# MadNLP/MadNLP.jl

Hardware: AMD Instinct MI355X
Metric: IP iterations/sec + ms per factorize!/solve!, condensed KKT n≈1e4 (higher is better)
Workload: dtype f64; 1 GPU; BASELINE config C3: case1354pegase-shaped sparse-condensed KKT, one instance; N=11192, m=16646, nnz(K)=68688; step = compress_J+compress_H+build_kkt+factorize (n_f=1) + inertia fetch + 2 solve_linear_system per instance; algorithm=BUNCHKAUFMAN (device: static-pivot LDL^T), outer_block=0, batch_per_gpu=1, batch_api=n/a (one instance), parallelism=1 GPU(s) x 1 independent instance(s)

## Files before the change

include/madnlp_hip.h:

```cpp
#ifndef MADNLP_HIP_H
#define MADNLP_HIP_H

#include <stdint.h>

#ifdef __cplusplus
extern "C" {
#endif

#define MNK_VERSION 100

enum { MNK_HOST = 0, MNK_DEVICE = 1 };

enum { MNK_BUNCHKAUFMAN = 1, MNK_LU = 2, MNK_QR = 3, MNK_CHOLESKY = 4, MNK_LDL = 5, MNK_EVD = 6 };

typedef struct mnk_ctx mnk_ctx;
typedef struct mnk_sc mnk_sc;
typedef struct mnk_dc mnk_dc;
typedef struct mnk_ls mnk_ls;

int mnk_version(void);
const char* mnk_last_error_string(void);
int mnk_ctx_create(int device, void* stream, mnk_ctx** out);
int mnk_ctx_destroy(mnk_ctx* ctx);
int mnk_ctx_synchronize(mnk_ctx* ctx);
// ... 196 lines not shown
int mnk_ipm_vec_scatter_axpy(mnk_ipm* ipm, double* y, const int64_t* idx, double a, const double* x, int64_t n);
int mnk_ipm_vec_gather(mnk_ipm* ipm, double* out, double a, const double* x, const int64_t* idx, int64_t n);
int mnk_ipm_bound_dual_axpy(mnk_ipm* ipm, double* zl, double* zu, double a, const double* dzl, const double* dzu);
int mnk_ipm_bound_dual_fill(mnk_ipm* ipm, double* zl, double* zu, double v);
int mnk_ipm_gemv(mnk_ipm* ipm, int trans, int64_t m, int64_t n, double alpha, const double* A, int64_t lda, const double* x,
                 double beta, double* y);

int mnk_ipm_vec_mul(mnk_ipm* ipm, double* out, const double* a, const double* b, int64_t n);
int mnk_ipm_scale_cons(mnk_ipm* ipm, double* c, const double* con_scale, const double* slack, const int64_t* slack_pos,
                       int64_t ns, const double* rhs, int64_t m);
int mnk_ipm_scale_grad(mnk_ipm* ipm, double* f, int64_t n, int64_t ntot, double factor);

typedef struct mnk_opf mnk_opf;
int mnk_opf_create(mnk_ctx* ctx, int64_t nbus, int64_t ngen, int64_t nbranch, const int32_t* fr, const int32_t* to,
                   const int32_t* gen_bus, const double* arc_coef, const double* bus_data, const double* gen_cost,
                   mnk_opf** out);
int mnk_opf_destroy(mnk_opf* opf);
int mnk_opf_sizes(mnk_opf* opf, int64_t* n, int64_t* m, int64_t* nnzj, int64_t* nnzh);
int mnk_opf_obj_terms(mnk_opf* opf, const double* x, double* terms );
int mnk_opf_grad(mnk_opf* opf, const double* x, double* g);
int mnk_opf_cons(mnk_opf* opf, const double* x, double* c);
int mnk_opf_jac_coord(mnk_opf* opf, const double* x, double* jac);
int mnk_opf_hess_coord(mnk_opf* opf, const double* x, const double* y, double obj_weight, double* hess);

typedef struct mnk_tape mnk_tape;
int mnk_tape_create(mnk_ctx* ctx, int64_t n, int64_t m, void* out);
int mnk_tape_destroy(void* tape);
int mnk_tape_add_pattern(void* tape, int kind , int64_t R, int k, int q,
                         const int32_t* var_index, const double* params, const int32_t* rows,
                         int64_t ninstr0, const int32_t* code0, int64_t nconst0, const double* consts0, int64_t nout0,
                         const int32_t* out_operand0, const int32_t* out_j0, const int32_t* out_l0, int nslot0,
                         int64_t ninstr1, const int32_t* code1, int64_t nconst1, const double* consts1, int64_t nout1,
                         const int32_t* out_operand1, const int32_t* out_j1, const int32_t* out_l1, int nslot1,
                         int64_t ninstr2, const int32_t* code2, int64_t nconst2, const double* consts2, int64_t nout2,
                         const int32_t* out_operand2, const int32_t* out_j2, const int32_t* out_l2, int nslot2);
int mnk_tape_finalize(void* tape);
int mnk_tape_sizes(void* tape, int64_t* n, int64_t* m, int64_t* nterms, int64_t* nnzj, int64_t* nnzh);
int mnk_tape_extended(void* tape, int* mask);
int mnk_tape_get_structure(void* tape, int32_t* jac_I, int32_t* jac_J, int32_t* hess_I, int32_t* hess_J);
int mnk_tape_obj_terms(void* tape, const double* x, double* terms );
int mnk_tape_grad(void* tape, const double* x, double* g);
int mnk_tape_cons(void* tape, const double* x, double* c);
int mnk_tape_jac_coord(void* tape, const double* x, double* jac);
int mnk_tape_hess_coord(void* tape, const double* x, const double* y, double obj_weight, double* hess);

typedef struct mnk_schur mnk_schur;
int mnk_schur_create(mnk_ctx* ctx, int64_t ns_local, int64_t blk, int64_t nd, int algo, mnk_schur** out);
int mnk_schur_destroy(mnk_schur* h);
int mnk_schur_set_block(mnk_schur* h, int64_t k, const double* A_kk, int64_t lda, const double* C_dk, int64_t ldc,
                        int loc);
int mnk_schur_build_local(mnk_schur* h, const double* S0, int64_t lds0, int loc_s0, double* S_out, int64_t lds_out);
int mnk_schur_factorize_s(mnk_schur* h, const double* S, int64_t lds, int loc, int* info);
int mnk_schur_inertia_s(mnk_schur* h, int64_t* num_pos, int64_t* num_zero, int64_t* num_neg);
int mnk_schur_scenario_inertia(mnk_schur* h, int64_t k, int64_t* num_pos, int64_t* num_zero, int64_t* num_neg);
int mnk_schur_scenario_bk_info(mnk_schur* h, int64_t k, int* active, int* count);
int mnk_schur_forward(mnk_schur* h, double* rhs_k, double* contrib_d);
int mnk_schur_solve_s(mnk_schur* h, double* rhs_d);
int mnk_schur_backward(mnk_schur* h, double* rhs_k, const double* x_d);
void* mnk_schur_s_buffer(mnk_schur* h);
int mnk_schur_set_structure(mnk_schur* h, int64_t n, int64_t m, int64_t nv, int64_t nc, int64_t nnzh, const int32_t* hess_I,
                            const int32_t* hess_J, int64_t nnzj, const int32_t* jac_I, const int32_t* jac_J, int64_t n_ineq,
                            const int64_t* ind_ineq, int64_t n_eq, const int64_t* ind_eq, int index_base, int64_t ns_global,
                            const int64_t* local_scen, int own_design);
int mnk_schur_assemble(mnk_schur* h, const double* hess, const double* jac, const double* pr_diag, const double* du_diag, int loc);
void* mnk_schur_s0_buffer(mnk_schur* h);
int mnk_schur_get_block(mnk_schur* h, int64_t k, double* A_kk, double* C_dk, double* S0);
int mnk_schur_solve(mnk_schur* h, double* rhs_k, double* rhs_d, int loc);

int mnk_ls_debug_solve_trace(mnk_ls* ls, unsigned long long* out, int64_t n);

int mnk_ls_debug_dag_state(mnk_ls* ls, int* flags, int64_t nflags, int* chain, int64_t nchain, int* have);

int mnk_debug_grid_at_launch(int cu_first, int num_cu, int first, int per_cu);
int mnk_debug_shader_clock(mnk_ctx* ctx, double* mhz);

int mnk_debug_dag_tasks(int ntile, int chunk, int band_tiles, int js2, int taper0, int* out, int cap, int* first_phase);
int mnk_debug_dag_merged_tasks(int ntile, int chunk, int band_tiles, int js2, int taper0, int fill, int ninst, int period,
                               int* out, int cap);
int mnk_debug_dag_deal(int ntile, int chunk, int band_tiles, int js2, int taper0, int fill, int ninst, int period, int nq, int gang,
                       int* tasks_out, int* order, int cap, int* off, int* first_phase);

int mnk_sc_debug_tile_env(mnk_sc* sc, int64_t order, int32_t* out, int cap);
int mnk_debug_tile_env_csc(int64_t n, const int32_t* colptr, const int32_t* rowval, int index_base, int32_t* out, int cap);

int mnk_debug_update(mnk_ctx* ctx, int variant, int64_t M, int64_t K, const double* A, int64_t lda,
                     double* C, double* C2, int64_t ldc, int reps, double* ms);

#ifdef __cplusplus
}
#endif
#endif
```

madnlp.jl_amd/_lib.py:

```python
from __future__ import annotations

import ctypes as C
import os
import subprocess

_HERE = os.path.dirname(os.path.abspath(__file__))
CSRC = os.path.join(_HERE, "csrc")
LIBDIR = os.path.join(_HERE, "lib")
LIBPATH = os.path.join(LIBDIR, "libmadnlp_hip.so")
_LIB_OVERRIDE = os.environ.get("MNK_LIBPATH")
SOURCES = ["gemm_f64.hip", "dag.hip", "factor.hip", "solve.hip", "ls.hip", "sparse_kkt.hip", "dense_kkt.hip", "bk.hip", "schur.hip", "ipm_vec.hip", "opf_eval.hip", "qr.hip", "lu.hip", "evd.hip", "qn.hip", "tape_eval.hip", "nlp_scale.hip"]
HEADERS = ["common.h", "ls.h", "kkt_vec.h", "gemm_tile.h", "leaf64.h", "ipm_handle.h", os.path.join("..", "..", "include", "madnlp_hip.h")]

MNK_HOST, MNK_DEVICE = 0, 1
MNK_BUNCHKAUFMAN, MNK_LU, MNK_QR, MNK_CHOLESKY, MNK_LDL, MNK_EVD = 1, 2, 3, 4, 5, 6
MNK_SC_JT, MNK_SC_HESS, MNK_SC_AUG, MNK_SC_DIAGBUF = 0, 1, 2, 3
MNK_QN_BFGS, MNK_QN_DAMPED_BFGS = 1, 2


def _stale() -> bool:
    if not os.path.exists(LIBPATH):
        return True
    t = os.path.getmtime(LIBPATH)
    deps = [os.path.join(CSRC, s) for s in SOURCES + HEADERS]
# ... 130 lines not shown
    "mnk_ipm_set_f_RR": (C.c_int, [_vp, _vp, _vp, _vp, _vp, C.c_double]),
    "mnk_ipm_set_aug_rhs_RR": (C.c_int, [_vp, _vp, _vp, _vp, _vp, _vp, _vp, _vp, _vp, _vp, _vp, C.c_int64, _vp, _vp, _vp, C.c_double, C.c_double, _vp, _vp, _vp, _vp]),
    "mnk_ipm_finish_aug_solve_RR": (C.c_int, [_vp, _vp, _vp, _vp, _vp, _vp, _vp, _vp, _vp, _vp, _vp, C.c_int64, C.c_double, C.c_double]),
    "mnk_ipm_reset_bound_dual_1": (C.c_int, [_vp, _vp, _vp, C.c_int64, C.c_double, C.c_double]),
    "mnk_ipm_set_initial_bounds": (C.c_int, [_vp, _vp, _vp, C.c_int64, C.c_double]),
    "mnk_ipm_set_initial_rhs": (C.c_int, [_vp, _vp, _vp, _vp, _vp, _vp, C.c_int64, _vp, _vp]),
    "mnk_ipm_set_aug_rhs_ifr": (C.c_int, [_vp, _vp, C.c_int64, _vp, _vp, _vp, _vp]),
    "mnk_ipm_set_g_ifr": (C.c_int, [_vp, _vp, _vp, _vp, _vp, _vp, _vp, C.c_double]),
    "mnk_ipm_initialize_variables": (C.c_int, [_vp, _vp, _vp, _vp, C.c_int64, C.c_double, C.c_double]),
    "mnk_ipm_get_dot": (C.c_int, [_vp, _vp, _vp, C.c_int64, C.POINTER(C.c_double)]),
    "mnk_ipm_get_sum": (C.c_int, [_vp, _vp, C.c_int64, C.POINTER(C.c_double)]),
    "mnk_ipm_get_norm2": (C.c_int, [_vp, _vp, C.c_int64, C.POINTER(C.c_double)]),
    "mnk_ipm_vec_copy": (C.c_int, [_vp, _vp, _vp, C.c_int64]),
    "mnk_ipm_vec_fill": (C.c_int, [_vp, _vp, C.c_int64, C.c_double]),
    "mnk_ipm_vec_axpby": (C.c_int, [_vp, _vp, C.c_double, _vp, C.c_double, _vp, C.c_int64]),
    "mnk_ipm_vec_scatter_axpy": (C.c_int, [_vp, _vp, _vp, C.c_double, _vp, C.c_int64]),
    "mnk_ipm_vec_gather": (C.c_int, [_vp, _vp, C.c_double, _vp, _vp, C.c_int64]),
    "mnk_ipm_bound_dual_axpy": (C.c_int, [_vp, _vp, _vp, C.c_double, _vp, _vp]),
    "mnk_ipm_bound_dual_fill": (C.c_int, [_vp, _vp, _vp, C.c_double]),
    "mnk_ipm_gemv": (C.c_int, [_vp, C.c_int, C.c_int64, C.c_int64, C.c_double, _vp, C.c_int64, _vp, C.c_double, _vp]),
    "mnk_ipm_vec_mul": (C.c_int, [_vp, _vp, _vp, _vp, C.c_int64]),
    "mnk_ipm_scale_cons": (C.c_int, [_vp, _vp, _vp, _vp, _vp, C.c_int64, _vp, C.c_int64]),
    "mnk_ipm_scale_grad": (C.c_int, [_vp, _vp, C.c_int64, C.c_int64, C.c_double]),
    "mnk_opf_create": (C.c_int, [_vp, C.c_int64, C.c_int64, C.c_int64, _vp, _vp, _vp, _vp, _vp, _vp, C.POINTER(_vp)]),
    "mnk_opf_destroy": (C.c_int, [_vp]),
    "mnk_opf_sizes": (C.c_int, [_vp, _i64p, _i64p, _i64p, _i64p]),
    "mnk_opf_obj_terms": (C.c_int, [_vp, _vp, _vp]),
    "mnk_opf_grad": (C.c_int, [_vp, _vp, _vp]),
    "mnk_opf_cons": (C.c_int, [_vp, _vp, _vp]),
    "mnk_opf_jac_coord": (C.c_int, [_vp, _vp, _vp]),
    "mnk_opf_hess_coord": (C.c_int, [_vp, _vp, _vp, C.c_double, _vp]),
    "mnk_tape_create": (C.c_int, [_vp, C.c_int64, C.c_int64, _vp]),
    "mnk_tape_destroy": (C.c_int, [_vp]),
    "mnk_tape_add_pattern": (C.c_int, [_vp, C.c_int, C.c_int64, C.c_int, C.c_int, _vp, _vp, _vp]
                             + [C.c_int64, _vp, C.c_int64, _vp, C.c_int64, _vp, _vp, _vp, C.c_int] * 3),
    "mnk_tape_finalize": (C.c_int, [_vp]),
    "mnk_tape_sizes": (C.c_int, [_vp, _i64p, _i64p, _i64p, _i64p, _i64p]),
    "mnk_tape_extended": (C.c_int, [_vp, _vp]),
    "mnk_tape_get_structure": (C.c_int, [_vp, _vp, _vp, _vp, _vp]),
    "mnk_tape_obj_terms": (C.c_int, [_vp, _vp, _vp]),
    "mnk_tape_grad": (C.c_int, [_vp, _vp, _vp]),
    "mnk_tape_cons": (C.c_int, [_vp, _vp, _vp]),
    "mnk_tape_jac_coord": (C.c_int, [_vp, _vp, _vp]),
    "mnk_tape_hess_coord": (C.c_int, [_vp, _vp, _vp, C.c_double, _vp]),
    "mnk_sc_set_aug_RR": (C.c_int, [_vp, _vp, _vp, _vp, _vp, _vp, _vp, _vp, _vp, _vp, _vp, C.c_double, C.c_double, C.c_double]),
    "mnk_dc_set_aug_RR": (C.c_int, [_vp, _vp, _vp, _vp, _vp, _vp, _vp, _vp, _vp, _vp, _vp, C.c_double, C.c_double, C.c_double]),
    "mnk_ls_bk_info": (C.c_int, [_vp, C.POINTER(C.c_int), C.POINTER(C.c_int), _vp, _vp]),
    "mnk_ls_get_stat": (C.c_int, [_vp, C.c_char_p, C.POINTER(C.c_double)]),
    "mnk_sc_set_bounds": (C.c_int, [_vp, C.c_int64, _vp, C.c_int64, _vp, C.c_int]),
    "mnk_sc_set_barrier_terms": (C.c_int, [_vp, _vp, _vp, _vp, _vp, _vp, C.c_int]),
    "mnk_sc_solve_kkt": (C.c_int, [_vp, _vp, _vp, C.c_int]),
    "mnk_sc_mul": (C.c_int, [_vp, _vp, _vp, C.c_double, C.c_double, C.c_int]),
    "mnk_dc_set_bounds": (C.c_int, [_vp, C.c_int64, _vp, C.c_int64, _vp, C.c_int]),
    "mnk_dc_set_barrier_terms": (C.c_int, [_vp, _vp, _vp, _vp, _vp, _vp, C.c_int]),
    "mnk_dc_solve_kkt": (C.c_int, [_vp, _vp, _vp, C.c_int]),
    "mnk_dc_mul": (C.c_int, [_vp, _vp, _vp, C.c_double, C.c_double, C.c_int]),
    "mnk_schur_create": (C.c_int, [_vp, C.c_int64, C.c_int64, C.c_int64, C.c_int, C.POINTER(_vp)]),
    "mnk_schur_destroy": (C.c_int, [_vp]),
    "mnk_schur_set_block": (C.c_int, [_vp, C.c_int64, _vp, C.c_int64, _vp, C.c_int64, C.c_int]),
    "mnk_schur_build_local": (C.c_int, [_vp, _vp, C.c_int64, C.c_int, _vp, C.c_int64]),
    "mnk_schur_factorize_s": (C.c_int, [_vp, _vp, C.c_int64, C.c_int, C.POINTER(C.c_int)]),
    "mnk_schur_inertia_s": (C.c_int, [_vp, _i64p, _i64p, _i64p]),
    "mnk_schur_scenario_inertia": (C.c_int, [_vp, C.c_int64, _i64p, _i64p, _i64p]),
    "mnk_schur_scenario_bk_info": (C.c_int, [_vp, C.c_int64, C.POINTER(C.c_int), C.POINTER(C.c_int)]),
    "mnk_schur_forward": (C.c_int, [_vp, _vp, _vp]),
    "mnk_schur_solve_s": (C.c_int, [_vp, _vp]),
    "mnk_schur_backward": (C.c_int, [_vp, _vp, _vp]),
    "mnk_schur_s_buffer": (C.c_void_p, [_vp]),
    "mnk_schur_set_structure": (C.c_int, [_vp, C.c_int64, C.c_int64, C.c_int64, C.c_int64, C.c_int64, _vp, _vp, C.c_int64, _vp, _vp,
                                          C.c_int64, _vp, C.c_int64, _vp, C.c_int, C.c_int64, _vp, C.c_int]),
    "mnk_schur_assemble": (C.c_int, [_vp, _vp, _vp, _vp, _vp, C.c_int]),
    "mnk_schur_s0_buffer": (_vp, [_vp]),
    "mnk_schur_get_block": (C.c_int, [_vp, C.c_int64, _vp, _vp, _vp]),
    "mnk_schur_solve": (C.c_int, [_vp, _vp, _vp, C.c_int]),
    "mnk_ls_debug_solve_trace": (C.c_int, [_vp, _vp, C.c_int64]),
    "mnk_ls_debug_dag_state": (C.c_int, [_vp, _vp, C.c_int64, _vp, C.c_int64, _vp]),
    "mnk_debug_grid_at_launch": (C.c_int, [C.c_int, C.c_int, C.c_int, C.c_int]),
    "mnk_debug_shader_clock": (C.c_int, [_vp, _vp]),
    "mnk_debug_dag_tasks": (C.c_int, [C.c_int, C.c_int, C.c_int, C.c_int, C.c_int, _vp, C.c_int, _vp]),
    "mnk_debug_dag_merged_tasks": (C.c_int, [C.c_int] * 8 + [_vp, C.c_int]),
    "mnk_debug_dag_deal": (C.c_int, [C.c_int] * 10 + [_vp, _vp, C.c_int, _vp, _vp]),
    "mnk_sc_debug_tile_env": (C.c_int, [_vp, C.c_int64, _vp, C.c_int]),
    "mnk_debug_tile_env_csc": (C.c_int, [C.c_int64, _vp, _vp, C.c_int, _vp, C.c_int]),
    "mnk_factorize_batch_begin": (C.c_int, []),
    "mnk_factorize_batch_end": (C.c_int, []),
    "mnk_solve_batch_begin": (C.c_int, []),
    "mnk_solve_batch_end": (C.c_int, []),
    "mnk_release_idle_streams": (C.c_int, [C.c_int]),
    "mnk_sc_step_batch": (C.c_int, [C.c_int, _vp, _vp, _vp, _vp, _vp, _vp, C.c_int]),
    "mnk_ls_inertia_batch": (C.c_int, [C.c_int, _vp, _i64p, _i64p, _i64p]),
    "mnk_ls_solve_batch": (C.c_int, [C.c_int, _vp, _vp, C.c_int]),
    "mnk_debug_update": (C.c_int, [_vp, C.c_int, C.c_int64, C.c_int64, _vp, C.c_int64, _vp, _vp, C.c_int64, C.c_int,
                                   C.POINTER(C.c_double)]),
    "mnk_gemm_nt": (C.c_int, [_vp, C.c_int, C.c_int64, C.c_int64, C.c_int64, _vp, C.c_int64, _vp,
                              C.c_int64, _vp, C.c_int64]),
}


def lib():
    global _lib
    if _lib is not None:
        return _lib
    if not os.path.exists(LIBPATH):
        raise ImportError(
            f"{LIBPATH} is missing: run `python -c 'import __graft_entry__ as g; g.build()'` "
            "(hipcc --offload-arch=gfx950).  There is no CPU fallback for the KKT hot path.")
    try:
        import torch
    except Exception:
        pass
    l = C.CDLL(_LIB_OVERRIDE if _LIB_OVERRIDE and os.path.exists(_LIB_OVERRIDE) else LIBPATH)
    for name, (res, args) in SIGNATURES.items():
        f = getattr(l, name)
        f.restype = res
        f.argtypes = args
    _lib = l
    return l


class HipError(RuntimeError):
    pass


def check(rc: int, what: str = ""):
    if rc != 0:
        msg = lib().mnk_last_error_string()
        raise HipError(f"{what} failed (rc={rc}): {msg.decode() if msg else ''}")
```

madnlp.jl_amd/csrc/common.h:

```cpp
#pragma once
#include <hip/hip_runtime.h>
#include <cstdint>
#include <cstdlib>
#include <cstdio>
#include <cstring>
#include <mutex>
#include <string>
#include <vector>

#include "../../include/madnlp_hip.h"

namespace mnk {

void set_error(const char* fmt, ...);

#define MNK_HIP(call)                                                                   \
    do {                                                                                \
        hipError_t e_ = (call);                                                         \
        if (e_ != hipSuccess) {                                                         \
            mnk::set_error("%s:%d: %s -> %s", __FILE__, __LINE__, #call, hipGetErrorString(e_)); \
            return -2;                                                                  \
        }                                                                               \
    } while (0)

// ... 115 lines not shown

struct mnk_ctx {
    int device = 0;
    hipStream_t stream = nullptr;
    bool own_stream = false;
    hipStream_t sp = nullptr, su = nullptr;
    int panel_cus = 0;
    hipStream_t sp_dag = nullptr, su_dag = nullptr;
    hipStream_t sp_dagB = nullptr, su_dagB = nullptr;
    bool shared_dag_streams = false;
    int dag_cus = 0;
    hipStream_t sp_dag2 = nullptr, su_dag2 = nullptr;
    int dag_cus2 = 0;
    hipEvent_t ev_a = nullptr, ev_b = nullptr;
    hipStream_t s_fill = nullptr;
    std::vector<hipEvent_t> ev_panel, ev_next, ev_next2, ev_bdone;
    int num_cu = 256;
    int cu_first = 0;
    int total_cu = 256;
    bool partitioned = false;
    void* persist_slot = nullptr;
    int children = 0;
    bool released = false;
};
int mnk_masked_stream_pair(mnk_ctx* ctx, int chain_cus, hipStream_t* sp, hipStream_t* su);
int mnk_ctx_ensure_panel_streams(mnk_ctx* ctx);
int mnk_ctx_ensure_dag(mnk_ctx* ctx);
int mnk_ctx_ensure_dag2(mnk_ctx* ctx);
int mnk_ctx_ensure_batch_streams(mnk_ctx* ctx);
int mnk_solve_warmup(hipStream_t s);
int mnk_ctx_bulk_wgs(const mnk_ctx* ctx, int first, int per_cu);
int mnk_dag_warmup(hipStream_t* streams, int n, int nwg);
int mnk_live_contexts(int device);
int mnk_persist_begin(mnk_ctx* ctx, hipStream_t s);
int mnk_persist_end(mnk_ctx* ctx, hipStream_t s, int rc);
void mnk_ctx_child_added(mnk_ctx* ctx);
void mnk_ctx_child_gone(mnk_ctx* ctx);

namespace mnk {
struct PpDag {
    int* front;
    const int* af;
    int ntile;
    int need_front;
    int front_from;
    int af_tilecol;
    long spin_limit;
    unsigned long long* trace;
    unsigned long long* vmax;
    int* dbg;
};
}

namespace mnk {

int launch_gemm_nt(hipStream_t s, int mode, int64_t M, int64_t N, int64_t K,
                   const double* A, int64_t lda, const double* B, int64_t ldb,
                   double* C, int64_t ldc, const double* colscale, double* C2, int64_t ldc2,
                   const int* info_flag);
struct TrsmBatchRec { double* X; double* V; const double* dblk; const double* inv16; const double* dinv; const int* info; };
struct GemmBatchRec { const double* A; const double* B; double* C; const int* info; };
int launch_gemm_nt_batch(hipStream_t s, int64_t M, int64_t N, int64_t K, const GemmBatchRec* recs_dev, int nbatch, int64_t lda,
                         int64_t ldb, int64_t ldc);
int launch_gemm_nt_lower_small(hipStream_t s, int64_t M, int64_t N, int64_t K, const double* A, int64_t lda,
                               const double* B, int64_t ldb, double* C, int64_t ldc, const int* info_flag);
int gemm_nt_lower_tiles(int64_t M, int64_t N);
int launch_gemm_nt_dbg(hipStream_t s, int shared_ab, int64_t M, int64_t N, int64_t K, const double* A, int64_t lda,
                       const double* B, int64_t ldb, double* C, int64_t ldc);
int launch_gemm_nt_lower_range(hipStream_t s, int64_t M, int64_t N, int64_t K, const double* A, int64_t lda,
                               const double* B, int64_t ldb, double* C, int64_t ldc, const int* info_flag,
                               int tile_begin, int tile_count);
int launch_gemm_nt_queue(hipStream_t s, int64_t M, int64_t N, int64_t K, const double* A, int64_t lda,
                         const double* B, int64_t ldb, double* C, int64_t ldc, int* counter, int cus,
                         const int* info_flag);

int dag_build_tasks(int ntile, int chunk, int band_tiles, int js2, std::vector<int>& out, int taper0, std::vector<int>* ready);
int dag_add_fill_tasks(int ntile, std::vector<int>& tasks, std::vector<int>& ready, int n1);
void dag_merge_tasks(const std::vector<int>& tasks, const std::vector<int>& ready, int ninst, int period, std::vector<int>& out);
constexpr int DAG_NQ = 8;
constexpr int DAG_QHEAD_STRIDE = 32;
constexpr int DAG_QHEAD_WORDS = (DAG_NQ + 1) * DAG_QHEAD_STRIDE;
void dag_deal_tasks(const std::vector<int>& tasks, const std::vector<int>& ready, int t0, int t1, int nq, int gang, std::vector<int>& order,
                    std::vector<int>& off);

}
```

madnlp.jl_amd/csrc/dag.hip:

```cpp
#include <algorithm>
#include <atomic>
#include <cfloat>
#include <climits>
#include <vector>

#include "gemm_tile.h"
#include "ls.h"

namespace mnk {


struct DagInst {
    double* F;
    int64_t ld;
    double* V;
    const double* dinv;
    const double* dblk;
    const double* inv16;
    int* front;
    int* af;
    int* tprog;
    int* info;
    unsigned long long* vmax;
    double* zfill;
    int64_t N;
    const int* env;
    const int* envgate;
};

typedef const DagInst __attribute__((address_space(4))) * DagInstP;

struct DagArgs {
    const DagInst* insts;
    const int4* tasks;
    int ntasks;
    int ntile;
    int* qctr;
    long spin_limit;
    unsigned long long* trace;
    unsigned long long* wgstat;
    int fake_share;
};

constexpr int DAG_BANDACC = 1, DAG_FINAL = 2, DAG_FIRST = 4, DAG_FILL = 8;

template <class IP>
__device__ __forceinline__ int dag_wait_front(IP a, long spin_limit, int s0, int s1, int s2, int s3, int c, int kend, int* s_val) {
    if (threadIdx.x < 64) {
        const int lane = threadIdx.x;
        const int idx = lane == 0 ? s0 : (lane == 1 ? s1 : (lane == 2 ? s2 : s3));
        long spins = 0;
        int r;
        for (;;) {
            int f = lane < 4 ? __hip_atomic_load(a->front + idx, __ATOMIC_RELAXED, __HIP_MEMORY_SCOPE_AGENT) : INT_MAX;
            f = min(f, __shfl_xor(f, 1));
            f = min(f, __shfl_xor(f, 2));
            r = __builtin_amdgcn_readfirstlane(f);
            if (r > c) break;
            __builtin_amdgcn_s_sleep(4);
            if ((++spins & 255) == 0) {
                if (__hip_atomic_load(a->info, __ATOMIC_RELAXED, __HIP_MEMORY_SCOPE_AGENT) != 0) {
                    r = -1;
                    break;
                }
                if (spins > spin_limit) {
                    if (lane == 0 && atomicCAS(a->info, 0, -7) == 0) a->info[1] = 1;
                    r = -1;
                    break;
                }
            }
        }
        if (r > kend) r = kend;
        __builtin_amdgcn_fence(__ATOMIC_ACQUIRE, "agent");
        if (lane == 0) *s_val = r;
    }
    __syncthreads();
    const int r = *s_val;
    __syncthreads();
    return r;
}

template <class IP>
__device__ __forceinline__ bool dag_wait_words(IP a, long spin_limit, const int* w0, int t0, const int* w1, int t1, int* s_val) {
    if (threadIdx.x < 64) {
        const int lane = threadIdx.x;
        long spins = 0;
        int ok = 1;
        for (;;) {
            const int v = lane < 2 ? __hip_atomic_load(lane == 0 ? w0 : w1, __ATOMIC_RELAXED, __HIP_MEMORY_SCOPE_AGENT) : INT_MAX;
            if (__all(v >= (lane == 0 ? t0 : (lane == 1 ? t1 : INT_MIN)))) break;
            __builtin_amdgcn_s_sleep(2);
            if ((++spins & 255) == 0) {
                if (__hip_atomic_load(a->info, __ATOMIC_RELAXED, __HIP_MEMORY_SCOPE_AGENT) != 0) {
                    ok = 0;
                    break;
                }
                if (spins > spin_limit) {
                    if (lane == 0 && atomicCAS(a->info, 0, -7) == 0) a->info[1] = 2;
                    ok = 0;
                    break;
                }
            }
        }
        __builtin_amdgcn_fence(__ATOMIC_ACQUIRE, "agent");
        if (lane == 0) *s_val = ok;
    }
    __syncthreads();
    const int ok = *s_val;
    __syncthreads();
    return ok != 0;
// ... 279 lines not shown
#pragma unroll
            for (int i = 0; i < 8; ++i) { asm volatile("" : "+v"(X[i][0])); asm volatile("" : "+v"(X[i][1])); }
            if (tr) tr[1] = tr[3] = wall_clock64();
            if (dag_wait_front(in, a.spin_limit, 2 * J, 2 * J + 1, 2 * J, 2 * J + 1, J, J + 1, &s_val) < 0) return false;
            if (tr) { tr[4] = wall_clock64(); s_stat[1] += tr[4] - tr[3]; }
            dag_finalize_tile<LDL>(in, row0, col0, 2 * J, smem_raw, tid, X, tr);
            if (tr) s_stat[3] += wall_clock64() - tr[4];
        } else if (!(I == J && kend > k0)) {
            v4f64 acc[4][4];
#pragma unroll
            for (int i = 0; i < 4; ++i)
#pragma unroll
                for (int j = 0; j < 4; ++j) acc[i][j] = v4f64{0.0, 0.0, 0.0, 0.0};
            if (flags & DAG_FINAL) __builtin_amdgcn_s_setprio(3);
            if (!gemm_nt_mainloop<2, 2, 4, 0, 8>(acc, Ak, in->ld, Bk, in->ld, (kend - k0) * 16, smem_raw, tid, gate)) return false;
            if (tr) tr[1] = wall_clock64();
            if (!wait_chunk_order()) return false;
            if (kend > k0)
                gemm_nt_epilogue<2, 2, 4, 2, false, true>(acc, row0, col0, (int64_t)1 << 40, (int64_t)1 << 40, in->F, in->ld, nullptr, nullptr, 0, tid);
            if (tr) tr[3] = wall_clock64();
        } else {
            v4f64 acc[4][4];
#pragma unroll
            for (int i = 0; i < 4; ++i)
#pragma unroll
                for (int j = 0; j < 4; ++j) acc[i][j] = v4f64{0.0, 0.0, 0.0, 0.0};
            __builtin_amdgcn_s_setprio(3);
            if (!wait_chunk_order()) return false;
            gemm_nt_load_neg_lower<2, 2, 4>(acc, row0, col0, in->F, in->ld, tid);
            if (!gemm_nt_mainloop<2, 2, 4, 0, 8>(acc, Ak, in->ld, Bk, in->ld, (kend - k0) * 16, smem_raw, tid, gate)) return false;
            if (tr) tr[1] = wall_clock64();
            gemm_nt_store_neg_lower<2, 2, 4>(acc, row0, col0, in->F, in->ld, tid);
            if (tr) tr[3] = wall_clock64();
        }
        return true;
        };
        const bool done = run_task();
        asm volatile("s_waitcnt vmcnt(0)" ::: "memory");
        __syncthreads();
        if (done && tid == 0) {
            __builtin_amdgcn_fence(__ATOMIC_RELEASE, "agent");
            asm volatile("s_waitcnt vmcnt(0)" ::: "memory");
            if (!(flags & DAG_FINAL)) {
                __hip_atomic_store(in->tprog + (int64_t)I * a.ntile + J, q + 1, __ATOMIC_RELAXED, __HIP_MEMORY_SCOPE_AGENT);
            } else if (!(flags & DAG_BANDACC)) {
                __hip_atomic_store(in->front + 2 * I, J + 1, __ATOMIC_RELAXED, __HIP_MEMORY_SCOPE_AGENT);
                __hip_atomic_store(in->front + 2 * I + 1, J + 1, __ATOMIC_RELAXED, __HIP_MEMORY_SCOPE_AGENT);
            } else {
                __hip_atomic_store(in->af + (int64_t)I * a.ntile + J, 1, __ATOMIC_RELAXED, __HIP_MEMORY_SCOPE_AGENT);
            }
            if (tr) tr[5] = wall_clock64();
        }
        __builtin_amdgcn_s_setprio(0);
        __syncthreads();
        };
        do_task((DagInstP)(uintptr_t)(a.insts + inst));
    }
}

struct DagArgs1 {
    double* F;
    int64_t ld;
    double* V;
    const double* dinv;
    const double* dblk;
    const double* inv16;
    const int4* tasks;
    int ntasks;
    int* front;
    int* af;
    int* tprog;
    int ntile;
    int* qctr;
    int* info;
    long spin_limit;
    unsigned long long* trace;
    unsigned long long* wgstat;
    unsigned long long* vmax;
    int fake_share;
    double* zfill;
    int64_t N;
    const int* env;
    const int* envgate;
    const int* qoff;
    int* qheads;
    int nq;
};

__device__ __forceinline__ int dag_pop(const int* __restrict__ qoff, int* __restrict__ qheads, int nq, int* sq) {
    const int h = sq[0];
    if (h >= 0) {
        const int beg = qoff[h], n = qoff[h + 1] - beg;
        const int i = atomicAdd(qheads + h * DAG_QHEAD_STRIDE, 1);
        if (i < n) return beg + i;
        sq[0] = -1 - h;
    }
    for (;;) {
        int best = -1, most = 0;
        for (int x = 0; x < nq; ++x) {
            const int left = qoff[x + 1] - qoff[x] - __hip_atomic_load(qheads + x * DAG_QHEAD_STRIDE, __ATOMIC_RELAXED, __HIP_MEMORY_SCOPE_AGENT);
            if (left > most) { most = left; best = x; }
        }
        if (best < 0) return INT_MAX;
        const int i = atomicAdd(qheads + best * DAG_QHEAD_STRIDE, 1);
        if (i < qoff[best + 1] - qoff[best]) {
            sq[1] += 1;
            atomicAdd(qheads + nq * DAG_QHEAD_STRIDE, 1);
            return qoff[best] + i;
        }
    }
}

template <bool LDL>
__global__ __launch_bounds__(256, 3) void dag_bulk_kernel1(DagArgs1 a) {
    extern __shared__ __attribute__((aligned(16))) char smem_raw[];
    __shared__ int s_val;
    __shared__ int s_q[2];
    if (threadIdx.x == 0) {
        unsigned xcc;
        asm volatile("s_getreg_b32 %0, hwreg(HW_REG_XCC_ID)" : "=s"(xcc));
        s_q[0] = a.nq > 0 ? (int)(xcc & 15u) % a.nq : 0;
        s_q[1] = 0;
    }
    __shared__ unsigned long long s_stat[4];
    if (threadIdx.x < 4) s_stat[threadIdx.x] = 0;
    const int* __restrict__ env = a.env != nullptr && __builtin_amdgcn_readfirstlane(*a.envgate) == 0 ? a.env : nullptr;
    __syncthreads();
    for (;;) {
        int tid = threadIdx.x;
        asm volatile("" : "+v"(tid));
        if (tid == 0)
            s_val = __hip_atomic_load(a.info, __ATOMIC_RELAXED, __HIP_MEMORY_SCOPE_AGENT) != 0
                        ? INT_MAX
                        : (a.nq > 0 ? dag_pop(a.qoff, a.qheads, a.nq, s_q) : atomicAdd(a.qctr, 1));
        __syncthreads();
        const int t = s_val;
        __syncthreads();
        if (t >= a.ntasks) {
            if (a.wgstat != nullptr && tid == 0) {
                unsigned long long* w = a.wgstat + (int64_t)blockIdx.x * 8;
                w[0] = s_stat[0]; w[1] = wall_clock64(); w[2] = s_stat[1]; w[3] = s_stat[2]; w[4] = s_stat[3];
                w[5] = a.nq > 0 ? (unsigned long long)(1 + (s_q[0] >= 0 ? s_q[0] : -1 - s_q[0])) : 0; w[6] = (unsigned long long)s_q[1];
            }
            return;
        }
        if (a.wgstat != nullptr && tid == 0) { if (s_stat[0] == 0) s_stat[0] = wall_clock64(); ++s_stat[2]; }
        const int4 tk = a.tasks[t];
        const int flags = __builtin_amdgcn_readfirstlane(tk.x) & 255, q = __builtin_amdgcn_readfirstlane(tk.x) >> 8;
        const int I = __builtin_amdgcn_readfirstlane(tk.y), J = __builtin_amdgcn_readfirstlane(tk.z) & 0xfff;
        const int kbeg = __builtin_amdgcn_readfirstlane(tk.w) & 0xffff, kend = __builtin_amdgcn_readfirstlane(tk.w) >> 16;
        const int64_t row0 = (int64_t)128 * I, col0 = (int64_t)128 * J;
        unsigned long long* tr = a.trace != nullptr && tid == 0
                                     ? a.trace + (int64_t)(a.nq > 0 ? (int)((unsigned)__builtin_amdgcn_readfirstlane(tk.z) >> 12) : t) * 8
                                     : nullptr;
        if (tr) { tr[0] = wall_clock64(); tr[6] = 0; tr[7] = 0; }
        if (flags & DAG_FILL) {
            if (a.zfill != nullptr) dag_fill_tile(&a, I, J, tid);
            continue;
        }

        int eI = 0, k0 = kbeg;
        if (env != nullptr) {
            eI = __builtin_amdgcn_readfirstlane(env[I]);
            k0 = min(kend, max(kbeg, max(eI, __builtin_amdgcn_readfirstlane(env[J]))));
        }
        int limit = 0;
        auto gate_at = [&](int kc) -> int {
            const unsigned long long w0 = tr ? wall_clock64() : 0;
            const int r = dag_wait_front(&a, a.spin_limit, 2 * I, 2 * I + 1, 2 * J, 2 * J + 1, kc, kend, &s_val);
            if (tr) { const unsigned long long w1 = wall_clock64(); tr[2] = w1; tr[6] += 1; tr[7] += w1 - w0; s_stat[1] += w1 - w0; }
            return r;
        };
        auto gate = [&](int kt) -> bool {
            if (kt < limit) return true;
            const int r = gate_at(k0 + (kt >> 4));
            if (r < 0) return false;
            limit = (__builtin_amdgcn_readfirstlane(r) - k0) * 16;
            return true;
        };
        const double* Ak = a.F + (a.fake_share > 0 ? (int64_t)128 * (kend + I % a.fake_share) : row0) + (int64_t)128 * k0 * a.ld;
        const double* Bk = (LDL ? a.V : a.F) + (a.fake_share > 0 ? (int64_t)128 * (kend + J % a.fake_share) : col0) + (int64_t)128 * k0 * a.ld;
        auto wait_chunk_order = [&]() -> bool {
            if (flags & DAG_FIRST) return true;
            const int* word = a.tprog + (int64_t)I * a.ntile + J;
            const unsigned long long w0 = tr ? wall_clock64() : 0;
            if (!dag_wait_words(&a, a.spin_limit, word, q, word, q, &s_val)) return false;
            if (tr) s_stat[1] += wall_clock64() - w0;
            return true;
        };
        if ((flags & DAG_FINAL) && !(flags & DAG_BANDACC)) {
            __builtin_amdgcn_s_setprio(3);
            if (!wait_chunk_order()) return;
            if (J < eI) {
                if (kend > kbeg && gate_at(kbeg) < 0) return;
                if (LDL) dag_zero_tile(a.V, a.ld, row0, col0, tid);
                goto publish;
            }
            v4f64 X[8][2];
            {
                const int lane = tid & 63, w = tid >> 6;
                const double* Cs = a.F + (row0 + 32 * w + (lane & 15)) + (col0 + (lane >> 4)) * a.ld;
#pragma unroll
                for (int cb = 0; cb < 8; ++cb)
#pragma unroll
                    for (int r = 0; r < 4; ++r) {
                        const double* cp = Cs + (int64_t)(16 * cb + 4 * r) * a.ld;
                        X[cb][0][r] = cp[0];
                        X[cb][1][r] = cp[16];
                    }
            }
            if (kend > kbeg && gate_at(kbeg) < 0) return;
            if (kend > k0) (void)gemm_nt_mainloop3<2, 8, true>(X, Ak, a.ld, Bk, a.ld, (kend - k0) * 16, smem_raw, tid);
#pragma unroll
            for (int i = 0; i < 8; ++i) { asm volatile("" : "+v"(X[i][0])); asm volatile("" : "+v"(X[i][1])); }
            if (tr) tr[1] = tr[3] = wall_clock64();
            if (dag_wait_front(&a, a.spin_limit, 2 * J, 2 * J + 1, 2 * J, 2 * J + 1, J, J + 1, &s_val) < 0) return;
            if (tr) { tr[4] = wall_clock64(); s_stat[1] += tr[4] - tr[3]; }
            dag_finalize_tile<LDL>(&a, row0, col0, 2 * J, smem_raw, tid, X, tr);
            if (tr) s_stat[3] += wall_clock64() - tr[4];
        } else if (!(I == J && kend > k0)) {
            v4f64 acc[4][4];
#pragma unroll
            for (int i = 0; i < 4; ++i)
#pragma unroll
                for (int j = 0; j < 4; ++j) acc[i][j] = v4f64{0.0, 0.0, 0.0, 0.0};
            if (flags & DAG_FINAL) __builtin_amdgcn_s_setprio(3);
            if (!gemm_nt_mainloop<2, 2, 4, 0, 8>(acc, Ak, a.ld, Bk, a.ld, (kend - k0) * 16, smem_raw, tid, gate)) return;
            if (tr) tr[1] = wall_clock64();
            if (!wait_chunk_order()) return;
            if (kend > k0)
                gemm_nt_epilogue<2, 2, 4, 2, false, true>(acc, row0, col0, (int64_t)1 << 40, (int64_t)1 << 40, a.F, a.ld, nullptr, nullptr, 0, tid);
            if (tr) tr[3] = wall_clock64();
        } else {
            v4f64 acc[4][4];
#pragma unroll
            for (int i = 0; i < 4; ++i)
#pragma unroll
                for (int j = 0; j < 4; ++j) acc[i][j] = v4f64{0.0, 0.0, 0.0, 0.0};
            __builtin_amdgcn_s_setprio(3);
            if (!wait_chunk_order()) return;
            gemm_nt_load_neg_lower<2, 2, 4>(acc, row0, col0, a.F, a.ld, tid);
            if (!gemm_nt_mainloop<2, 2, 4, 0, 8>(acc, Ak, a.ld, Bk, a.ld, (kend - k0) * 16, smem_raw, tid, gate)) return;
            if (tr) tr[1] = wall_clock64();
            gemm_nt_store_neg_lower<2, 2, 4>(acc, row0, col0, a.F, a.ld, tid);
            if (tr) tr[3] = wall_clock64();
        }
    publish:
        asm volatile("s_waitcnt vmcnt(0)" ::: "memory");
        __syncthreads();
        if (tid == 0) {
            __builtin_amdgcn_fence(__ATOMIC_RELEASE, "agent");
            asm volatile("s_waitcnt vmcnt(0)" ::: "memory");
            if (!(flags & DAG_FINAL)) {
                __hip_atomic_store(a.tprog + (int64_t)I * a.ntile + J, q + 1, __ATOMIC_RELAXED, __HIP_MEMORY_SCOPE_AGENT);
            } else if (!(flags & DAG_BANDACC)) {
                __hip_atomic_store(a.front + 2 * I, J + 1, __ATOMIC_RELAXED, __HIP_MEMORY_SCOPE_AGENT);
                __hip_atomic_store(a.front + 2 * I + 1, J + 1, __ATOMIC_RELAXED, __HIP_MEMORY_SCOPE_AGENT);
            } else {
                __hip_atomic_store(a.af + (int64_t)I * a.ntile + J, 1, __ATOMIC_RELAXED, __HIP_MEMORY_SCOPE_AGENT);
            }
            if (tr) tr[5] = wall_clock64();
        }
        __builtin_amdgcn_s_setprio(0);
        __syncthreads();
    }
}

int dag_build_tasks(int ntile, int chunk, int band_tiles, int js2, std::vector<int>& out, int taper0, std::vector<int>* ready) {
    struct T { int ready, cls, J, I, flags, q, kbeg, kend; };
    std::vector<T> ts;
    auto add_tile = [&](int I, int J, int K, bool band) {
        const int body = band ? K : std::max(0, K - 1);
        std::vector<int> cuts{body};
        int e = body;
        for (int len = taper0; len < chunk && e > 0; len *= 2) { e = std::max(0, e - len); cuts.push_back(e); }
        const int first = 1 + (I * 5 + J * 3) % chunk;
        while (e > first) { e = std::max(first, e - chunk); cuts.push_back(e); }
        if (e > 0) cuts.push_back(0);
        int q = 0;
        for (int c = (int)cuts.size() - 1; c > 0; --c, ++q) {
            const int kb = cuts[c], ke = cuts[c - 1];
            const bool last = band && ke == K;
            ts.push_back({ke, band ? 0 : 2, J, I, (band ? DAG_BANDACC : 0) | (last ? DAG_FINAL : 0) | (q == 0 ? DAG_FIRST : 0), q, kb, ke});
        }
        if (!band) ts.push_back({K, 1, J, I, DAG_FINAL | (q == 0 ? DAG_FIRST : 0), q, body, K});
    };
    for (int Jt = 0; Jt < ntile; ++Jt) {
        const int Js = Jt / 2;
        const int bt = Js >= js2 ? ntile : band_tiles;
        for (int I = 2 * Js + bt; I < ntile; ++I) add_tile(I, Jt, Jt, false);
        if (2 * Js - 2 > 0)
            for (int I = std::max(2 * Js, Jt); I < 2 * Js + bt && I < ntile; ++I) add_tile(I, Jt, 2 * Js - 2, true);
    }
    std::stable_sort(ts.begin(), ts.end(), [](const T& x, const T& y) {
        if (x.ready != y.ready) return x.ready < y.ready;
        if (x.cls != y.cls) return x.cls < y.cls;
        if (x.J != y.J) return x.J < y.J;
        return x.I < y.I;
    });
    out.clear();
    out.reserve(ts.size() * 4);
    if (ready != nullptr) { ready->clear(); ready->reserve(ts.size()); }
    int n1 = 0;
    for (const T& t : ts) {
        if (t.ready <= 2 * js2) ++n1;
        if (ready != nullptr) ready->push_back(t.ready);
        out.push_back(t.flags | (t.q << 8));
        out.push_back(t.I);
        out.push_back(t.J);
        out.push_back(t.kbeg | (t.kend << 16));
    }
    return n1;
}

int dag_add_fill_tasks(int ntile, std::vector<int>& tasks, std::vector<int>& ready, int n1) {
    const int nt = (int)(tasks.size() / 4), nfill = ntile * (ntile + 1) / 2;
    const int span = n1 > 0 ? n1 : nt;
    if (span <= 0) return n1;
    std::vector<int> out, rdy;
    out.reserve(tasks.size() + 4 * (size_t)nfill);
    rdy.reserve(ready.size() + nfill);
    int fi = 0, fj = 0, done = 0;
    auto emit_fill = [&](int r) {
        out.push_back(DAG_FILL); out.push_back(fi); out.push_back(fj); out.push_back(0);
        rdy.push_back(r);
        if (++fi >= ntile) { ++fj; fi = fj; }
        ++done;
    };
    for (int t = 0; t < nt; ++t) {
        for (int k = 0; k < 4; ++k) out.push_back(tasks[4 * t + k]);
        rdy.push_back(ready[t]);
        if (t < span)
            while (done < (int)((int64_t)(t + 1) * nfill / span)) emit_fill(ready[t]);
    }
    tasks.swap(out);
    ready.swap(rdy);
    return n1 > 0 ? n1 + nfill : 0;
}

void dag_merge_tasks(const std::vector<int>& tasks, const std::vector<int>& ready, int ninst, int period, std::vector<int>& out) {
    const int nt = (int)ready.size();
    out.clear();
    out.reserve((size_t)ninst * nt * 4);
    std::vector<int> pos(ninst, 0);
    for (;;) {
        int best = -1;
        long bkey = 0;
        for (int i = 0; i < ninst; ++i) {
            if (pos[i] >= nt) continue;
            const long key = (long)i * period + ready[pos[i]];
            if (best < 0 || key < bkey) { best = i; bkey = key; }
        }
        if (best < 0) break;
        const int t = pos[best]++;
        out.push_back(tasks[4 * t]);
        out.push_back(tasks[4 * t + 1] | (best << 16));
        out.push_back(tasks[4 * t + 2]);
        out.push_back(tasks[4 * t + 3]);
    }
}

void dag_deal_tasks(const std::vector<int>& tasks, const std::vector<int>& ready, int t0, int t1, int nq, int gang, std::vector<int>& order,
                    std::vector<int>& off) {
    nq = std::max(nq, 1);
    std::vector<std::vector<int>> qs(nq);
    std::vector<int64_t> load(nq, 0);
    int rr = 0;
    auto cls = [&](int t) { const int f = tasks[4 * (size_t)t] & 255; return (f & DAG_FILL) ? 3 : ((f & DAG_BANDACC) ? 0 : ((f & DAG_FINAL) ? 1 : 2)); };
    auto ksteps = [&](int t) { return (tasks[4 * (size_t)t] & DAG_FILL) ? 0 : (tasks[4 * (size_t)t + 3] >> 16) - (tasks[4 * (size_t)t + 3] & 0xffff); };
    auto same = [&](int x, int y) {
        return ready[x] == ready[y] && cls(x) == cls(y) && tasks[4 * (size_t)x + 2] == tasks[4 * (size_t)y + 2] &&
               tasks[4 * (size_t)x + 3] == tasks[4 * (size_t)y + 3] && (tasks[4 * (size_t)x + 1] >> 16) == (tasks[4 * (size_t)y + 1] >> 16);
    };
    auto deal = [&](int b, int e) {
        int q = 0;
        if (gang >= 0) {
            q = rr % nq;
            for (int i = 1; i < nq; ++i)
                if (load[(rr + i) % nq] < load[q]) q = (rr + i) % nq;
            rr = q + 1;
        }
        for (int t = b; t < e; ++t) { qs[q].push_back(t); load[q] += ksteps(t); }
    };
    for (int i = t0; i < t1;) {
        int j = i + 1;
        const int c = cls(i);
        if (gang > 1 && (c == 0 || c == 2))
            while (j < t1 && same(i, j)) ++j;
        for (int b = i; b < j; b += std::max(gang, 1)) deal(b, std::min(j, b + std::max(gang, 1)));
        i = j;
    }
    order.clear();
    off.assign(1, 0);
    for (int q = 0; q < nq; ++q) {
        order.insert(order.end(), qs[q].begin(), qs[q].end());
        off.push_back((int)order.size());
    }
}

template <bool LDL>
static int launch_bulk_t(hipStream_t s, const DagArgs& a, int nwg) {
    const size_t smem = TILE3_LDS_BYTES;
    auto kern = dag_bulk_kernel<LDL>;
    static std::atomic<uint64_t> attr_devs{0};
    int dev = 0;
    MNK_HIP(hipGetDevice(&dev));
    if (!(attr_devs.load(std::memory_order_relaxed) >> (dev & 63) & 1)) {
        MNK_HIP(hipFuncSetAttribute((const void*)kern, hipFuncAttributeMaxDynamicSharedMemorySize, (int)smem));
        attr_devs.fetch_or(1ull << (dev & 63), std::memory_order_relaxed);
    }
    hipLaunchKernelGGL(kern, dim3(nwg), dim3(256), smem, s, a);
    MNK_HIP(hipGetLastError());
    return 0;
}

template <bool LDL>
static int launch_bulk1_t(hipStream_t s, const DagArgs1& a, int nwg) {
    const size_t smem = TILE3_LDS_BYTES;
    auto kern = dag_bulk_kernel1<LDL>;
    static std::atomic<uint64_t> attr_devs{0};
    int dev = 0;
    MNK_HIP(hipGetDevice(&dev));
    if (!(attr_devs.load(std::memory_order_relaxed) >> (dev & 63) & 1)) {
        MNK_HIP(hipFuncSetAttribute((const void*)kern, hipFuncAttributeMaxDynamicSharedMemorySize, (int)smem));
        attr_devs.fetch_or(1ull << (dev & 63), std::memory_order_relaxed);
    }
    hipLaunchKernelGGL(kern, dim3(nwg), dim3(256), smem, s, a);
    MNK_HIP(hipGetLastError());
    return 0;
}

static int launch_dag_bulk(hipStream_t s, bool ldl, const DagInst& one, const DagInst* insts, const int* tasks, int ntasks, int ntile,
                           int* qctr, long spin_limit, int nwg, unsigned long long* trace, unsigned long long* wgstat,
                           const int* qoff = nullptr, int* qheads = nullptr, int nq = 0) {
    if (ntasks <= 0) return 0;
    static const int fake = getenv("MNK_DAG_FAKE_SHARE") ? atoi(getenv("MNK_DAG_FAKE_SHARE")) : 0;
    if (insts == nullptr) {
        DagArgs1 a{one.F, one.ld, one.V, one.dinv, one.dblk, one.inv16, reinterpret_cast<const int4*>(tasks), ntasks, one.front, one.af,
                   one.tprog, ntile, qctr, one.info, spin_limit, trace, wgstat, one.vmax, fake, one.zfill, one.N, one.env, one.envgate,
                   qoff, qheads, nq};
        return ldl ? launch_bulk1_t<true>(s, a, nwg) : launch_bulk1_t<false>(s, a, nwg);
    }
    DagArgs a{insts, reinterpret_cast<const int4*>(tasks), ntasks, ntile, qctr, spin_limit, trace, wgstat, fake};
    return ldl ? launch_bulk_t<true>(s, a, nwg) : launch_bulk_t<false>(s, a, nwg);
}

}

using namespace mnk;

int mnk_dag_warmup(hipStream_t* streams, int n, int nwg) {
    static mnk::DevBuf<int> ctr;
    if (!ctr.p) {
        if (ctr.alloc(4)) return -2;
        MNK_HIP(hipMemset(ctr.p, 0, 4 * sizeof(int)));
    }
    for (int i = 0; i < n; ++i) {
        if (streams[i] == nullptr) continue;
        mnk::DagArgs1 a1{};
        a1.qctr = ctr.p;
        a1.info = ctr.p + 1;
        mnk::DagArgs a{};
        a.qctr = ctr.p;
        int rc = mnk::launch_bulk1_t<true>(streams[i], a1, nwg);
        if (!rc) rc = mnk::launch_bulk1_t<false>(streams[i], a1, nwg);
        if (!rc) rc = mnk::launch_bulk_t<true>(streams[i], a, nwg);
        if (!rc) rc = mnk::launch_bulk_t<false>(streams[i], a, nwg);
        if (rc) return rc;
    }
    for (int i = 0; i < n; ++i)
        if (streams[i] != nullptr) MNK_HIP(mnk::stream_wait(streams[i]));
    return 0;
}

long mnk_ls_dag_spin_limit(const mnk_ls* ls) {
    if (ls->dag_spin_limit > 0) return ls->dag_spin_limit;
    const double n = (double)ls->Np;
    const double t_est = n * n * n / 3.0 / 50e12;
    const double polls = 10.0 * t_est / 0.17e-6;
    const double floor_polls = mnk_live_contexts(ls->ctx->device) > 1 ? 5880000.0 : 588000.0;
    return (long)std::min(16777216.0, std::max(floor_polls, polls));
}

static int bulk_xcds(const mnk_ctx* c, int first) {
    bool has[8] = {false, false, false, false, false, false, false, false};
    for (int b = std::max(first, 0); b < c->num_cu; ++b) has[(c->cu_first + b) % 8] = true;
    int n = 0;
    for (bool x : has) n += x ? 1 : 0;
    return n;
}

static mnk::DagInst dag_instance(mnk_ls* ls) {
    const int ntile = (int)(ls->Np / 128), nblk = (int)(ls->Np / NBI);
    int* front = ls->dag_flags.p + 2;
    int* af = front + nblk;
    int* tprog = af + (size_t)ntile * ntile;
    double* zfill = (ls->dag_fill && ls->dag_has_fill && ls->spare_pending && ls->fact_spare.p && !ls->spare_zeroed) ? ls->fact_spare.p : nullptr;
    const bool env = ls->envelope && ls->env_dev != nullptr && ls->env_word.p != nullptr;
    return mnk::DagInst{ls->fact.p, ls->ld, ls->algo == MNK_LDL ? ls->vfull.p : nullptr, ls->dinv.p, ls->dblk.p, ls->inv16.p,
                        front, af, tprog, ls->info_dev.p, mnk_ls_growth_word(ls), zfill, ls->N, env ? ls->env_dev : nullptr,
                        env ? ls->env_word.p + 1 : nullptr};
}

int mnk_ls_dag_prepare(mnk_ls* ls) {
    mnk_ctx* ctx = ls->ctx;
    hipStream_t s = ctx->stream;
    const int64_t Np = ls->Np, ld = ls->ld;
    const bool ldl = ls->algo == MNK_LDL;
    const int ntile = (int)(Np / 128), nblk = (int)(Np / NBI), nsc = (int)((Np + 255) / 256);
    const size_t nflags = (size_t)2 + nblk + 2 * (size_t)ntile * ntile;
    auto give_up = [&]() {
        (void)hipGetLastError();
        ls->dag_tasks.release();
        ls->dag_flags.release();
        ls->dag_qoff.release();
        ls->dag_qheads.release();
        ls->vfull.release();
        return 1;
    };
    if (!ls->dag_tasks.p) {
        const int64_t deep_rows = std::min<int64_t>((int64_t)ctx->dag_cus2 * NBI, ls->dag_deep_rows);
        ls->dag_js2 = (ctx->dag_cus2 > 0 && Np <= deep_rows) ? 0 : nsc;
        if (ls->dag_js2_override >= 0) ls->dag_js2 = std::min(nsc, ls->dag_js2_override);
        std::vector<int>& h = ls->dag_host_tasks;
        ls->dag_ntasks1 = mnk::dag_build_tasks(ntile, ls->dag_chunk, ls->dag_band / 2, ls->dag_js2, h, ls->dag_taper0, &ls->dag_host_ready);
        ls->dag_has_fill = ls->dag_fill && ls->prefill && Np <= ls->prefill_max_rows;
        if (ls->dag_has_fill && h.empty()) ls->dag_has_fill = false;
        if (ls->dag_has_fill) ls->dag_ntasks1 = mnk::dag_add_fill_tasks(ntile, h, ls->dag_host_ready, ls->dag_ntasks1);
        ls->dag_ntasks = (int)(h.size() / 4);
        std::vector<int> dev_list = h, qoff(32, 0);
        ls->dag_nq[0] = ls->dag_nq[1] = 0;
        if (ls->dag_xcd_queues && ls->dag_ntasks < (1 << 20) && ntile < 4096) {
            const int part[3] = {0, ls->dag_ntasks1, ls->dag_ntasks};
            const int chain_cus[2] = {ctx->dag_cus, ctx->dag_cus2};
            for (int ph = 0; ph < 2; ++ph) {
                const int t0 = part[ph], t1 = part[ph + 1];
                if (t1 - t0 < mnk_ctx_bulk_wgs(ctx, chain_cus[ph], 3) || bulk_xcds(ctx, chain_cus[ph]) != mnk::DAG_NQ) continue;
                std::vector<int> order, off;
                mnk::dag_deal_tasks(h, ls->dag_host_ready, t0, t1, mnk::DAG_NQ, ls->dag_gang, order, off);
                for (int p = 0; p < t1 - t0; ++p) {
                    for (int k = 0; k < 4; ++k) dev_list[4 * (size_t)(t0 + p) + k] = h[4 * (size_t)order[p] + k];
                    dev_list[4 * (size_t)(t0 + p) + 2] |= (order[p] - t0) << 12;
                }
                for (int x = 0; x <= mnk::DAG_NQ; ++x) qoff[16 * ph + x] = off[x];
                ls->dag_nq[ph] = mnk::DAG_NQ;
            }
        }
        if (ls->dag_tasks.alloc(h.size() + 4)) return give_up();
        if (!ls->dag_qoff.p && ls->dag_qoff.alloc(qoff.size())) return give_up();
        if (!ls->dag_qheads.p && ls->dag_qheads.alloc(2 * (size_t)mnk::DAG_QHEAD_WORDS)) return give_up();
        {
            mnk::H2DGuard h2d;
            if (!h.empty() && hipMemcpyAsync(ls->dag_tasks.p, dev_list.data(), dev_list.size() * sizeof(int), hipMemcpyHostToDevice, s) != hipSuccess) return give_up();
            if (hipMemcpyAsync(ls->dag_qoff.p, qoff.data(), qoff.size() * sizeof(int), hipMemcpyHostToDevice, s) != hipSuccess) return give_up();
            if (mnk::stream_wait(s) != hipSuccess) return give_up();
        }
        if (ls->dag_flags.alloc(nflags)) return give_up();
    }
    if (ldl && !ls->vfull.p && ls->vfull.alloc((size_t)ld * Np + SLACK)) {
        (void)hipGetLastError();
        bool ok = false;
        if (ls->fact_spare.p && !ls->spare_zeroed) {
            ls->fact_spare.release();
            ls->prefill = 0;
            ls->spare_pending = false;
            ok = ls->vfull.alloc((size_t)ld * Np + SLACK) == 0;
        }
        if (!ok) return give_up();
    }
    if (ls->dag_trace_on) {
        const size_t ntr = (size_t)ls->dag_ntasks * 8 + 4096 * 8 + 1024 * 8;
        if (ls->dag_trace.n < ntr && ls->dag_trace.alloc(ntr)) return give_up();
    }
    return 0;
}

int mnk_ls_run_factorization_dag(mnk_ls* ls) {
    mnk_ctx* ctx = ls->ctx;
    hipStream_t s = ctx->stream;
    const int64_t Np = ls->Np;
    const bool ldl = ls->algo == MNK_LDL;
    const int ntile = (int)(Np / 128), nblk = (int)(Np / NBI), nsc = (int)((Np + 255) / 256);
    const size_t nflags = (size_t)2 + nblk + 2 * (size_t)ntile * ntile;
    MNK_REQUIRE(ls->dag_tasks.p && ls->dag_flags.p && (!ldl || ls->vfull.p), "task-DAG schedule: mnk_ls_dag_prepare was not called");
    const mnk::DagInst inst = dag_instance(ls);
    ls->dag_filled = inst.zfill != nullptr;
    ls->env_used = inst.env != nullptr;
    hipLaunchKernelGGL(mnk::dag_reset_kernel, dim3((unsigned)std::min<size_t>((nflags + 1023) / 1024, 64)), dim3(256), 0, s,
                       ls->dag_flags.p, (int64_t)nflags, ls->info_dev.p, inst, (mnk::DagInst*)nullptr, (const mnk::SmallSysRec*)nullptr,
                       ls->env_word.p, ls->dag_qheads.p, ls->dag_qheads.p ? 2 * mnk::DAG_QHEAD_WORDS : 0);
    ls->env_armed = false;
    int* qctr = ls->dag_flags.p;
    int* front = inst.front;
    const long spin_limit = mnk_ls_dag_spin_limit(ls);
    unsigned long long* trace = nullptr;
    if (ls->dag_trace_on && ls->dag_trace.p) {
        const size_t ntr = (size_t)ls->dag_ntasks * 8 + 4096 * 8 + 1024 * 8;
        MNK_HIP(hipMemsetAsync(ls->dag_trace.p, 0, ntr * sizeof(unsigned long long), s));
        trace = ls->dag_trace.p;
    }
    const int js2 = ls->dag_js2;
    auto phase = [&](hipStream_t sp, hipStream_t su, int chain_cus, int task0, int ntask, int* counter, int js_begin, int js_end,
                     unsigned strips) -> int {
        const bool small = js_begin == 0 && js_end == nsc && js2 == 0 && ls->dag_chain_inline;
        if (small) sp = s;
        MNK_HIP(hipEventRecord(ctx->ev_a, s));
        if (!small) MNK_HIP(hipStreamWaitEvent(sp, ctx->ev_a, 0));
        MNK_HIP(hipStreamWaitEvent(su, ctx->ev_a, 0));
        mnk::PpDag dag{front, inst.af, ntile, 0, 0, -1, spin_limit, trace ? trace + (size_t)ls->dag_ntasks * 8 + (size_t)js_begin * 8 * 16 : nullptr,
                  mnk_ls_growth_word(ls), ls->dag_debug ? ls->dag_dbg.p : nullptr};
        int rc = mnk_launch_pchain(ls, sp, dag, js_begin, js_end, strips);
        if (rc) return rc;
        const int ph = (int)(counter - qctr), nq = ls->dag_nq[ph];
        MNK_REQUIRE(nq == 0 || (ntask >= mnk_ctx_bulk_wgs(ctx, chain_cus, 3) && bulk_xcds(ctx, chain_cus) == nq),
                    "task-DAG schedule: the bulk grid does not cover the XCDs the task list was dealt for");
        rc = mnk::launch_dag_bulk(su, ldl, inst, nullptr, ls->dag_tasks.p + 4 * (size_t)task0, ntask, ntile, counter, spin_limit,
                                  std::min(ntask, mnk_ctx_bulk_wgs(ctx, chain_cus, 3)), trace ? trace + 8 * (size_t)task0 : nullptr,
                                  trace ? trace + (size_t)ls->dag_ntasks * 8 + 4096 * 8 + (task0 > 0 ? 512 * 8 : 0) : nullptr,
                                  ls->dag_qoff.p + 16 * ph, ls->dag_qheads.p + ph * mnk::DAG_QHEAD_WORDS, nq);
        if (rc) return rc;
        if (js_begin == 0 && js_end > 0) {
            const int64_t safe = std::min<int64_t>(js_end, std::max<int64_t>(0, (ntile - ls->dag_band / 2 - 1) / 2)) & ~(int64_t)1;
            if (strips == (unsigned)ls->dag_band && safe > 0) {
                rc = mnk_ls_invert_blocks(ls, su, 0, safe);
                if (rc) return rc;
                ls->inv_done = safe;
            }
        }
        if (small) {
            rc = mnk_ls_invert_blocks(ls, s, 0, nsc);
            if (rc) return rc;
            ls->inv_done = nsc;
        } else if (js_begin == 0 && js_end == nsc && js2 == 0) {
            hipLaunchKernelGGL(mnk::dag_gate_kernel, dim3(1), dim3(1), 0, su, front + (nblk - 1), ntile, ls->info_dev.p, spin_limit);
            rc = mnk_ls_invert_blocks(ls, su, 0, nsc);
            if (rc) return rc;
            ls->inv_done = nsc;
        }
        if (!small) MNK_HIP(hipEventRecord(ctx->ev_a, sp));
        MNK_HIP(hipEventRecord(ctx->ev_b, su));
        if (!small) MNK_HIP(hipStreamWaitEvent(s, ctx->ev_a, 0));
        MNK_HIP(hipStreamWaitEvent(s, ctx->ev_b, 0));
        return 0;
    };
    if (js2 > 0) {
        int rc = phase(ctx->sp_dag, ctx->su_dag, ctx->dag_cus, 0, ls->dag_ntasks1, qctr, 0, std::min(js2, nsc),
                       (unsigned)std::min<int64_t>(ls->dag_band, Np / NBI));
        if (rc) return rc;
    }
    if (js2 < nsc) {
        const int64_t rows2 = Np - 256 * (int64_t)js2;
        MNK_REQUIRE(ctx->sp_dag2 != nullptr, "task-DAG schedule: the deep-band streams are missing");
        int rc = phase(ctx->sp_dag2, ctx->su_dag2, ctx->dag_cus2, ls->dag_ntasks1, ls->dag_ntasks - ls->dag_ntasks1,
                       qctr + 1, js2, nsc, (unsigned)(rows2 / NBI));
        if (rc) return rc;
    }
    return 0;
}

namespace {
struct BatchState {
    int depth = 0;
    bool active = false;
    std::vector<mnk_ls*> pend;
};
thread_local BatchState t_batch;

struct BatchBuffers {
    mnk::DevBuf<int> tasks;
    mnk::DevBuf<int> qctr;
    mnk::DevBuf<char> insts, pcsys, aux;
    char* stage = nullptr;
    size_t stage_bytes = 0;
    hipEvent_t stage_ev = nullptr;
    int ntile = 0, ninst = 0, period = 0, chunk = 0, taper0 = 0, band = 0, ntasks = 0;
    bool fill = false;
    hipEvent_t ev[4] = {nullptr, nullptr, nullptr, nullptr};
};
BatchBuffers g_batch[64];
}

bool mnk_batch_active() { return t_batch.active; }

bool mnk_batch_defer(mnk_ls* ls) {
    if (!t_batch.active) return false;
    const int nsc = (int)((ls->Np + 255) / 256);
    if (ls->algo_now != 5 || (ls->dag_js2 != nsc && ls->dag_js2 != 0) || ls->dag_trace_on || ls->ctx->partitioned) return false;
    if (mnk_ctx_ensure_batch_streams(ls->ctx) != 0) (void)hipGetLastError();
    if (!ls->ctx->sp_dagB) return false;
    if (!ls->ev_defer && hipEventCreateWithFlags(&ls->ev_defer, hipEventDisableTiming) != hipSuccess) { (void)hipGetLastError(); return false; }
    if (hipEventRecord(ls->ev_defer, ls->ctx->stream) != hipSuccess) { (void)hipGetLastError(); return false; }
    ls->deferred = true;
    t_batch.pend.push_back(ls);
    return true;
}

static void batch_mark_done(mnk_ls* ls) {
    ls->factorized = true;
    ls->info_valid = false;
    ls->bk_active = false;
    ls->deferred = false;
}

static int batch_run_group(std::vector<mnk_ls*>& g) {
    mnk_ls* l0 = g[0];
    mnk_ctx* c0 = l0->ctx;
    hipStream_t h = c0->stream;
    MNK_HIP(hipSetDevice(c0->device));
    const int64_t Np = l0->Np;
    const bool ldl = l0->algo == MNK_LDL;
    const int ntile = (int)(Np / 128), nsc = (int)((Np + 255) / 256), ninst = (int)g.size();
    const size_t nflags = (size_t)2 + (size_t)(Np / NBI) + 2 * (size_t)ntile * ntile;
    for (mnk_ls* ls : g)
        if (ls->ctx->stream != h) MNK_HIP(hipStreamWaitEvent(h, ls->ev_defer, 0));
    int rc = mnk_persist_begin(c0, h);
    if (rc) return rc;
    auto body = [&]() -> int {
        BatchBuffers& B = g_batch[c0->device & 63];
        const int period = std::max((ntile + 1) / 2, l0->batch_period > 0 ? l0->batch_period : 0);
        if (B.ntile != ntile || B.ninst != ninst || B.period != period || B.chunk != l0->dag_chunk || B.taper0 != l0->dag_taper0 ||
            B.band != l0->dag_band || B.fill != l0->dag_has_fill || !B.tasks.p) {
            std::vector<int> merged;
            mnk::dag_merge_tasks(l0->dag_host_tasks, l0->dag_host_ready, ninst, period, merged);
            if (B.tasks.alloc(merged.size() + 4)) return -2;
            { mnk::H2DGuard h2d; MNK_HIP(hipMemcpy(B.tasks.p, merged.data(), merged.size() * sizeof(int), hipMemcpyHostToDevice)); }
            if (!B.qctr.p && B.qctr.alloc(4)) return -2;
            if (B.insts.alloc(sizeof(mnk::DagInst) * (size_t)ninst)) return -2;
            for (hipEvent_t& e : B.ev)
                if (!e) MNK_HIP(hipEventCreateWithFlags(&e, hipEventDisableTiming));
            B.ntile = ntile; B.ninst = ninst; B.period = period; B.chunk = l0->dag_chunk; B.taper0 = l0->dag_taper0;
            B.band = l0->dag_band; B.fill = l0->dag_has_fill; B.ntasks = (int)(merged.size() / 4);
        }
        std::vector<mnk::DagInst> hin;
        mnk::DagInst* insts_dev = reinterpret_cast<mnk::DagInst*>(B.insts.p);
        for (mnk_ls* ls : g) {
            hin.push_back(dag_instance(ls));
            ls->dag_filled = hin.back().zfill != nullptr;
            ls->env_used = hin.back().env != nullptr;
            hipLaunchKernelGGL(mnk::dag_reset_kernel, dim3((unsigned)std::min<size_t>((nflags + 1023) / 1024, 64)), dim3(256), 0, h,
                               ls->dag_flags.p, (int64_t)nflags, ls->info_dev.p, hin.back(), insts_dev + (hin.size() - 1),
                               (const mnk::SmallSysRec*)nullptr, ls->env_word.p);
            ls->env_armed = false;
        }
        MNK_HIP(hipMemsetAsync(B.qctr.p, 0, 4 * sizeof(int), h));
        hipStream_t sp[2] = {c0->sp_dag, c0->sp_dagB}, su = c0->su_dagB;
        MNK_HIP(hipEventRecord(B.ev[0], h));
        MNK_HIP(hipStreamWaitEvent(sp[0], B.ev[0], 0));
        MNK_HIP(hipStreamWaitEvent(sp[1], B.ev[0], 0));
        MNK_HIP(hipStreamWaitEvent(su, B.ev[0], 0));
        const unsigned strips = (unsigned)std::min<int64_t>(l0->dag_band, Np / NBI);
        const int bulk_wgs = mnk_ctx_bulk_wgs(c0, 2 * c0->dag_cus, 3);
        auto launch_chain = [&](int i) -> int {
            mnk_ls* ls = g[i];
            mnk::PpDag dag{hin[i].front, hin[i].af, ntile, 0, 0, -1, mnk_ls_dag_spin_limit(ls), nullptr, mnk_ls_growth_word(ls)};
            return mnk_launch_pchain(ls, sp[i & 1], dag, 0, nsc, strips);
        };
        auto launch_tail = [&](int i) -> int {
            mnk_ls* ls = g[i];
            int r = mnk_ls_invert_blocks(ls, sp[i & 1], 0, nsc);
            if (r) return r;
            ls->inv_done = nsc;
            return mnk_ls_launch_finish_info(ls, sp[i & 1]);
        };
        for (int i = 0; i < std::min(2, ninst); ++i) {
            int r = launch_chain(i);
            if (r) return r;
        }
        int r = mnk::launch_dag_bulk(su, ldl, hin[0], insts_dev, B.tasks.p, B.ntasks, ntile, B.qctr.p,
                                     mnk_ls_dag_spin_limit(l0), std::min(B.ntasks, bulk_wgs), nullptr, nullptr);
        if (r) return r;
        for (int i = 0; i < ninst; ++i) {
            r = launch_tail(i);
            if (r) return r;
            if (i + 2 < ninst) {
                r = launch_chain(i + 2);
                if (r) return r;
            }
        }
        MNK_HIP(hipEventRecord(B.ev[1], sp[0]));
        MNK_HIP(hipEventRecord(B.ev[2], sp[1]));
        MNK_HIP(hipEventRecord(B.ev[3], su));
        for (int e = 1; e < 4; ++e) MNK_HIP(hipStreamWaitEvent(h, B.ev[e], 0));
        return 0;
    };
    rc = body();
    rc = mnk_persist_end(c0, h, rc);
    if (rc) return rc;
    MNK_HIP(hipEventRecord(l0->ev_defer, h));
    for (mnk_ls* ls : g) {
        if (ls->ctx->stream != h) MNK_HIP(hipStreamWaitEvent(ls->ctx->stream, l0->ev_defer, 0));
        batch_mark_done(ls);
        int r = mnk_ls_prefill_spare(ls);
        if (r) return r;
    }
    return 0;
}

static int batch_run_group_small(std::vector<mnk_ls*>& g) {
    mnk_ls* l0 = g[0];
    mnk_ctx* c0 = l0->ctx;
    hipStream_t h = c0->stream;
    MNK_HIP(hipSetDevice(c0->device));
    const int64_t Np = l0->Np;
    const bool ldl = l0->algo == MNK_LDL;
    const int ntile = (int)(Np / 128), nsc = (int)((Np + 255) / 256), strips = (int)(Np / NBI);
    const size_t nflags = (size_t)2 + (size_t)(Np / NBI) + 2 * (size_t)ntile * ntile;
    const int ntasks1 = l0->dag_ntasks;
    const int bulk_min = ntasks1 > 0 ? std::max(32, c0->num_cu / 4) : 0;
    auto chain_cus_for = [&](int k) { return std::min(c0->num_cu, (k * strips + 63) / 64 * 64); };
    int kmax = std::min(32, (c0->num_cu - bulk_min) / strips);
    while (kmax > 1 && chain_cus_for(kmax) > c0->num_cu - bulk_min) --kmax;
    if (kmax < 2) {
        for (mnk_ls* ls : g) {
            ls->deferred = false;
            int rc = mnk_ls_run_factorization_now(ls);
            if (rc) return rc;
        }
        return 0;
    }
    for (mnk_ls* ls : g)
        if (ls->ctx->stream != h) MNK_HIP(hipStreamWaitEvent(h, ls->ev_defer, 0));
    BatchBuffers& B = g_batch[c0->device & 63];
    for (size_t r0 = 0; r0 < g.size(); r0 += (size_t)kmax) {
        const int k = (int)std::min<size_t>(kmax, g.size() - r0);
        hipStream_t sp = nullptr, su = nullptr;
        int rc = mnk_masked_stream_pair(c0, chain_cus_for(k), &sp, &su);
        if (rc) return rc;
        if (ntasks1 > 0 && su == nullptr) { set_error("factorize batch: no CUs left for the bulk kernel"); return -1; }
        rc = mnk_persist_begin(c0, h);
        if (rc) return rc;
        auto body = [&]() -> int {
            if (ntasks1 > 0 && (B.ntile != ntile || B.ninst != k || B.period != 0 || B.chunk != l0->dag_chunk || B.taper0 != l0->dag_taper0 ||
                                B.band != l0->dag_band || B.fill != l0->dag_has_fill || !B.tasks.p)) {
                std::vector<int> merged;
                mnk::dag_merge_tasks(l0->dag_host_tasks, l0->dag_host_ready, k, 0, merged);
                if (B.tasks.alloc(merged.size() + 4)) return -2;
                { mnk::H2DGuard h2d; MNK_HIP(hipMemcpy(B.tasks.p, merged.data(), merged.size() * sizeof(int), hipMemcpyHostToDevice)); }
                B.ntile = ntile; B.ninst = k; B.period = 0; B.chunk = l0->dag_chunk; B.taper0 = l0->dag_taper0;
                B.band = l0->dag_band; B.fill = l0->dag_has_fill; B.ntasks = (int)(merged.size() / 4);
            }
            if (!B.qctr.p && B.qctr.alloc(4)) return -2;
            if (B.insts.n < sizeof(mnk::DagInst) * (size_t)k && B.insts.alloc(sizeof(mnk::DagInst) * (size_t)std::max(k, 32))) return -2;
            if (B.pcsys.n < mnk_pchain_sys_bytes() * (size_t)k && B.pcsys.alloc(mnk_pchain_sys_bytes() * (size_t)std::max(k, 32))) return -2;
            for (hipEvent_t& e : B.ev)
                if (!e) MNK_HIP(hipEventCreateWithFlags(&e, hipEventDisableTiming));
            std::vector<mnk::DagInst> hin;
            std::vector<int*> fronts;
            std::vector<const int*> afs;
            mnk::DagInst* insts_dev = reinterpret_cast<mnk::DagInst*>(B.insts.p);
            const size_t pc_bytes = mnk_pchain_sys_bytes();
            const size_t need = (size_t)k * (sizeof(mnk::DagInst) + pc_bytes + sizeof(mnk::SmallSysRec));
            if (B.aux.n < sizeof(mnk::SmallSysRec) * (size_t)k && B.aux.alloc(sizeof(mnk::SmallSysRec) * (size_t)std::max(k, 32))) return -2;
            if (B.stage_ev == nullptr) MNK_HIP(hipEventCreateWithFlags(&B.stage_ev, hipEventDisableTiming));
            else MNK_HIP(hipEventSynchronize(B.stage_ev));
            if (B.stage_bytes < need) {
                mnk::LaunchLock lock;
                if (B.stage) { mnk::quiesce_persistent(); (void)hipHostFree(B.stage); B.stage = nullptr; }
                const size_t cap = (size_t)std::max(k, 32) * (sizeof(mnk::DagInst) + pc_bytes + sizeof(mnk::SmallSysRec));
                MNK_HIP(hipHostMalloc((void**)&B.stage, cap, hipHostMallocDefault));
                B.stage_bytes = cap;
            }
            mnk::DagInst* st_inst = reinterpret_cast<mnk::DagInst*>(B.stage);
            char* st_pc = B.stage + (size_t)k * sizeof(mnk::DagInst);
            mnk::SmallSysRec* st_aux = reinterpret_cast<mnk::SmallSysRec*>(st_pc + (size_t)k * pc_bytes);
            const bool batch_aux = l0->linv_mfma && !l0->solve512;
            for (int i = 0; i < k; ++i) {
                mnk_ls* ls = g[r0 + i];
                hin.push_back(dag_instance(ls));
                ls->dag_filled = hin.back().zfill != nullptr;
                hin.back().env = nullptr;
                hin.back().envgate = nullptr;
                ls->env_used = false;
                fronts.push_back(hin.back().front);
                afs.push_back(hin.back().af);
                st_inst[i] = hin.back();
                mnk_pchain_fill_sys(ls, st_pc + (size_t)i * pc_bytes, hin.back().front, hin.back().af);
                mnk_ls_fill_small_rec(ls, st_aux + i);
            }
            MNK_HIP(hipMemcpyAsync(B.insts.p, st_inst, (size_t)k * sizeof(mnk::DagInst), hipMemcpyHostToDevice, h));
            MNK_HIP(hipMemcpyAsync(B.pcsys.p, st_pc, (size_t)k * pc_bytes, hipMemcpyHostToDevice, h));
            MNK_HIP(hipMemcpyAsync(B.aux.p, st_aux, (size_t)k * sizeof(mnk::SmallSysRec), hipMemcpyHostToDevice, h));
            MNK_HIP(hipEventRecord(B.stage_ev, h));
            const mnk::SmallSysRec* aux_dev = reinterpret_cast<const mnk::SmallSysRec*>(B.aux.p);
            hipLaunchKernelGGL(mnk::dag_reset_kernel, dim3((unsigned)std::min<size_t>((nflags + 1023) / 1024, 64), (unsigned)k), dim3(256), 0, h,
                               (int*)nullptr, (int64_t)0, (int*)nullptr, hin[0], (mnk::DagInst*)nullptr, aux_dev);
            MNK_HIP(hipMemsetAsync(B.qctr.p, 0, 4 * sizeof(int), h));
            MNK_HIP(hipEventRecord(B.ev[0], h));
            MNK_HIP(hipStreamWaitEvent(sp, B.ev[0], 0));
            if (su != nullptr) MNK_HIP(hipStreamWaitEvent(su, B.ev[0], 0));
            int r = mnk_launch_pchain_multi(g.data() + r0, k, sp, nullptr, B.pcsys.p, fronts.data(), afs.data());
            if (r) return r;
            if (ntasks1 > 0) {
                const int bulk_wgs = mnk_ctx_bulk_wgs(c0, chain_cus_for(k), 3);
                r = mnk::launch_dag_bulk(su, ldl, hin[0], insts_dev, B.tasks.p, B.ntasks, ntile, B.qctr.p, mnk_ls_dag_spin_limit(l0),
                                         std::min(B.ntasks, bulk_wgs), nullptr, nullptr);
                if (r) return r;
                MNK_HIP(hipEventRecord(B.ev[2], su));
                MNK_HIP(hipStreamWaitEvent(h, B.ev[2], 0));
            }
            MNK_HIP(hipEventRecord(B.ev[1], sp));
            MNK_HIP(hipStreamWaitEvent(h, B.ev[1], 0));
            if (su != nullptr) MNK_HIP(hipStreamWaitEvent(su, B.ev[1], 0));
            if (su != nullptr) MNK_HIP(hipStreamWaitEvent(sp, B.ev[2], 0));
            if (batch_aux) {
                r = mnk_ls_invert_blocks_batch(h, ldl, aux_dev, k, Np);
                if (r) return r;
                r = mnk_ls_finish_info_batch(h, aux_dev, k, ldl ? (l0->N >= 4096 ? 1024 : 256) : 64);
                if (r) return r;
                for (int i = 0; i < k; ++i) {
                    mnk_ls* ls = g[r0 + i];
                    ls->inv_done = nsc;
                    if (!ls->ev_info) MNK_HIP(hipEventCreateWithFlags(&ls->ev_info, hipEventDisableTiming));
                    MNK_HIP(hipEventRecord(ls->ev_info, h));
                    ls->ev_info_recorded = true;
                }
                return 0;
            }
            hipStream_t inv_s[3] = {h, sp, su != nullptr ? su : sp};
            for (int i = 0; i < k; ++i) {
                mnk_ls* ls = g[r0 + i];
                hipStream_t si = inv_s[i % 3];
                r = mnk_ls_invert_blocks(ls, si, 0, nsc);
                if (r) return r;
                ls->inv_done = nsc;
                r = mnk_ls_launch_finish_info(ls, si);
                if (r) return r;
            }
            MNK_HIP(hipEventRecord(B.ev[1], sp));
            MNK_HIP(hipStreamWaitEvent(h, B.ev[1], 0));
            if (su != nullptr) {
                MNK_HIP(hipEventRecord(B.ev[2], su));
                MNK_HIP(hipStreamWaitEvent(h, B.ev[2], 0));
            }
            return 0;
        };
        rc = body();
        rc = mnk_persist_end(c0, h, rc);
        if (rc) return rc;
    }
    MNK_HIP(hipEventRecord(l0->ev_defer, h));
    for (mnk_ls* ls : g) {
        if (ls->ctx->stream != h) MNK_HIP(hipStreamWaitEvent(ls->ctx->stream, l0->ev_defer, 0));
        batch_mark_done(ls);
        int r = mnk_ls_prefill_spare(ls);
        if (r) return r;
    }
    return 0;
}

static int batch_flush() {
    std::vector<mnk_ls*> pend;
    pend.swap(t_batch.pend);
    int rc_all = 0;
    while (!pend.empty()) {
        mnk_ls* l0 = pend.front();
// ... 30 lines not shown

bool mnk_ls_pending_elsewhere(const mnk_ls* ls) {
    return ls->deferred && std::find(t_batch.pend.begin(), t_batch.pend.end(), ls) == t_batch.pend.end();
}

int mnk_ls_sync_deferred_fact(mnk_ls* ls) {
    if (!ls->deferred) return 0;
    if (std::find(t_batch.pend.begin(), t_batch.pend.end(), ls) == t_batch.pend.end()) {
        set_error("a factorize! call of this solver is pending in a batch that another thread opened (mnk_factorize_batch_end must come first)");
        return -1;
    }
    return batch_flush();
}

extern "C" int mnk_factorize_batch_begin(void) {
    ++t_batch.depth;
    t_batch.active = true;
    return 0;
}

extern "C" int mnk_factorize_batch_end(void) {
    if (t_batch.depth <= 0) { set_error("mnk_factorize_batch_end: no batch is open on this thread"); return -1; }
    if (--t_batch.depth > 0) return 0;
    t_batch.active = false;
    return batch_flush();
}

extern "C" int mnk_debug_dag_tasks(int ntile, int chunk, int band_tiles, int js2, int taper0, int* out, int cap, int* first_phase) {
    if (ntile <= 0 || chunk <= 0 || band_tiles <= 0 || taper0 <= 0) return -1;
    std::vector<int> h;
    const int n1 = mnk::dag_build_tasks(ntile, chunk, band_tiles, js2, h, taper0, nullptr);
    const int n = (int)(h.size() / 4);
    if (first_phase != nullptr) *first_phase = n1;
    if (out != nullptr)
        for (int i = 0; i < std::min(n, cap) * 4; ++i) out[i] = h[i];
    return n;
}

extern "C" int mnk_debug_dag_merged_tasks(int ntile, int chunk, int band_tiles, int js2, int taper0, int fill, int ninst, int period,
                                          int* out, int cap) {
    if (ntile <= 0 || chunk <= 0 || band_tiles <= 0 || taper0 <= 0 || ninst <= 0 || period < 0) return -1;
    std::vector<int> h, ready, merged;
    int n1 = mnk::dag_build_tasks(ntile, chunk, band_tiles, js2, h, taper0, &ready);
    if (fill) n1 = mnk::dag_add_fill_tasks(ntile, h, ready, n1);
    mnk::dag_merge_tasks(h, ready, ninst, period, merged);
    const int n = (int)(merged.size() / 4);
    if (out != nullptr)
        for (int i = 0; i < std::min(n, cap) * 4; ++i) out[i] = merged[i];
    return n;
}

extern "C" int mnk_debug_dag_deal(int ntile, int chunk, int band_tiles, int js2, int taper0, int fill, int ninst, int period, int nq,
                                  int gang, int* tasks_out, int* order, int cap, int* off, int* first_phase) {
    if (ntile <= 0 || chunk <= 0 || band_tiles <= 0 || taper0 <= 0 || ninst <= 0 || period < 0 || nq <= 0 || nq > 64 || gang == 0) return -1;
    std::vector<int> h, ready;
    int n1 = mnk::dag_build_tasks(ntile, chunk, band_tiles, js2, h, taper0, &ready);
    if (fill) n1 = mnk::dag_add_fill_tasks(ntile, h, ready, n1);
    if (ninst > 1) {
        std::vector<int> merged, mready, pos(ninst, 0);
        mnk::dag_merge_tasks(h, ready, ninst, period, merged);
        for (size_t t = 0; t < merged.size() / 4; ++t) { const int i = merged[4 * t + 1] >> 16; mready.push_back(i * period + ready[pos[i]++]); }
        h.swap(merged);
        ready.swap(mready);
        n1 = (int)ready.size();
    }
    const int n = (int)ready.size();
    if (first_phase != nullptr) *first_phase = n1;
    const int part[3] = {0, n1, n};
    int written = 0;
    for (int ph = 0; ph < 2; ++ph) {
        std::vector<int> ord, o;
        mnk::dag_deal_tasks(h, ready, part[ph], part[ph + 1], nq, gang, ord, o);
        for (int x = 0; x <= nq; ++x)
            if (off != nullptr) off[ph * (nq + 1) + x] = part[ph] + o[x];
        for (int v : ord) {
            if (order != nullptr && written < cap) order[written] = v;
            ++written;
        }
    }
    if (tasks_out != nullptr)
        for (int i = 0; i < std::min(n, cap) * 4; ++i) tasks_out[i] = h[i];
    return n;
}
```

madnlp.jl_amd/csrc/factor.hip:

```cpp
#include <atomic>
#include <type_traits>
#include <atomic>
#include <cfloat>
#include <chrono>
#include <cmath>
#include <cstdlib>

#include "ls.h"
#include "leaf64.h"

namespace mnk {

template <bool LDL, int NS>
__device__ __forceinline__ void trsm64_mfma_body(double* __restrict__ F, int64_t ld, int64_t j0, int64_t Np,
                                                 const double* __restrict__ Dblk, const double* __restrict__ inv16,
                                                 const double* __restrict__ dinv, double* __restrict__ W, int64_t ldw,
                                                 int64_t wcol, const int* __restrict__ info,
                                                 unsigned long long* __restrict__ vmax) {
    if (*info != 0) return;
    const int lane = threadIdx.x & 63, wave = threadIdx.x >> 6;
    const int l15 = lane & 15, l4 = lane >> 4;
    const int64_t r0 = j0 + 64 + ((int64_t)blockIdx.x * 4 + wave) * (16 * NS);
    if (r0 >= Np) return;
    double Ln[6][4];
// ... 912 lines not shown
        }
    }
    const bool ldl = ls->algo == MNK_LDL;
    const int epoch16 = ls->epoch * 16;
    double* V = ldl ? ls->vfull.p : nullptr;
    if (ldl)
        hipLaunchKernelGGL(pchain_kernel<true>, dim3(strips), dim3(256), PC_LDS_BYTES, sp, ls->fact.p, ls->ld, ls->Np, ls->dblk.p,
                           ls->inv16.p, ls->dvec.p, ls->dinv.p, V, ls->info_dev.p, ls->pivot_tol, ls->flag_p.p, epoch16,
                           ls->debug_pp_missing, dag, js_begin, js_end);
    else
        hipLaunchKernelGGL(pchain_kernel<false>, dim3(strips), dim3(256), PC_LDS_BYTES, sp, ls->fact.p, ls->ld, ls->Np, ls->dblk.p,
                           ls->inv16.p, ls->dvec.p, ls->dinv.p, V, ls->info_dev.p, ls->pivot_tol, ls->flag_p.p, epoch16,
                           ls->debug_pp_missing, dag, js_begin, js_end);
    MNK_HIP(hipGetLastError());
    return 0;
}

static int run_factorization_body(mnk_ls* ls);

size_t mnk_pchain_sys_bytes() { return sizeof(mnk::PcSys); }
void mnk_pchain_fill_sys(mnk_ls* ls, void* rec_host, int* front, const int* af) {
    const bool ldl = ls->algo == MNK_LDL;
    *static_cast<mnk::PcSys*>(rec_host) = mnk::PcSys{ls->fact.p, ls->ld, ls->Np, ls->dblk.p, ls->inv16.p, ls->dvec.p, ls->dinv.p,
                                                       ldl ? ls->vfull.p : nullptr, ls->info_dev.p, ls->pivot_tol, ls->flag_p.p,
                                                       ls->epoch * 16, front, af, (int)(ls->Np / 128), mnk_ls_dag_spin_limit(ls),
                                                       mnk_ls_growth_word(ls)};
}

int mnk_launch_pchain_multi(mnk_ls* const* v, int n, hipStream_t sp, hipStream_t fill_stream, void* table, int* const* front,
                            const int* const* af) {
    {
        static std::atomic<uint64_t> attr_devs{0};
        int dev = 0;
        MNK_HIP(hipGetDevice(&dev));
        if (!(attr_devs.load(std::memory_order_relaxed) >> (dev & 63) & 1)) {
            MNK_HIP(hipFuncSetAttribute((const void*)pchain_multi_kernel<true>, hipFuncAttributeMaxDynamicSharedMemorySize, PC_LDS_BYTES));
            MNK_HIP(hipFuncSetAttribute((const void*)pchain_multi_kernel<false>, hipFuncAttributeMaxDynamicSharedMemorySize, PC_LDS_BYTES));
            attr_devs.fetch_or(1ull << (dev & 63), std::memory_order_relaxed);
        }
    }
    mnk::PcSys* dst = static_cast<mnk::PcSys*>(table);
    const bool ldl = v[0]->algo == MNK_LDL;
    const int strips = (int)(v[0]->Np / NBI);
    for (int i = 0; i < n && fill_stream != nullptr; ++i) {
        mnk_ls* ls = v[i];
        mnk::PcSys rec{ls->fact.p, ls->ld, ls->Np, ls->dblk.p, ls->inv16.p, ls->dvec.p, ls->dinv.p, ldl ? ls->vfull.p : nullptr,
                       ls->info_dev.p, ls->pivot_tol, ls->flag_p.p, ls->epoch * 16, front[i], af[i], (int)(ls->Np / 128),
                       mnk_ls_dag_spin_limit(ls), mnk_ls_growth_word(ls)};
        hipLaunchKernelGGL(pc_set_sys_kernel, dim3(1), dim3(1), 0, fill_stream, rec, dst + i);
    }
    MNK_HIP(hipGetLastError());
    if (ldl)
        hipLaunchKernelGGL(pchain_multi_kernel<true>, dim3((unsigned)(n * strips)), dim3(256), PC_LDS_BYTES, sp, dst, strips);
    else
        hipLaunchKernelGGL(pchain_multi_kernel<false>, dim3((unsigned)(n * strips)), dim3(256), PC_LDS_BYTES, sp, dst, strips);
    MNK_HIP(hipGetLastError());
    return 0;
}

int mnk_ls_run_factorization(mnk_ls* ls) {
    if (ls->algo == MNK_QR) return mnk_qr_factor(ls);
    if (ls->algo == MNK_LU) return mnk_lu_factor(ls);
    if (ls->algo == MNK_EVD) return mnk_evd_factor(ls);
    mnk_ctx* ctx = ls->ctx;
    hipStream_t s = ctx->stream;
    const int64_t Np = ls->Np;
    if (ls->panel_algo >= 4 && !ls->flag_p.p) {
        if (ls->flag_p.alloc(Np / NBI + 1)) return -2;
        MNK_HIP(hipMemsetAsync(ls->flag_p.p, 0, (Np / NBI + 1) * sizeof(int), s));
    }
    ++ls->epoch;
    ls->inv_done = 0;
    ls->factor_invalid = false;
    ls->t_fact_launch_ms = mnk_host_ms();
    {
        const int want = (ls->early_reject && ls->accept_only_pd && ls->algo == MNK_LDL && ls->src_persistent) ? 1 : 0;
        if (want != ls->reject_on_device) {
            MNK_HIP(hipMemsetAsync(ls->info_dev.p + 2, want, sizeof(int), s));
            ls->reject_on_device = want;
        }
    }
    ls->algo_now = ls->panel_algo;
    ls->env_used = false;
    const int64_t min_rows = mnk_batch_active() ? std::min<int64_t>(ls->dag_min_rows, 256) : ls->dag_min_rows;
    if (ls->algo_now == 5 && (ctx->dag_cus < ls->dag_band || !ls->lookahead || Np < min_rows || Np > ls->dag_max_rows)) ls->algo_now = 4;
    if (ls->algo_now == 5 && ctx->sp_dag == nullptr && mnk_ctx_ensure_dag(ctx) != 0) { (void)hipGetLastError(); ls->algo_now = 4; }
    if (ls->algo_now == 5 && ctx->sp_dag == nullptr) ls->algo_now = 4;
    ++ls->fact_count;
    if (ls->pp_blocked && ls->fact_count >= ls->pp_retry_at) ls->pp_blocked = false;
    if (ls->algo_now >= 4 && ls->pp_blocked) ls->algo_now = 1;
    if (ls->algo_now == 5 && mnk_ls_dag_prepare(ls) != 0) ls->algo_now = 4;
    if (ls->algo_now == 5 && ls->dag_js2 < (Np + 255) / 256) {
        if (mnk_ctx_ensure_dag2(ctx) != 0) (void)hipGetLastError();
        if (ctx->sp_dag2 == nullptr) ls->algo_now = 4;
    }
    if (ls->algo_now == 5 && mnk_batch_defer(ls)) return 0;
    return mnk_ls_run_factorization_now(ls);
}

int mnk_ls_run_factorization_now(mnk_ls* ls) {
    mnk_ctx* ctx = ls->ctx;
    hipStream_t s = ctx->stream;
    const bool persistent = ls->algo_now >= 4;
    if (persistent) {
        int rc0 = mnk_persist_begin(ctx, s);
        if (rc0) return rc0;
    }
    const int rc_run = run_factorization_body(ls);
    return persistent ? mnk_persist_end(ctx, s, rc_run) : rc_run;
}

static int run_factorization_body(mnk_ls* ls) {
    mnk_ctx* ctx = ls->ctx;
    hipStream_t s = ctx->stream;
    const int64_t Np = ls->Np, ld = ls->ld;
    const bool ldl = ls->algo == MNK_LDL;
    double* F = ls->fact.p;
    const int64_t NBO = mnk_ls_effective_nbo(ls);
    if (ls->algo_now != 5) MNK_HIP(hipMemsetAsync(ls->info_dev.p, 0, 2 * sizeof(int), s));
    std::vector<int64_t> bnd{0};
    for (int64_t pos = 0; pos < Np;) {
        const bool tail = ls->lookahead && NBO < Np && ls->tail_rows > 0 && Np - pos <= ls->tail_rows && ls->tail_nbo < NBO;
        pos = std::min<int64_t>(pos + (tail ? ls->tail_nbo : NBO), Np);
        bnd.push_back(pos);
    }
    const int64_t npanel = (int64_t)bnd.size() - 1;
    const bool la = ls->lookahead && npanel > 1;

    if (ls->algo_now == 5) {
        int rc = mnk_ls_run_factorization_dag(ls);
        if (rc) return rc;
    } else if (!la) {
        for (int64_t ko = 0; ko < Np; ko += NBO) {
            const int64_t kend = std::min<int64_t>(ko + NBO, Np);
            int rc = factor_outer_panel(ls, s, ko, kend, ls->wbuf[0].p);
            if (rc) return rc;
            const int64_t Mt = Np - kend;
            if (Mt > 0) {
                const double* Wsrc = ldl ? ls->wbuf[0].p + kend : F + kend + ko * ld;
                rc = launch_gemm_nt(s, 2, Mt, Mt, kend - ko, Wsrc, ldl ? ls->ldw : ld, F + kend + ko * ld, ld,
                                    F + kend + kend * ld, ld, nullptr, nullptr, 0, ls->info_dev.p);
                if (rc) return rc;
            }
        }
    } else {
        { int rc_s = mnk_ctx_ensure_panel_streams(ctx); if (rc_s) return rc_s; }
        hipStream_t sp = ctx->sp, su = ctx->su;
        if ((int64_t)ctx->ev_panel.size() < npanel + 1) {
            const size_t old = ctx->ev_panel.size();
            ctx->ev_panel.resize(npanel + 1);
            ctx->ev_next.resize(npanel + 1);
            ctx->ev_next2.resize(npanel + 1);
            ctx->ev_bdone.resize(npanel + 1);
            for (size_t e = old; e < ctx->ev_panel.size(); ++e) {
                MNK_HIP(hipEventCreateWithFlags(&ctx->ev_panel[e], hipEventDisableTiming));
                MNK_HIP(hipEventCreateWithFlags(&ctx->ev_next[e], hipEventDisableTiming));
                MNK_HIP(hipEventCreateWithFlags(&ctx->ev_next2[e], hipEventDisableTiming));
                MNK_HIP(hipEventCreateWithFlags(&ctx->ev_bdone[e], hipEventDisableTiming));
            }
        }
        const int pcus = ctx->panel_cus;
        const int ucus = pcus > 0 ? ctx->num_cu - pcus : ctx->num_cu;
        const bool share = ls->share != 0;
        if (share) {
            if (ls->tile_ctr.n < 8 * ((size_t)npanel + 1)) {
                int rc0 = ls->tile_ctr.alloc(8 * ((size_t)npanel + 1));
// ... 309 lines not shown
```

madnlp.jl_amd/csrc/gemm_tile.h:

```cpp
#pragma once
#include "common.h"

namespace mnk {

typedef double v4f64 __attribute__((ext_vector_type(4)));
typedef double v2f64 __attribute__((ext_vector_type(2)));

constexpr int BK = 16;
constexpr bool tile_big(int wm, int wn, int wt) { return wm == 2 && wn == 2 && wt == 4; }
constexpr int tile_bk(int wm, int wn, int wt) { return tile_big(wm, wn, wt) ? 8 : BK; }
constexpr int tile_occ(int wm, int wn, int wt) { return tile_big(wm, wn, wt) ? 3 : 2; }

template <int MODE>
__device__ __forceinline__ void decode_tile(int logical, int ntm, int nc, int sw, int& tm, int& tn) {
    if (MODE == 2 || MODE == 4) {
        const double bq = 2.0 * ntm + 1.0;
        int c = (int)((bq - sqrt(bq * bq - 8.0 * (double)logical)) * 0.5);
        if (c < 0) c = 0;
        while (c > 0 && c * ntm - c * (c - 1) / 2 > logical) --c;
        while ((c + 1) * ntm - (c + 1) * c / 2 <= logical) ++c;
        if (sw <= 1) {
            tn = c;
            tm = tn + (logical - (c * ntm - c * (c - 1) / 2));
            return;
        }
        const int r0 = (c / sw) * sw;
        const int W = nc - r0 < sw ? nc - r0 : sw;
        int rem = logical - (r0 * ntm - r0 * (r0 - 1) / 2);
        const int tri = W * (W + 1) / 2;
        if (rem < tri) {
            int i = (int)((sqrt(8.0 * (double)rem + 1.0) - 1.0) * 0.5);
            while (i > 0 && i * (i + 1) / 2 > rem) --i;
            while ((i + 1) * (i + 2) / 2 <= rem) ++i;
            tm = r0 + i;
            tn = r0 + (rem - i * (i + 1) / 2);
        } else {
            rem -= tri;
            tm = r0 + W + rem / W;
            tn = r0 + rem % W;
        }
    } else {
        tm = logical % ntm;
        tn = logical / ntm;
    }
}

struct GemmNoGate {
    __device__ __forceinline__ bool operator()(int) const { return true; }
};
template <int WM, int WN, int WT, int DBG, int BKT, class GATE = GemmNoGate>
__device__ __forceinline__ bool gemm_nt_mainloop(v4f64 (&acc)[WT][WT], const double* __restrict__ Ag, int64_t lda,
                                                 const double* __restrict__ Bg, int64_t ldb, int nk, char* smem_raw,
                                                 int tid, GATE gate = GATE()) {
    constexpr int NT = 64 * WM * WN;
    constexpr int WS = 16 * WT;
    constexpr int BM = WS * WM, BN = WS * WN;
    constexpr int LDA_S = BM + 16, LDB_S = BN + 16;
    constexpr int APIECES = (BM / 2) * BKT / NT;
    constexpr int BPIECES = (BN / 2) * BKT / NT;
    static_assert(APIECES >= 1 && BPIECES >= 1, "tile too small for the thread count");

    double* As = reinterpret_cast<double*>(smem_raw);
    double* Bs = As + 2 * BKT * LDA_S;

    const int lane = tid & 63;
    const int wave = tid >> 6;
    const int wm = wave % WM, wn = wave / WM;
    const int l15 = lane & 15, l4 = lane >> 4;

    v2f64 ra[APIECES], rb[BPIECES];

    auto gload = [&](int kt) {
        const int64_t k0 = (int64_t)kt * BKT;
#pragma unroll
        for (int q = 0; q < APIECES; ++q) {
            int p = tid + NT * q;
            int k = p / (BM / 2), r = (p % (BM / 2)) * 2;
            ra[q] = *reinterpret_cast<const v2f64*>(Ag + r + (k0 + k) * lda);
        }
#pragma unroll
        for (int q = 0; q < BPIECES; ++q) {
            int p = tid + NT * q;
            int k = p / (BN / 2), r = (p % (BN / 2)) * 2;
            rb[q] = *reinterpret_cast<const v2f64*>(Bg + r + (k0 + k) * ldb);
        }
    };
    auto sstore = [&](int buf) {
        double* as = As + buf * BKT * LDA_S;
        double* bs = Bs + buf * BKT * LDB_S;
#pragma unroll
        for (int q = 0; q < APIECES; ++q) {
            int p = tid + NT * q;
            int k = p / (BM / 2), r = (p % (BM / 2)) * 2;
            *reinterpret_cast<v2f64*>(as + k * LDA_S + r) = ra[q];
        }
#pragma unroll
        for (int q = 0; q < BPIECES; ++q) {
            int p = tid + NT * q;
            int k = p / (BN / 2), r = (p % (BN / 2)) * 2;
            *reinterpret_cast<v2f64*>(bs + k * LDB_S + r) = rb[q];
        }
    };

    constexpr bool DMA = BM == 128 && BN == 128 && (DBG == 0 || DBG == 1 || DBG == 4);
    constexpr int NW = NT / 64;
    auto gl_lds = [&](int kt, int buf) {
        const int64_t k0 = (int64_t)kt * BKT;
        double* as = As + buf * BKT * LDA_S;
        double* bs = Bs + buf * BKT * LDB_S;
#pragma unroll
        for (int i = 0; i < BKT / NW; ++i) {
            const int k = wave * (BKT / NW) + i;
            __builtin_amdgcn_global_load_lds((const __attribute__((address_space(1))) void*)(Ag + (k0 + k) * lda + lane * 2),
                                             (__attribute__((address_space(3))) void*)(as + k * LDA_S), 16, 0, 0);
            __builtin_amdgcn_global_load_lds((const __attribute__((address_space(1))) void*)(Bg + (k0 + k) * ldb + lane * 2),
                                             (__attribute__((address_space(3))) void*)(bs + k * LDB_S), 16, 0, 0);
        }
    };
    if (nk <= 0) return true;
    if (!gate(0)) return false;
    if (DMA) {
        gl_lds(0, 0);
        asm volatile("s_waitcnt vmcnt(0)" ::: "memory");
    } else {
        gload(0);
        sstore(0);
    }
    __syncthreads();

    for (int kt = 0; kt < nk; ++kt) {
        const int cur = kt & 1;
        if (kt + 1 < nk && !gate(kt + 1)) return false;
        if (DMA) {
            if (kt + 1 < nk) gl_lds(kt + 1, cur ^ 1);
        } else if (DBG != 3 && kt + 1 < nk) {
            gload(kt + 1);
        }
        const double* as = As + cur * BKT * LDA_S + wm * WS + l15;
        const double* bs = Bs + cur * BKT * LDB_S + wn * WS + l15;
#pragma unroll
        for (int kk = 0; kk < BKT / 4; ++kk) {
            double af[WT], bf[WT];
#pragma unroll
            for (int i = 0; i < WT; ++i) {
                af[i] = as[(kk * 4 + l4) * LDA_S + i * 16];
                bf[i] = bs[(kk * 4 + l4) * LDB_S + i * 16];
            }
#pragma unroll
            for (int ni = 0; ni < WT; ++ni)
#pragma unroll
                for (int mi = 0; mi < WT; ++mi)
                    acc[ni][mi] = __builtin_amdgcn_mfma_f64_16x16x4f64(bf[ni], af[mi], acc[ni][mi], 0, 0, 0);
        }
        if (DMA) {
            asm volatile("s_waitcnt vmcnt(0)" ::: "memory");
            __syncthreads();
        } else {
            if (DBG != 3 && kt + 1 < nk) sstore(cur ^ 1);
            if (DBG != 2 && DBG != 3) __syncthreads();
        }
    }
    return true;
}

constexpr int TILE3_ROWS = 8 * 128 + 16 * 4;
constexpr int TILE3_LDS_BYTES = 3 * 2 * TILE3_ROWS * 8;
__device__ __forceinline__ constexpr int tile3_row(int k) { return k * 128 + 16 * ((k + 1) >> 1); }
template <int MI = 4, int NI = 4, bool NEG = false, class GATE = GemmNoGate>
__device__ __forceinline__ bool gemm_nt_mainloop3(v4f64 (&acc)[NI][MI], const double* __restrict__ Ag, int64_t lda,
                                                  const double* __restrict__ Bg, int64_t ldb, int nk, char* smem_raw, int tid,
                                                  GATE gate = GATE()) {
    static_assert(MI * NI == 16 && 128 % (16 * MI) == 0, "four waves cover the 128x128 tile");
    constexpr int BKT = 8, WSM = 16 * MI, WSN = 16 * NI, WAVES_M = 128 / WSM;
    double* Ls = reinterpret_cast<double*>(smem_raw);
    const int lane = tid & 63;
    const int wave = tid >> 6;
    const int wm = wave % WAVES_M, wn = wave / WAVES_M;
    const int l15 = lane & 15, l4 = lane >> 4;
    auto gl_lds = [&](int kt, int buf) {
        const int64_t k0 = (int64_t)kt * BKT;
        double* as = Ls + buf * 2 * TILE3_ROWS;
        double* bs = as + TILE3_ROWS;
#pragma unroll
        for (int i = 0; i < 2; ++i) {
            const int k = wave * 2 + i;
            const int off = tile3_row(k);
            __builtin_amdgcn_global_load_lds((const __attribute__((address_space(1))) void*)(Ag + (k0 + k) * lda + lane * 2),
                                             (__attribute__((address_space(3))) void*)(as + off), 16, 0, 0);
            __builtin_amdgcn_global_load_lds((const __attribute__((address_space(1))) void*)(Bg + (k0 + k) * ldb + lane * 2),
                                             (__attribute__((address_space(3))) void*)(bs + off), 16, 0, 0);
        }
    };
    if (nk <= 0) return true;
    if (!gate(0)) return false;
    gl_lds(0, 0);
    if (nk > 1) {
        if (!gate(1)) return false;
        gl_lds(1, 1);
        asm volatile("s_waitcnt vmcnt(4)\n\ts_barrier" ::: "memory");
    } else {
        asm volatile("s_waitcnt vmcnt(0)\n\ts_barrier" ::: "memory");
    }
    int cur = 0;
    for (int kt = 0; kt < nk; ++kt) {
        const int nxt2 = cur == 0 ? 2 : cur - 1;
        const bool more = kt + 2 < nk;
        if (more) {
            if (!gate(kt + 2)) return false;
            gl_lds(kt + 2, nxt2);
        }
        const double* as = Ls + cur * 2 * TILE3_ROWS + wm * WSM + l15 + tile3_row(l4);
        const double* bs = Ls + cur * 2 * TILE3_ROWS + TILE3_ROWS + wn * WSN + l15 + tile3_row(l4);
#pragma unroll
        for (int kk = 0; kk < BKT / 4; ++kk) {
            double af[MI];
#pragma unroll
            for (int i = 0; i < MI; ++i) {
                af[i] = as[kk * (4 * 128 + 32) + i * 16];
                if (NEG) af[i] = -af[i];
            }
#pragma unroll
            for (int n0 = 0; n0 < NI; n0 += 4) {
                double bf[4];
#pragma unroll
                for (int i = 0; i < 4; ++i) bf[i] = bs[kk * (4 * 128 + 32) + (n0 + i) * 16];
#pragma unroll
                for (int ni = 0; ni < 4; ++ni)
#pragma unroll
                    for (int mi = 0; mi < MI; ++mi)
                        acc[n0 + ni][mi] = __builtin_amdgcn_mfma_f64_16x16x4f64(bf[ni], af[mi], acc[n0 + ni][mi], 0, 0, 0);
                if (NI > 4) __builtin_amdgcn_sched_barrier(0);
            }
        }
        if (more)
            asm volatile("s_waitcnt vmcnt(4)\n\ts_barrier" ::: "memory");
// ... 128 lines not shown
```

madnlp.jl_amd/csrc/ls.h:

```cpp
#pragma once
#include <algorithm>
#include <functional>
#include <memory>
#include <string>
#include <vector>

#include "common.h"

struct mnk_sc {
    mnk_ctx* ctx = nullptr;
    int64_t n = 0, m = 0, nnzj = 0, nnzh = 0;
    int64_t nnz_jt = 0, nnz_hess = 0, nnz_aug = 0, len_jptr = 0;
    std::vector<int32_t> jt_colptr, jt_rowval, h_colptr, h_rowval, aug_colptr, aug_rowval;
    std::vector<int32_t> tile_env;
    mnk::DevBuf<int32_t> d_tile_env;
    std::vector<int64_t> jt_map, h_map;
    std::vector<int32_t> d_dst, d_src, hp_dst, hp_src, j_dst, j_c, j_k, j_l;
    mnk::DevBuf<int32_t> jt_seg_ptr, jt_seg_src, h_seg_ptr, h_seg_src;
    mnk::DevBuf<int32_t> aug_hptr, aug_hsrc;
    mnk::DevBuf<int32_t> aug_dsrc;
    mnk::DevBuf<int32_t> aug_jptr, aug_jc, aug_jk, aug_jl;
    mnk::DevBuf<int32_t> aug_row, aug_col;
    mnk::DevBuf<int32_t> d_jt_colptr, d_jt_rowval, d_jt_colidx, d_h_colptr, d_h_rowval, d_h_colidx;
    mnk::DevBuf<double> jac_coo, hess_coo, jt_nz, h_nz, aug_nz, diag_buffer, pr_diag, du_diag;
    void* extra = nullptr;
    std::shared_ptr<int> alive = std::make_shared<int>(0);
};

inline std::vector<int32_t> mnk_tile_envelope(int64_t n, const int32_t* row, const int32_t* col, int64_t nnz) {
    std::vector<int32_t> fnz(n);
    for (int64_t i = 0; i < n; ++i) fnz[i] = (int32_t)i;
    for (int64_t k = 0; k < nnz; ++k)
        if (row[k] >= 0 && row[k] < n && col[k] < fnz[row[k]]) fnz[row[k]] = col[k];
    const int64_t ntile = (n + 127) / 128;
    std::vector<int32_t> env(ntile);
    for (int64_t I = 0; I < ntile; ++I) {
        int32_t f = (int32_t)(128 * I);
        for (int64_t i = 128 * I; i < std::min<int64_t>(n, 128 * I + 128); ++i) f = std::min(f, fnz[i]);
        env[I] = f / 128;
    }
    return env;
}

struct mnk_dc {
    mnk_ctx* ctx = nullptr;
    int condensed = 1;
    bool mirror_pending = false;
    int64_t n = 0, m = 0, ns = 0, n_eq = 0, order = 0;
    std::vector<int64_t> ind_ineq, ind_eq;
    mnk::DevBuf<int64_t> d_ind_ineq, d_ind_eq;
    mnk::DevBuf<double> hess, jac, aug, pr_diag, du_diag, diag_buffer;
    mnk::DevBuf<double> jis;
    int64_t ld_jis = 0, kpad = 0, npad = 0;
    void* extra = nullptr;
    void* qn = nullptr;
    std::shared_ptr<int> alive = std::make_shared<int>(0);
};
void mnk_dc_qn_release(mnk_dc* dc);

constexpr int EVD_BLOCK = 32;

struct mnk_ls {
    mnk_ctx* ctx = nullptr;
    int64_t N = 0, Np = 0, ld = 0, ldw = 0, nbo = 512;
    bool nbo_auto = true;
    int algo = MNK_LDL;
    double pivot_tol = 0.0;
    int lookahead = 1;
    int share = 1;
    int small_tiles = 400;
    int split_a = 2;
    int64_t single_rows = 2560;
    int64_t tail_rows = 4096;
    int64_t tail_nbo = 256;
    int small_tiles_mid = 1000;
    mnk::DevBuf<int> tile_ctr;
    mnk::DevBuf<double> fact, wbuf[2], linv, dblk, inv16, linv256, linv256t, dvec, dinv, xwork;
    mnk::DevBuf<double> fact_spare;
    hipEvent_t ev_spare = nullptr, ev_free = nullptr;
    bool spare_zeroed = false, spare_pending = false;
    int prefill = 1;
    int64_t prefill_max_rows = 24576;
    int epoch = 0;
    mnk::DevBuf<int> flag_p;
    int panel0_whole = 1;
    int algo_now = 1;
    bool pp_blocked = false;
    int64_t fact_count = 0, pp_retry_at = 0, pp_backoff = 16;
    int pp_fallbacks = 0;
    int last_timeout_site = 0;
    double stall_ms_total = 0.0;
    double t_fact_launch_ms = 0.0;
    int64_t pp_fuse_rows = 4096;
    int64_t own_cols = 128;
    mnk::DevBuf<int> dag_tasks;
    int dag_ntasks = 0, dag_ntasks1 = 0, dag_js2 = 0;
    std::vector<int> dag_host_tasks, dag_host_ready;
    int dag_fill = 1;
    bool dag_has_fill = false;
    bool dag_filled = false;
    int batch_period = 0;
    hipEvent_t ev_info = nullptr;
    bool ev_info_recorded = false;
    hipEvent_t ev_defer = nullptr;
    bool deferred = false;
    int dag_xcd_queues = 1;
    int dag_gang = 4;
    int dag_nq[2] = {0, 0};
    mnk::DevBuf<int> dag_qoff;
    mnk::DevBuf<int> dag_qheads;
    mnk::DevBuf<int> dag_flags;
    mnk::DevBuf<double> vfull;
    mnk::DevBuf<unsigned long long> dag_trace;
    bool dag_trace_on = false;
    int64_t inv_done = 0;
    int dag_band = 16;
    int dag_taper0 = 2;
    long dag_spin_limit = 0;
    int dag_chunk = 64;
    int64_t dag_min_rows = 1280;
    int64_t dag_deep_rows = 5376;
    int envelope = 1;
    const int32_t* env_dev = nullptr;
    std::vector<int32_t> env_host;
    mnk::DevBuf<int32_t> env_own;
    mnk::DevBuf<int> env_word;
    bool env_used = false;
    bool env_armed = false;
    int64_t dag_max_rows = 30720;
    int panel_algo = 5;
    int persistent_solve = 1;
    int solve512 = 0;
    int64_t solve512_min_rows = 4096;
    int dag_chain_inline = 1;
    std::vector<std::string> env_keys;
    int dag_js2_override = -1;
    int linv_mfma = 1;
    mnk::DevBuf<double> linv512, linv512t, linv512tmp;
    int pub_next = 0;
    bool pub_clean[2] = {false, false};
    int* solve_abort = nullptr;
    long ps_spin_limit = 6000000;
    int debug_pp_missing = -1;
    int debug_ps_missing = -1;
    mnk::DevBuf<unsigned long long> solve_trace;
    mnk::DevBuf<int> info_dev;
    mnk::DevBuf<unsigned long long> inertia_dev;
    unsigned long long* pin = nullptr;
    unsigned long long* pin_dev = nullptr;
    bool bk_requested = false;
    int bk_fallback = 1;
    int early_reject = 0;
    int reject_on_device = -1;
    bool src_persistent = false;
    bool factor_invalid = false;
    int64_t early_rejects = 0, early_reject_col = -1, early_reject_redone = 0;
    int probe = 1;
    mnk_ls* probe_ls = nullptr;
    int64_t probe_order = 0;
    int64_t probe_hint_col = -1;
    int probe_since_hint = 1 << 20;
    bool probe_last_rejected = false;
    int64_t probe_hits = 0, probe_misses = 0;
    int accept_only_pd = 0;
    double bk_growth_tol = 64.0, bk_growth_tol_qd = 1e8;
    double last_growth = 0.0;
    int64_t last_sign_changes = 0;
    mnk::DevBuf<unsigned long long> amax_dev;
    bool bk_active = false;
    int bk_count = 0;
    std::function<int()> retransfer;
    mnk::DevBuf<int> bk_perm, bk_ptype;
    mnk::DevBuf<double> bk_doff, bk_dcoup, bk_work;
    mnk::DevBuf<char> bk_state;
    mnk::DevBuf<double> bk_wv, bk_tmp;
    mnk::DevBuf<unsigned long long> bk_msg;
    mnk::DevBuf<int> bk_aux;
    int bk_panel_wgs = 0;
    int bk_max_wgs = 0;
    long bk_spin_limit = 1L << 21;
    int debug_bk_missing = -1;
    bool bk_multi_last = false, bk_mw_blocked = false;
    int bk_mw_fallbacks = 0;
    bool factorized = false, info_valid = false;
    int dag_debug = 0;
    mnk::DevBuf<int> dag_dbg;
    std::vector<int> dbg_flags, dbg_chain;
    bool spare_by_dag = false;
    int info = 0;
    int64_t npos = 0, nzero = 0, nneg = 0;
    mnk::DevBuf<double> qr_v, qr_t, qr_w, qr_p;
    mnk::DevBuf<double> lu_ut, lu_p;
    mnk::DevBuf<int> lu_cand, lu_ipiv, lu_perm, lu_info;
    mnk::DevBuf<double> evd_a, evd_v, evd_rt, evd_colsum, evd_lam, evd_part;
    mnk::DevBuf<int> evd_ident, evd_rank;
    int evd_sweep_cap = 60;
    int evd_sweeps = 0;
};

int64_t mnk_ls_effective_nbo(const mnk_ls* ls);
int mnk_qr_alloc(mnk_ls* ls);
int mnk_qr_factor(mnk_ls* ls);
int mnk_qr_solve(mnk_ls* ls, double* x, int64_t nrhs, int64_t ldx, int loc);
int mnk_launch_tril_to_full(hipStream_t s, double* F, int64_t ld, int64_t N, int64_t Np);
int mnk_launch_upper_bsolve(hipStream_t s, const double* F, int64_t ld, int64_t Np, double* y, double* x);
int mnk_lu_alloc(mnk_ls* ls);
int mnk_lu_factor(mnk_ls* ls);
int mnk_lu_fetch_info(mnk_ls* ls);
// ... 54 lines not shown
```

madnlp.jl_amd/csrc/ls.hip:

```cpp
#include <cstdarg>
#include <cstdlib>
#include <atomic>
#include <map>
#include <mutex>

#include <cfloat>
#include "ls.h"

namespace mnk {

static thread_local std::string g_err;
void set_error(const char* fmt, ...) {
    char buf[1024];
    va_list ap;
    va_start(ap, fmt);
    vsnprintf(buf, sizeof(buf), fmt, ap);
    va_end(ap);
    g_err = buf;
}

__global__ __launch_bounds__(256) void fill_lower_kernel(double* __restrict__ F, int64_t ld, int64_t N, int64_t Np) {
    const int64_t col = blockIdx.x;
    const int64_t first = (col / PAD) * PAD;
    const int64_t r = first + ((int64_t)blockIdx.y * 256 + threadIdx.x) * 2;
// ... 538 lines not shown
    rc |= ls->linv.alloc((size_t)(ls->Np / NBI) * NBI * NBI);
    rc |= ls->dblk.alloc((size_t)(ls->Np / NBI) * NBI * NBI);
    rc |= ls->inv16.alloc((size_t)(ls->Np / NBI) * 1024);
    rc |= ls->linv256.alloc((size_t)((ls->Np + 255) / 256) * 65536);
    rc |= ls->linv256t.alloc((size_t)((ls->Np + 255) / 256) * 65536);
    rc |= ls->dvec.alloc(ls->Np);
    rc |= ls->dinv.alloc(ls->Np);
    rc |= ls->xwork.alloc(10 * ls->Np);
    if (hipHostMalloc((void**)&ls->solve_abort, sizeof(int), hipHostMallocDefault) != hipSuccess) {
        (void)hipGetLastError();
        ls->solve_abort = nullptr;
        rc |= -2;
    } else {
        *ls->solve_abort = 0;
    }
    if (hipHostMalloc((void**)&ls->pin, 8 * sizeof(unsigned long long), hipHostMallocMapped) != hipSuccess ||
        hipHostGetDevicePointer((void**)&ls->pin_dev, ls->pin, 0) != hipSuccess) {
        (void)hipGetLastError();
        rc |= -2;
    }
    rc |= ls->info_dev.alloc(4);
    rc |= ls->inertia_dev.alloc(3);
    if (algo == MNK_QR) {
        rc |= mnk_qr_alloc(ls);
        ls->prefill = 0;
    }
    if (algo == MNK_LU) {
        rc |= mnk_lu_alloc(ls);
        ls->prefill = 0;
    }
    if (algo == MNK_EVD) {
        rc |= mnk_evd_alloc(ls);
        ls->prefill = 0;
    }
    if (rc) { delete ls; return -2; }
    MNK_HIP(hipMemsetAsync(ls->fact.p, 0, ((size_t)ls->ld * ls->Np + SLACK) * sizeof(double), ctx->stream));
    mnk_ctx_child_added(ctx);
    *out = ls;
    return 0;
}

int mnk_ls_destroy(mnk_ls* ls) {
    if (!ls) return 0;
    (void)hipSetDevice(ls->ctx->device);
    if (mnk_ls_pending_elsewhere(ls)) {
        set_error("mnk_ls_destroy: a factorize! call of this solver is pending in a batch that another thread opened "
                  "(that thread's mnk_factorize_batch_end must come first); the solver was NOT destroyed");
        return -1;
    }
    (void)mnk_ls_sync_deferred(ls);
    (void)mnk::stream_wait(ls->ctx->stream);
    if (ls->probe_ls) { (void)mnk_ls_destroy(ls->probe_ls); ls->probe_ls = nullptr; }
    mnk::LaunchLock lock;
    mnk::quiesce_persistent();
    if (ls->solve_abort) (void)hipHostFree(ls->solve_abort);
    if (ls->pin) (void)hipHostFree(ls->pin);
    if (ls->ctx->s_fill) (void)mnk::stream_wait(ls->ctx->s_fill);
    if (ls->ev_spare) (void)hipEventDestroy(ls->ev_spare);
    if (ls->ev_free) (void)hipEventDestroy(ls->ev_free);
    if (ls->ev_defer) (void)hipEventDestroy(ls->ev_defer);
    if (ls->ev_info) (void)hipEventDestroy(ls->ev_info);
    mnk_ctx* ctx = ls->ctx;
    delete ls;
    mnk_ctx_child_gone(ctx);
    return 0;
}

int mnk_ls_set_option(mnk_ls* ls, const char* key, double value) {
    MNK_REQUIRE(ls && key, "mnk_ls_set_option: NULL argument");
    { int rc_d = mnk_ls_sync_deferred(ls); if (rc_d) return rc_d; }
    for (const std::string& k : ls->env_keys)
        if (k == key) {
            static std::mutex warn_mutex;
            static std::vector<std::string> warned;
            std::lock_guard<std::mutex> lock(warn_mutex);
            if (std::find(warned.begin(), warned.end(), k) == warned.end()) {
                warned.push_back(k);
                fprintf(stderr, "madnlp_hip: set_option('%s', %g) ignored: the option is pinned by MNK_OPTIONS / MNK_PANEL_ALGO / "
                                "MNK_PERSISTENT_SOLVE for this process (query: get_stat(\"pinned:%s\"))\n", key, value, key);
            }
            return 0;
        }
    if (!strcmp(key, "pivot_tol")) { ls->pivot_tol = value; return 0; }
    if (!strcmp(key, "envelope")) { ls->envelope = value != 0.0; return 0; }
    if (!strcmp(key, "split_a")) { ls->split_a = (int)value; return 0; }
    if (!strcmp(key, "tail_rows")) { ls->tail_rows = (int64_t)value; return 0; }
    if (!strcmp(key, "tail_nbo")) { ls->tail_nbo = (int64_t)value; return 0; }
    if (!strcmp(key, "own_cols")) { ls->own_cols = std::max<long>(64, (long)value / 64 * 64); return 0; }
    if (!strcmp(key, "panel0_whole")) { ls->panel0_whole = (int)value; return 0; }
    if (!strcmp(key, "dag_js2")) { ls->dag_js2_override = (int)value; return 0; }
    if (!strcmp(key, "outer_block")) {
        int64_t v = (int64_t)value;
        MNK_REQUIRE(v == 0 || (v >= NBI && v % NBI == 0), "outer_block must be 0 (by size) or a positive multiple of 64");
        ls->nbo_auto = v == 0;
        if (v > 0) ls->nbo = v;
        ls->wbuf[0].release();
        ls->wbuf[1].release();
        return 0;
    }
    if (!strcmp(key, "solve512")) { ls->solve512 = value != 0; return 0; }
    if (!strcmp(key, "solve512_min_rows")) { ls->solve512_min_rows = (int64_t)value; return 0; }
    if (!strcmp(key, "linv_mfma")) { ls->linv_mfma = value != 0.0; return 0; }
    if (!strcmp(key, "dag_chain_inline")) { ls->dag_chain_inline = value != 0.0; return 0; }
    if (!strcmp(key, "prefill")) { ls->prefill = value != 0; return 0; }
    if (!strcmp(key, "prefill_max_rows")) { ls->prefill_max_rows = (int64_t)value; return 0; }
    if (!strcmp(key, "single_rows")) {
        ls->single_rows = (int64_t)value;
        ls->wbuf[0].release();
        ls->wbuf[1].release();
        return 0;
    }
    if (!strcmp(key, "lookahead")) { ls->lookahead = value != 0.0; return 0; }
    if (!strcmp(key, "share")) { ls->share = (int)value; return 0; }
    if (!strcmp(key, "small_tiles")) { ls->small_tiles = (int)value; return 0; }
    if (!strcmp(key, "small_tiles_mid")) { ls->small_tiles_mid = (int)value; return 0; }
    if (!strcmp(key, "panel_algo")) {
        MNK_REQUIRE((int)value == 1 || (int)value == 4 || (int)value == 5, "panel_algo must be 1, 4 or 5");
        ls->panel_algo = (int)value;
        return 0;
    }
    if (!strcmp(key, "pp_fuse_rows")) { ls->pp_fuse_rows = (int64_t)value; return 0; }
    if (!strcmp(key, "dag_min_rows")) { ls->dag_min_rows = (int64_t)value; return 0; }
    if (!strcmp(key, "dag_taper0")) {
        MNK_REQUIRE(value >= 1.0 && value <= 16.0, "dag_taper0 must be in 1..16");
        ls->dag_taper0 = (int)value;
        ls->dag_tasks.release();
        return 0;
    }
    if (!strcmp(key, "dag_chunk")) {
        MNK_REQUIRE(value >= 1.0 && value <= 64.0, "dag_chunk must be in 1..64");
        ls->dag_chunk = (int)value;
        ls->dag_tasks.release();
        return 0;
    }
    if (!strcmp(key, "dag_band")) {
        MNK_REQUIRE(value >= 8.0 && value <= 64.0 && (int)value % 4 == 0 && (double)(int)value == value, "dag_band must be a multiple of 4 in 8..64");
        ls->dag_band = (int)value;
        ls->dag_tasks.release();
        return 0;
    }
    if (!strcmp(key, "dag_spin_limit")) {
        MNK_REQUIRE(value >= 1024.0, "dag_spin_limit must be at least 1024");
        ls->dag_spin_limit = (long)value;
        return 0;
    }
    if (!strcmp(key, "dag_fill")) { ls->dag_fill = value != 0.0; ls->dag_tasks.release(); return 0; }
    if (!strcmp(key, "dag_xcd_queues")) { ls->dag_xcd_queues = value != 0.0; ls->dag_tasks.release(); return 0; }
    if (!strcmp(key, "dag_gang")) {
        MNK_REQUIRE(value <= 64.0 && value != 0.0 && (double)(int)value == value, "dag_gang must be an integer in 1..64 (or negative)");
        ls->dag_gang = (int)value;
        ls->dag_tasks.release();
        return 0;
    }
    if (!strcmp(key, "batch_period")) { ls->batch_period = (int)value; return 0; }
    if (!strcmp(key, "dag_trace")) { ls->dag_trace_on = value != 0.0; return 0; }
    if (!strcmp(key, "dag_max_rows")) { ls->dag_max_rows = (int64_t)value; return 0; }
    if (!strcmp(key, "dag_deep_rows")) { ls->dag_deep_rows = (int64_t)value; ls->dag_tasks.release(); return 0; }
    if (!strcmp(key, "bk_fallback")) { ls->bk_fallback = (int)value; return 0; }
    if (!strcmp(key, "bk_panel_wgs")) {
        MNK_REQUIRE(value == 0.0 || value == 1.0, "bk_panel_wgs must be 0 or 1");
        ls->bk_panel_wgs = (int)value;
        return 0;
    }
    if (!strcmp(key, "accept_only_pd")) { ls->accept_only_pd = value != 0; return 0; }
    if (!strcmp(key, "probe")) { ls->probe = value != 0; return 0; }
    if (!strcmp(key, "early_reject")) { ls->early_reject = value != 0; return 0; }
// ... 35 lines not shown
    if (!strcmp(key, "debug_pp_missing")) { ls->debug_pp_missing = (int)value; return 0; }
    if (!strcmp(key, "debug_ps_missing")) { ls->debug_ps_missing = (int)value; return 0; }
    if (!strcmp(key, "solve_trace")) {
        if (value != 0.0) {
            int rc = ls->solve_trace.alloc((size_t)(ls->Np / 64) * 8);
            if (rc) return rc;
            MNK_HIP(hipMemset(ls->solve_trace.p, 0, (size_t)(ls->Np / 64) * 8 * sizeof(unsigned long long)));
        } else {
            ls->solve_trace.release();
        }
        return 0;
    }
    set_error("mnk_ls_set_option: unknown option '%s'", key);
    return -1;
}

static int ensure_wbuf(mnk_ls* ls) {
    if (ls->algo != MNK_LDL || ls->wbuf[0].p) return 0;
    const size_t cnt = (size_t)ls->ldw * std::min<int64_t>(mnk_ls_effective_nbo(ls), ls->Np) + SLACK;
    int rc = ls->wbuf[0].alloc(cnt);
    if (!rc && mnk_ls_effective_nbo(ls) < ls->Np) rc = ls->wbuf[1].alloc(cnt);
    return rc;
}

static unsigned long long* amax_word(mnk_ls* ls) {
    if (!(ls->bk_requested && ls->bk_fallback && ls->algo == MNK_LDL)) return nullptr;
    if (!ls->amax_dev.p && ls->amax_dev.alloc(AMAX_WORDS)) return nullptr;
    (void)hipMemsetAsync(ls->amax_dev.p, 0, AMAX_WORDS * sizeof(unsigned long long), ls->ctx->stream);
    return ls->amax_dev.p;
}

static int prepare_fill(mnk_ls* ls) {
    mnk_ctx* ctx = ls->ctx;
    hipStream_t s = ctx->stream;
    dim3 grid((unsigned)ls->Np, (unsigned)((ls->Np / 2 + 255) / 256));
    bool pre = ls->prefill && ls->Np <= ls->prefill_max_rows;
    if (pre && !ls->fact_spare.p) {
        if (ls->fact_spare.alloc(ls->fact.n) != 0) { (void)hipGetLastError(); ls->prefill = 0; pre = false; }
        if (pre && !ctx->s_fill && hipStreamCreateWithFlags(&ctx->s_fill, hipStreamNonBlocking) != hipSuccess) { ls->prefill = 0; pre = false; }
        if (pre && (hipEventCreateWithFlags(&ls->ev_spare, hipEventDisableTiming) != hipSuccess ||
                    hipEventCreateWithFlags(&ls->ev_free, hipEventDisableTiming) != hipSuccess)) { ls->prefill = 0; pre = false; }
        if (pre) MNK_HIP(hipMemsetAsync(ls->fact_spare.p, 0, ls->fact_spare.n * sizeof(double), s));
    }
    if (pre && ls->spare_zeroed && ls->spare_by_dag && !ls->info_valid) {
        ls->spare_zeroed = false;
        ls->spare_by_dag = false;
    }
    if (pre && ls->spare_zeroed) {
        std::swap(ls->fact.p, ls->fact_spare.p);
        MNK_HIP(hipStreamWaitEvent(s, ls->ev_spare, 0));
        ls->spare_zeroed = false;
    } else {
        hipLaunchKernelGGL(fill_lower_kernel, grid, dim3(256), 0, s, ls->fact.p, ls->ld, ls->N, ls->Np);
    }
    ls->spare_pending = pre;
    MNK_HIP(hipGetLastError());
    return 0;
}

}
int mnk_ls_prefill_spare(mnk_ls* ls) {
    if (!ls->spare_pending) return 0;
    ls->spare_pending = false;
    if (ls->dag_filled) {
        ls->dag_filled = false;
        MNK_HIP(hipEventRecord(ls->ev_spare, ls->ctx->stream));
        ls->spare_zeroed = true;
        ls->spare_by_dag = true;
        return 0;
    }
    ls->spare_by_dag = false;
    mnk_ctx* ctx = ls->ctx;
    dim3 grid((unsigned)ls->Np, (unsigned)((ls->Np / 2 + 255) / 256));
    MNK_HIP(hipEventRecord(ls->ev_free, ctx->stream));
    MNK_HIP(hipStreamWaitEvent(ctx->s_fill, ls->ev_free, 0));
    hipLaunchKernelGGL(fill_lower_kernel, grid, dim3(256), 0, ctx->s_fill, ls->fact_spare.p, ls->ld, ls->N, ls->Np);
    MNK_HIP(hipGetLastError());
    MNK_HIP(hipEventRecord(ls->ev_spare, ctx->s_fill));
    ls->spare_zeroed = true;
    return 0;
}
extern "C" {

static int* set_envelope(mnk_ls* ls, const int32_t* env_dev, const std::vector<int32_t>& env_host) {
    ls->env_dev = nullptr;
    if (!ls->envelope || env_dev == nullptr || ls->algo == MNK_QR || ls->algo == MNK_LU || ls->algo == MNK_EVD) return nullptr;
    if (!ls->env_word.p) {
        if (ls->env_word.alloc(2) || hipMemsetAsync(ls->env_word.p, 0, 2 * sizeof(int), ls->ctx->stream) != hipSuccess) {
            (void)hipGetLastError();
            ls->env_word.release();
            return nullptr;
        }
    }
    if (ls->env_armed && hipMemsetAsync(ls->env_word.p, 0, sizeof(int), ls->ctx->stream) != hipSuccess) { (void)hipGetLastError(); return nullptr; }
    ls->env_armed = true;
    ls->env_dev = env_dev;
    ls->env_host.assign(env_host.begin(), env_host.begin() + std::min<size_t>(env_host.size(), (size_t)(ls->Np / 128)));
    return ls->env_word.p;
}

static int transfer_sc(mnk_ls* ls, mnk_sc* sc) {
    int rc = prepare_fill(ls);
    if (rc) return rc;
    const int64_t nnz = sc->nnz_aug;
    int* nonfinite = set_envelope(ls, sc->d_tile_env.p, sc->tile_env);
    hipLaunchKernelGGL(scatter_csc_kernel, dim3((unsigned)((nnz + 255) / 256)), dim3(256), 0, ls->ctx->stream,
                       ls->fact.p, ls->ld, sc->aug_row.p, sc->aug_col.p, sc->aug_nz.p, nnz, amax_word(ls),
                       ls->N < sc->n ? (int32_t)ls->N : INT32_MAX, nonfinite);
    MNK_HIP(hipGetLastError());
    return 0;
}

static int probe_leading_block(mnk_ls* ls, mnk_sc* sc, bool* rejected) {
    *rejected = false;
    if (!(ls->probe && ls->early_reject && ls->accept_only_pd && ls->algo == MNK_LDL && ls->N == sc->n && !mnk_batch_active())) return 0;
    if (ls->probe_last_rejected || ls->probe_hint_col < 0 || ls->probe_since_hint > 3) return 0;
    const int64_t m = (ls->probe_hint_col + 256) / 256 * 256;
    if (m < 512 || 2 * m > ls->N) return 0;
    if (ls->probe_ls == nullptr || ls->probe_order != m) {
        if (ls->probe_ls) { (void)mnk_ls_destroy(ls->probe_ls); ls->probe_ls = nullptr; }
        mnk_ls* child = nullptr;
        if (mnk_ls_create(ls->ctx, m, ls->algo, &child) != 0) { (void)hipGetLastError(); return 0; }
        child->probe = 0;
        child->accept_only_pd = 1;
        child->early_reject = 1;
        ls->probe_ls = child;
        ls->probe_order = m;
    }
    mnk_ls* c = ls->probe_ls;
    c->pivot_tol = ls->pivot_tol;
    c->envelope = ls->envelope;
    if (c->dag_xcd_queues != ls->dag_xcd_queues || c->dag_gang != ls->dag_gang) {
        c->dag_xcd_queues = ls->dag_xcd_queues;
        c->dag_gang = ls->dag_gang;
        c->dag_tasks.release();
    }
    int rc = mnk_ls_factorize_sc_async(c, sc);
    if (!rc) rc = mnk_ls_fetch_info(c);
    if (rc) return rc;
    if (c->npos == m && c->nzero == 0 && c->nneg == 0) { ++ls->probe_misses; return 0; }
    ++ls->probe_hits;
    ++ls->early_rejects;
    ls->early_reject_col = c->factor_invalid ? c->early_reject_col : m - 1;
    ls->info = 1;
    ls->npos = c->npos;
    ls->nzero = c->nzero;
    ls->nneg = ls->N - ls->npos - ls->nzero;
    ls->factor_invalid = true;
    ls->info_valid = true;
    ls->factorized = true;
    ls->bk_active = false;
    ls->probe_last_rejected = true;
    if (2 * ls->early_reject_col < ls->N) { ls->probe_hint_col = ls->early_reject_col; ls->probe_since_hint = 0; }
    *rejected = true;
    return 0;
}

int mnk_ls_factorize_sc_async(mnk_ls* ls, mnk_sc* sc) {
    MNK_REQUIRE(ls && sc && sc->ctx, "mnk_ls_factorize_sc: NULL argument or host-only handle");
    MNK_REQUIRE(sc->n >= ls->N, "mnk_ls_factorize_sc: the solver's order exceeds the KKT system's");
    MNK_HIP(hipSetDevice(ls->ctx->device));
    { int rc_d = mnk_ls_sync_deferred(ls); if (rc_d) return rc_d; }
    int rc = ensure_wbuf(ls);
    if (rc) return rc;
    bool probe_rejected = false;
    rc = probe_leading_block(ls, sc, &probe_rejected);
    if (rc) return rc;
    if (!probe_rejected) {
        rc = transfer_sc(ls, sc);
        if (rc) return rc;
    }
    ls->src_persistent = true;
    ls->retransfer = [ls, sc, w = std::weak_ptr<int>(sc->alive)]() {
        if (w.expired()) {
            set_error("factorize!: the KKT handle of the last factorize! call was destroyed before its inertia was fetched; the "
                      "matrix cannot be transferred again for the fall-back tier");
            return -5;
        }
        return transfer_sc(ls, sc);
    };
    if (probe_rejected) return 0;
    return mnk_ls_run_factorization(ls);
}

static int transfer_dense(mnk_ls* ls, const double* Adev, int64_t lda) {
    ls->env_dev = nullptr;
    dim3 grid((unsigned)ls->Np, (unsigned)((ls->Np + 1023) / 1024));
    hipLaunchKernelGGL(copy_lower_kernel, grid, dim3(256), 0, ls->ctx->stream, ls->fact.p, ls->ld, Adev, lda,
                       ls->N, ls->Np, amax_word(ls));
    MNK_HIP(hipGetLastError());
    return 0;
}

static int factorize_dense_dev(mnk_ls* ls, const double* Adev, int64_t lda, bool src_persistent = false) {
    int rc = ensure_wbuf(ls);
    if (rc) return rc;
    rc = transfer_dense(ls, Adev, lda);
    if (rc) return rc;
    ls->src_persistent = src_persistent;
    ls->retransfer = [ls, Adev, lda]() { return transfer_dense(ls, Adev, lda); };
    return mnk_ls_run_factorization(ls);
}

}
int mnk_ls_factorize_dense_dev_async(mnk_ls* ls, const double* Adev, int64_t lda) {
    MNK_REQUIRE(ls && Adev && lda >= ls->N, "mnk_ls_factorize_dense_dev_async: bad argument");
    MNK_HIP(hipSetDevice(ls->ctx->device));
    { int rc_d = mnk_ls_sync_deferred(ls); if (rc_d) return rc_d; }
    return factorize_dense_dev(ls, Adev, lda);
}
extern "C" {

int mnk_ls_factorize_dc_async(mnk_ls* ls, mnk_dc* dc) {
    MNK_REQUIRE(ls && dc, "mnk_ls_factorize_dc: NULL argument");
    MNK_REQUIRE(dc->order == ls->N, "mnk_ls_factorize_dc: order mismatch");
    MNK_HIP(hipSetDevice(ls->ctx->device));
    { int rc_d = mnk_ls_sync_deferred(ls); if (rc_d) return rc_d; }
    int rc = factorize_dense_dev(ls, dc->aug.p, round_up(dc->order, PAD), true);
    ls->retransfer = [ls, dc, w = std::weak_ptr<int>(dc->alive)]() {
        if (w.expired()) {
            set_error("factorize!: the KKT handle of the last factorize! call was destroyed before its inertia was fetched; the "
                      "matrix cannot be transferred again for the fall-back tier");
            return -5;
        }
        return transfer_dense(ls, dc->aug.p, round_up(dc->order, PAD));
    };
    return rc;
}

static int finish_info(mnk_ls* ls, int* info) {
    int rc = mnk_ls_fetch_info(ls);
    if (rc) return rc;
    if (info) *info = ls->info;
    return 0;
}

int mnk_ls_factorize_sc(mnk_ls* ls, mnk_sc* sc, int* info) {
    int rc = mnk_ls_factorize_sc_async(ls, sc);
    return rc ? rc : finish_info(ls, info);
}

int mnk_ls_factorize_dc(mnk_ls* ls, mnk_dc* dc, int* info) {
    int rc = mnk_ls_factorize_dc_async(ls, dc);
    return rc ? rc : finish_info(ls, info);
}

int mnk_ls_factorize_dense(mnk_ls* ls, const double* A, int64_t lda, int loc, int* info) {
    MNK_REQUIRE(ls && A, "mnk_ls_factorize_dense: NULL argument");
    MNK_REQUIRE(lda >= ls->N, "mnk_ls_factorize_dense: lda < N");
    MNK_HIP(hipSetDevice(ls->ctx->device));
    { int rc_d = mnk_ls_sync_deferred(ls); if (rc_d) return rc_d; }
    int rc;
    if (loc == MNK_DEVICE) {
        rc = factorize_dense_dev(ls, A, lda);
    } else {
        DevBuf<double> tmp;
        rc = tmp.alloc((size_t)ls->N * ls->N);
        if (rc) return rc;
        MNK_HIP(mnk::h2d_copy_2d(tmp.p, ls->N * sizeof(double), A, lda * sizeof(double), ls->N * sizeof(double), ls->N,
                                 ls->ctx->stream));
        rc = factorize_dense_dev(ls, tmp.p, ls->N);
        MNK_HIP(mnk::stream_wait(ls->ctx->stream));
        if (!rc) rc = finish_info(ls, info);
        ls->retransfer = nullptr;
        return rc;
    }
    rc = rc ? rc : finish_info(ls, info);
    ls->retransfer = nullptr;
    return rc;
}

int mnk_ls_factorize_csc(mnk_ls* ls, const int32_t* colptr, const int32_t* rowval, const double* nzval,
                         int index_base, int* info) {
    MNK_REQUIRE(ls && colptr && rowval && nzval, "mnk_ls_factorize_csc: NULL argument");
    MNK_HIP(hipSetDevice(ls->ctx->device));
    { int rc_d = mnk_ls_sync_deferred(ls); if (rc_d) return rc_d; }
    const int64_t N = ls->N;
    const int64_t nnz = colptr[N] - index_base;
    std::vector<int32_t> row(nnz), col(nnz);
    for (int64_t c = 0; c < N; ++c)
        for (int64_t k = colptr[c] - index_base; k < colptr[c + 1] - index_base; ++k) {
            row[k] = rowval[k] - index_base;
            col[k] = (int32_t)c;
            MNK_REQUIRE(row[k] >= c && row[k] < N, "mnk_ls_factorize_csc: matrix must be lower triangular");
        }
    DevBuf<int32_t> drow, dcol;
    DevBuf<double> dnz;
    std::vector<double> nzv(nzval, nzval + nnz);
    int rc = drow.upload(row, ls->ctx->stream);
    rc |= dcol.upload(col, ls->ctx->stream);
    rc |= dnz.upload(nzv, ls->ctx->stream);
    const std::vector<int32_t> env = ls->envelope ? mnk_tile_envelope(N, row.data(), col.data(), nnz) : std::vector<int32_t>();
    if (ls->envelope) rc |= ls->env_own.upload(env, ls->ctx->stream);
    if (rc) return -2;
    rc = ensure_wbuf(ls);
    if (rc) return rc;
    auto transfer = [ls, nnz, &drow, &dcol, &dnz, &env]() -> int {
        int r = prepare_fill(ls);
        if (r) return r;
        int* nonfinite = set_envelope(ls, env.empty() ? nullptr : ls->env_own.p, env);
        if (nnz > 0)
            hipLaunchKernelGGL(scatter_csc_kernel, dim3((unsigned)((nnz + 255) / 256)), dim3(256), 0, ls->ctx->stream,
                               ls->fact.p, ls->ld, drow.p, dcol.p, dnz.p, nnz, amax_word(ls), INT32_MAX, nonfinite);
        MNK_HIP(hipGetLastError());
        return 0;
    };
    rc = transfer();
    if (rc) return rc;
    ls->src_persistent = false;
    ls->retransfer = transfer;
    rc = mnk_ls_run_factorization(ls);
    if (!rc) {
        MNK_HIP(mnk::stream_wait(ls->ctx->stream));
        rc = finish_info(ls, info);
    }
    ls->retransfer = nullptr;
    return rc;
}

int mnk_debug_tile_env_csc(int64_t n, const int32_t* colptr, const int32_t* rowval, int index_base, int32_t* out, int cap) {
    if (n <= 0 || colptr == nullptr || rowval == nullptr || cap < 0) return -1;
    const int64_t nnz = colptr[n] - index_base;
    std::vector<int32_t> row(nnz), col(nnz);
    for (int64_t c = 0; c < n; ++c)
        for (int64_t k = colptr[c] - index_base; k < colptr[c + 1] - index_base; ++k) { row[k] = rowval[k] - index_base; col[k] = (int32_t)c; }
    const std::vector<int32_t> env = mnk_tile_envelope(n, row.data(), col.data(), nnz);
    if (out != nullptr)
        for (int I = 0; I < std::min((int)env.size(), cap); ++I) out[I] = env[I];
    return (int)env.size();
}

int mnk_ls_inertia(mnk_ls* ls, int64_t* num_pos, int64_t* num_zero, int64_t* num_neg) {
    MNK_REQUIRE(ls, "mnk_ls_inertia: NULL argument");
    MNK_REQUIRE(ls->algo != MNK_QR, "mnk_ls_inertia: a QR factorization reveals no inertia (is_inertia is false for QR)");
    MNK_REQUIRE(ls->algo != MNK_LU, "mnk_ls_inertia: an LU factorization reveals no inertia (is_inertia is false for LU)");
    { int rc_d = mnk_ls_sync_deferred(ls); if (rc_d) return rc_d; }
    MNK_REQUIRE(ls->factorized, "mnk_ls_inertia: factorize first");
    MNK_HIP(hipSetDevice(ls->ctx->device));
    int rc = mnk_ls_fetch_info(ls);
    if (rc) return rc;
    if (num_pos) *num_pos = ls->npos;
    if (num_zero) *num_zero = ls->nzero;
    if (num_neg) *num_neg = ls->nneg;
    return 0;
}

int mnk_ls_check_solve(mnk_ls* ls) {
    MNK_REQUIRE(ls, "mnk_ls_check_solve: NULL argument");
    MNK_HIP(hipSetDevice(ls->ctx->device));
    { int rc_q = mnk_solve_sync_deferred(ls); if (rc_q) return rc_q; }
    MNK_HIP(mnk::stream_wait(ls->ctx->stream));
    if (mnk_ls_take_solve_abort(ls)) {
        set_error("mnk_ls_check_solve: a persistent solve on device-resident data gave up waiting for a peer workgroup "
                  "(device oversubscribed by another process?); its result is invalid -- solve again "
                  "(persistent_solve is now off for this solver)");
        return -3;
    }
    return 0;
}

static int ensure_complete_factor(mnk_ls* ls, const char* who) {
    if (ls->reject_on_device == 1) { int rc_i = mnk_ls_fetch_info(ls); if (rc_i) return rc_i; }
    if (!ls->factor_invalid) return 0;
    { static const bool peek = getenv("MNK_DBG_NO_REDO") != nullptr; if (peek) return 0; }
    if (!ls->retransfer) {
        set_error("%s: the last factorization was stopped at its first non-positive pivot (early_reject) and its source is gone: "
                  "there is no factor", who);
        return -1;
    }
    const int keep = ls->early_reject;
    ls->early_reject = 0;
    int rc = ls->retransfer();
    if (!rc) rc = mnk_ls_run_factorization(ls);
    if (!rc) rc = mnk_ls_fetch_info(ls);
    ls->early_reject = keep;
    ++ls->early_reject_redone;
    return rc;
}

int mnk_ls_solve(mnk_ls* ls, double* x, int64_t nrhs, int64_t ldx, int loc) {
    MNK_REQUIRE(ls && x, "mnk_ls_solve: NULL argument");
    { int rc_d = mnk_ls_sync_deferred_fact(ls); if (rc_d) return rc_d; }
    MNK_REQUIRE(ls->factorized, "mnk_ls_solve: factorize first");
    MNK_HIP(hipSetDevice(ls->ctx->device));
    { int rc_f = ensure_complete_factor(ls, "mnk_ls_solve"); if (rc_f) return rc_f; }
    MNK_REQUIRE(nrhs >= 1 && ldx >= ls->N, "mnk_ls_solve: bad nrhs/ldx");
    MNK_HIP(hipSetDevice(ls->ctx->device));
    if (ls->algo == MNK_QR) return mnk_qr_solve(ls, x, nrhs, ldx, loc);
    if (ls->algo == MNK_LU) return mnk_lu_solve(ls, x, nrhs, ldx, loc);
    if (ls->algo == MNK_EVD) return mnk_evd_solve(ls, x, nrhs, ldx, loc);
    if (ls->solve_abort && *ls->solve_abort != 0) {
        *ls->solve_abort = 0;
        ls->persistent_solve = 0;
        ls->pub_clean[0] = ls->pub_clean[1] = false;
        set_error("mnk_ls_solve: an earlier persistent solve on device-resident data gave up waiting for a peer "
                  "workgroup (device oversubscribed by another process?); its result is invalid -- refactorize/solve "
                  "again (persistent_solve is now off for this solver)");
        return -3;
    }
    hipStream_t s = ls->ctx->stream;
    const int64_t N = ls->N, Np = ls->Np;
    double* w = ls->xwork.p;
    for (int64_t k = 0; k < nrhs; ++k) {
        double* xk = x + k * ldx;
        if (loc == MNK_DEVICE) {
            if (nrhs == 1 && mnk_solve_defer(ls, xk)) continue;
            int rc = mnk_solve_sync_deferred(ls);
            if (rc) return rc;
            rc = mnk_ls_run_solve(ls, w, xk);
            if (rc) return rc;
            continue;
        }
// ... 69 lines not shown
    MNK_REQUIRE(ls && out && ls->solve_trace.p, "mnk_ls_debug_solve_trace: tracing is off (option solve_trace)");
    MNK_HIP(hipSetDevice(ls->ctx->device));
    MNK_HIP(mnk::stream_wait(ls->ctx->stream));
    const int64_t cnt = std::min<int64_t>(n, (ls->Np / 64) * 8);
    MNK_HIP(mnk::d2h_copy(out, ls->solve_trace.p, cnt * sizeof(unsigned long long), ls->ctx->stream));
    return 0;
}

int mnk_ls_get_factor(mnk_ls* ls, double* L, double* D, int loc) {
    MNK_REQUIRE(ls && L, "mnk_ls_get_factor: NULL argument");
    { int rc_d = mnk_ls_sync_deferred(ls); if (rc_d) return rc_d; }
    MNK_REQUIRE(ls->factorized, "mnk_ls_get_factor: factorize first");
    { int rc_f = ensure_complete_factor(ls, "mnk_ls_get_factor"); if (rc_f) return rc_f; }
    MNK_HIP(hipSetDevice(ls->ctx->device));
    hipStream_t s = ls->ctx->stream;
    if (loc == MNK_DEVICE) {
        MNK_HIP(hipMemcpy2DAsync(L, ls->N * sizeof(double), ls->fact.p, ls->ld * sizeof(double), ls->N * sizeof(double), ls->N,
                                 hipMemcpyDeviceToDevice, s));
        if (D) MNK_HIP(hipMemcpyAsync(D, ls->dvec.p, ls->N * sizeof(double), hipMemcpyDeviceToDevice, s));
        MNK_HIP(mnk::stream_wait(s));
    } else {
        MNK_HIP(mnk::d2h_copy_2d(L, ls->N * sizeof(double), ls->fact.p, ls->ld * sizeof(double), ls->N * sizeof(double), ls->N, s));
        if (D) MNK_HIP(mnk::d2h_copy(D, ls->dvec.p, ls->N * sizeof(double), s));
    }
    return 0;
}

int mnk_ls_get_stat(mnk_ls* ls, const char* key, double* value) {
    MNK_REQUIRE(ls && key && value, "mnk_ls_get_stat: NULL argument");
    MNK_HIP(hipSetDevice(ls->ctx->device));
    { int rc_d = mnk_ls_sync_deferred(ls); if (rc_d) return rc_d; }
    if (ls->factorized) {
        int rc = mnk_ls_fetch_info(ls);
        if (rc) return rc;
    }
    if (!strncmp(key, "pinned:", 7)) {
        *value = std::find(ls->env_keys.begin(), ls->env_keys.end(), std::string(key + 7)) != ls->env_keys.end() ? 1.0 : 0.0;
        return 0;
    }
    if (!strcmp(key, "panel_algo")) { *value = ls->algo_now; return 0; }
    if (!strcmp(key, "pp_fallbacks")) { *value = ls->pp_fallbacks; return 0; }
    if (!strcmp(key, "timeout_site")) { *value = ls->last_timeout_site; return 0; }
    if (!strcmp(key, "probe_hits")) { *value = (double)ls->probe_hits; return 0; }
    if (!strcmp(key, "probe_misses")) { *value = (double)ls->probe_misses; return 0; }
    if (!strcmp(key, "early_rejects")) { *value = (double)ls->early_rejects; return 0; }
    if (!strcmp(key, "early_reject_redone")) { *value = (double)ls->early_reject_redone; return 0; }
    if (!strcmp(key, "early_reject_col")) { *value = (double)ls->early_reject_col; return 0; }
    if (!strcmp(key, "stall_ms_total")) { *value = ls->stall_ms_total; return 0; }
    if (!strcmp(key, "stall_ms_process")) { *value = mnk_process_stall_ms(); return 0; }
    if (!strcmp(key, "growth")) { *value = ls->last_growth; return 0; }
    if (!strcmp(key, "sign_changes")) { *value = (double)ls->last_sign_changes; return 0; }
    if (!strcmp(key, "bk_count")) { *value = ls->bk_count; return 0; }
    if (!strcmp(key, "evd_sweeps")) { *value = ls->evd_sweeps; return 0; }
    if (!strcmp(key, "bk_panel_multi")) { *value = ls->bk_multi_last ? 1.0 : 0.0; return 0; }
    if (!strcmp(key, "bk_mw_fallbacks")) { *value = ls->bk_mw_fallbacks; return 0; }
    if (!strcmp(key, "dag_bulk_wgs")) { *value = ls->ctx->dag_cus > 0 ? mnk_ctx_bulk_wgs(ls->ctx, ls->ctx->dag_cus, 3) : 0; return 0; }
    if (!strcmp(key, "dag_ntasks")) { *value = ls->dag_ntasks; return 0; }
    if (!strcmp(key, "dag_ntasks1")) { *value = ls->dag_ntasks1; return 0; }
    if (!strcmp(key, "dag_js2")) { *value = ls->dag_js2; return 0; }
    if (!strcmp(key, "dag_nq")) { *value = std::max(ls->dag_nq[0], ls->dag_nq[1]); return 0; }
    if (!strcmp(key, "dag_steals")) {
        int st[2] = {0, 0};
        if (ls->dag_qheads.p != nullptr)
            for (int ph = 0; ph < 2; ++ph)
                MNK_HIP(mnk::d2h_copy(&st[ph], ls->dag_qheads.p + ph * mnk::DAG_QHEAD_WORDS + mnk::DAG_NQ * mnk::DAG_QHEAD_STRIDE, sizeof(int), ls->ctx->stream));
        *value = (double)st[0] + (double)st[1];
        return 0;
    }
    if (!strcmp(key, "env_ksteps") || !strcmp(key, "env_ksteps_skipped")) {
        int64_t total = 0, skipped = 0;
        int gate = 1;
        if (ls->env_used && ls->env_word.p) MNK_HIP(mnk::d2h_copy(&gate, ls->env_word.p + 1, sizeof(int), ls->ctx->stream));
        const std::vector<int>& h = ls->dag_host_tasks;
        const int ne = (int)ls->env_host.size();
        for (size_t t = 0; t + 3 < h.size(); t += 4) {
            const int flags = h[t] & 255, I = h[t + 1] & 0xffff, J = h[t + 2], kb = h[t + 3] & 0xffff, ke = h[t + 3] >> 16;
            if (flags & 8) continue;
            total += ke - kb;
            if (!ls->env_used || gate != 0 || I >= ne || J >= ne) continue;
            const int e = std::max(ls->env_host[I], ls->env_host[J]);
            skipped += std::min(ke, std::max(kb, e)) - kb;
        }
        *value = (double)(!strcmp(key, "env_ksteps") ? total : skipped);
        return 0;
    }
    set_error("mnk_ls_get_stat: unknown key '%s'", key);
    return -1;
}

int mnk_ls_bk_info(mnk_ls* ls, int* active, int* count, int32_t* perm, double* doff) {
    MNK_REQUIRE(ls, "mnk_ls_bk_info: NULL argument");
    MNK_HIP(hipSetDevice(ls->ctx->device));
    { int rc_d = mnk_ls_sync_deferred(ls); if (rc_d) return rc_d; }
    if (ls->factorized) {
        int rc = mnk_ls_fetch_info(ls);
        if (rc) return rc;
    }
    if (active) *active = ls->bk_active ? 1 : 0;
    if (count) *count = ls->bk_count;
    if (ls->bk_active && (perm || doff)) {
        hipStream_t s = ls->ctx->stream;
        if (perm) MNK_HIP(mnk::d2h_copy(perm, ls->bk_perm.p, ls->N * sizeof(int32_t), s));
        if (doff) MNK_HIP(mnk::d2h_copy(doff, ls->bk_doff.p, ls->N * sizeof(double), s));
    }
    return 0;
}

int mnk_gemm_nt(mnk_ctx* ctx, int mode, int64_t M, int64_t N, int64_t K, const double* A, int64_t lda,
                const double* B, int64_t ldb, double* C, int64_t ldc) {
    MNK_REQUIRE(ctx && A && B && C, "mnk_gemm_nt: NULL argument");
    MNK_HIP(hipSetDevice(ctx->device));
    return launch_gemm_nt(ctx->stream, mode, M, N, K, A, lda, B, ldb, C, ldc, nullptr, nullptr, 0, nullptr);
}

__global__ void clock_probe_kernel(unsigned long long* out, int iters, double a, double b) {
    double x = (double)threadIdx.x;
    const unsigned long long t0 = wall_clock64();
    for (int i = 0; i < iters; ++i) {
#pragma unroll
        for (int j = 0; j < 16; ++j) x = __builtin_fma(x, a, b);
    }
    const unsigned long long t1 = wall_clock64();
    if (threadIdx.x == 0) out[0] = t1 - t0;
    if (x == 1.2345) out[1] = 1;
}

int mnk_debug_update(mnk_ctx* ctx, int variant, int64_t M, int64_t K, const double* A, int64_t lda, double* C,
                     double* C2, int64_t ldc, int reps, double* ms) {
    MNK_REQUIRE(ctx && A && C && ms, "mnk_debug_update: NULL argument");
    MNK_HIP(hipSetDevice(ctx->device));
    { int rc_s = mnk_ctx_ensure_panel_streams(ctx); if (rc_s) return rc_s; }
    hipStream_t s = ctx->stream, su = ctx->su, sp = ctx->sp;
    MNK_REQUIRE(su && sp, "mnk_debug_update: no look-ahead streams");
    DevBuf<int> ctr;
    int rc = ctr.alloc(8 * (size_t)reps);
    if (rc) return rc;
    MNK_HIP(hipMemsetAsync(ctr.p, 0, 8 * (size_t)reps * sizeof(int), s));
    hipEvent_t e0, e1;
    MNK_HIP(hipEventCreate(&e0));
    MNK_HIP(hipEventCreate(&e1));
    const int pcus = ctx->panel_cus, ucus = ctx->num_cu - pcus;
    MNK_HIP(hipEventRecord(e0, s));
    MNK_HIP(hipEventRecord(ctx->ev_a, s));
    MNK_HIP(hipStreamWaitEvent(su, ctx->ev_a, 0));
    MNK_HIP(hipStreamWaitEvent(sp, ctx->ev_a, 0));
    for (int r = 0; r < reps && !rc; ++r) {
        switch (variant) {
        case 0: rc = launch_gemm_nt(s, 2, M, M, K, A, lda, A, lda, C, ldc, nullptr, nullptr, 0, nullptr); break;
        case 1: rc = launch_gemm_nt_queue(s, M, M, K, A, lda, A, lda, C, ldc, ctr.p + 8 * r, ctx->num_cu, nullptr); break;
        case 2: rc = launch_gemm_nt(su, 2, M, M, K, A, lda, A, lda, C, ldc, nullptr, nullptr, 0, nullptr); break;
        case 3: rc = launch_gemm_nt_queue(su, M, M, K, A, lda, A, lda, C, ldc, ctr.p + 8 * r, ucus, nullptr); break;
        case 4:
            rc = launch_gemm_nt_queue(su, M, M, K, A, lda, A, lda, C, ldc, ctr.p + 8 * r, ucus, nullptr);
            if (!rc) rc = launch_gemm_nt_queue(sp, M, M, K, A, lda, A, lda, C, ldc, ctr.p + 8 * r, pcus, nullptr);
            break;
        case 20: break;
        case 21: rc = launch_gemm_nt(su, 2, M, M, K, A, lda, A, lda, C, ldc, nullptr, nullptr, 0, nullptr); break;
        case 9: rc = launch_gemm_nt_dbg(s, 1, M, M, K, A, lda, A, lda, C, ldc); break;
        case 10: rc = launch_gemm_nt_dbg(su, 1, M, M, K, A, lda, A, lda, C, ldc); break;
        case 11: rc = launch_gemm_nt_dbg(su, 2, M, M, K, A, lda, A, lda, C, ldc); break;
        case 12: rc = launch_gemm_nt_dbg(su, 3, M, M, K, A, lda, A, lda, C, ldc); break;
        case 13: rc = launch_gemm_nt_dbg(su, 5, M, M, K, A, lda, A, lda, C, ldc); break;
        case 14: rc = launch_gemm_nt_dbg(s, 5, M, M, K, A, lda, A, lda, C, ldc); break;
        case 15: rc = launch_gemm_nt_dbg(su, 6, M, M, K, A, lda, A, lda, C, ldc); break;
        case 16: rc = launch_gemm_nt_dbg(s, 6, M, M, K, A, lda, A, lda, C, ldc); break;
        case 6: case 7: case 8: {
// ... 38 lines not shown
```

madnlp.jl_amd/csrc/sparse_kkt.hip:

```cpp
#pragma clang fp contract(off)

#include <algorithm>
#include <numeric>

#include "ls.h"
#include "kkt_vec.h"

namespace mnk {

__global__ void segsum_kernel(double* __restrict__ dst, const double* __restrict__ src,
                              const int32_t* __restrict__ ptr, const int32_t* __restrict__ idx, int64_t nseg) {
    const int64_t s = blockIdx.x * (int64_t)blockDim.x + threadIdx.x;
    if (s >= nseg) return;
    double acc = 0.0;
    for (int32_t k = ptr[s]; k < ptr[s + 1]; ++k) acc += src[idx[k]];
    dst[s] = acc;
}

__global__ void condense_kernel(double* __restrict__ K, const double* __restrict__ Hnz,
                                const double* __restrict__ pr_diag, const double* __restrict__ du,
                                double* __restrict__ Dout, double* __restrict__ pr_keep, double* __restrict__ du_keep,
                                const double* __restrict__ Jt, const int32_t* __restrict__ hptr,
                                const int32_t* __restrict__ hsrc, const int32_t* __restrict__ dsrc,
                                const int32_t* __restrict__ jptr, const int32_t* __restrict__ jc,
// ... 136 lines not shown
        jtI[k] = jac_J[k] - index_base;
        jtJ[k] = jac_I[k] - index_base;
        MNK_REQUIRE(jtI[k] >= 0 && jtI[k] < n && jtJ[k] >= 0 && jtJ[k] < m, "mnk_sc_create: Jacobian index out of range");
    }
    for (int64_t k = 0; k < nnzh; ++k) {
        int32_t i = hess_I[k] - index_base, j = hess_J[k] - index_base;
        MNK_REQUIRE(i >= 0 && i < n && j >= 0 && j < n, "mnk_sc_create: Hessian index out of range");
        if (j > i) std::swap(i, j);
        hI[k] = i;
        hJ[k] = j;
    }
    mnk_sc* sc = new mnk_sc();
    sc->ctx = ctx;
    sc->n = n; sc->m = m; sc->nnzj = nnzj; sc->nnzh = nnzh;
    CscPattern jt = coo_to_csc(n, m, jtI, jtJ);
    CscPattern hh = coo_to_csc(n, n, hI, hJ);
    sc->jt_colptr = jt.colptr; sc->jt_rowval = jt.rowval; sc->jt_map = jt.map;
    sc->h_colptr = hh.colptr; sc->h_rowval = hh.rowval; sc->h_map = hh.map;
    sc->nnz_jt = (int64_t)jt.rowval.size();
    sc->nnz_hess = (int64_t)hh.rowval.size();

    int64_t L = 0;
    for (int64_t c = 0; c < m; ++c) {
        const int64_t k = jt.colptr[c + 1] - jt.colptr[c];
        L += k * (k + 1) / 2;
    }
    const int64_t T = n + sc->nnz_hess + L;
    MNK_REQUIRE(T < (int64_t)2000000000, "mnk_sc_create: symbolic structure exceeds int32 range");
    std::vector<int64_t> key(T);
    std::vector<int8_t> kind(T);
    std::vector<int32_t> sa(T), sb(T), scc(T);
    int64_t t = 0;
    for (int64_t i = 0; i < n; ++i, ++t) { key[t] = i * n + i; kind[t] = -1; sa[t] = (int32_t)i; sb[t] = 0; scc[t] = 0; }
    {
        std::vector<int32_t> hcol = col_index(hh.colptr);
        for (int64_t k = 0; k < sc->nnz_hess; ++k, ++t) {
            key[t] = (int64_t)hcol[k] * n + hh.rowval[k]; kind[t] = 0; sa[t] = (int32_t)k; sb[t] = 0; scc[t] = 0;
        }
    }
    for (int64_t c = 0; c < m; ++c)
        for (int32_t j = jt.colptr[c]; j < jt.colptr[c + 1]; ++j)
            for (int32_t k = j; k < jt.colptr[c + 1]; ++k, ++t) {
                const int64_t c1 = jt.rowval[j], c2 = jt.rowval[k];
                key[t] = c1 * n + c2;
                kind[t] = 1; sa[t] = (int32_t)c; sb[t] = j; scc[t] = k;
            }
    std::vector<int64_t> ord(T);
    std::iota(ord.begin(), ord.end(), 0);
    std::stable_sort(ord.begin(), ord.end(), [&](int64_t a, int64_t b) { return key[a] < key[b]; });

    std::vector<int32_t> a_hptr, a_hsrc, a_dsrc, a_jptr, a_jc, a_jk, a_jl, a_row, a_col;
    sc->aug_colptr.assign(n + 1, 0);
    int64_t slot = -1, prev = -1;
    for (int64_t q = 0; q < T; ++q) {
        const int64_t e = ord[q];
        if (key[e] != prev) {
            prev = key[e];
            ++slot;
            const int32_t col = (int32_t)(key[e] / n), row = (int32_t)(key[e] % n);
            a_row.push_back(row); a_col.push_back(col);
            sc->aug_rowval.push_back(row);
            sc->aug_colptr[col + 1]++;
            a_hptr.push_back((int32_t)a_hsrc.size());
            a_jptr.push_back((int32_t)a_jc.size());
            a_dsrc.push_back(-1);
        }
        if (kind[e] == -1) {
            a_dsrc[slot] = sa[e];
            sc->d_dst.push_back((int32_t)slot); sc->d_src.push_back(sa[e]);
        } else if (kind[e] == 0) {
            a_hsrc.push_back(sa[e]);
            sc->hp_dst.push_back((int32_t)slot); sc->hp_src.push_back(sa[e]);
        } else {
            a_jc.push_back(sa[e]); a_jk.push_back(sb[e]); a_jl.push_back(scc[e]);
            sc->j_dst.push_back((int32_t)slot); sc->j_c.push_back(sa[e]); sc->j_k.push_back(sb[e]); sc->j_l.push_back(scc[e]);
        }
    }
    a_hptr.push_back((int32_t)a_hsrc.size());
    a_jptr.push_back((int32_t)a_jc.size());
    for (int64_t c = 0; c < n; ++c) sc->aug_colptr[c + 1] += sc->aug_colptr[c];
    sc->nnz_aug = slot + 1;
    sc->len_jptr = L;
    sc->tile_env = mnk_tile_envelope(n, a_row.data(), a_col.data(), sc->nnz_aug);

    if (!ctx) { *out = sc; return 0; }
    hipStream_t s = ctx->stream;
    std::vector<int32_t> ptr, src;
    int rc = 0;
    group_by_slot(jt.map, sc->nnz_jt, ptr, src);
    rc |= sc->jt_seg_ptr.upload(ptr, s); rc |= sc->jt_seg_src.upload(src, s);
    group_by_slot(hh.map, sc->nnz_hess, ptr, src);
    rc |= sc->h_seg_ptr.upload(ptr, s); rc |= sc->h_seg_src.upload(src, s);
    rc |= sc->aug_hptr.upload(a_hptr, s); rc |= sc->aug_hsrc.upload(a_hsrc, s);
    rc |= sc->aug_dsrc.upload(a_dsrc, s);
    rc |= sc->aug_jptr.upload(a_jptr, s); rc |= sc->aug_jc.upload(a_jc, s);
    rc |= sc->aug_jk.upload(a_jk, s); rc |= sc->aug_jl.upload(a_jl, s);
    rc |= sc->aug_row.upload(a_row, s); rc |= sc->aug_col.upload(a_col, s);
    rc |= sc->d_tile_env.upload(sc->tile_env, s);
    rc |= sc->d_jt_colptr.upload(sc->jt_colptr, s); rc |= sc->d_jt_rowval.upload(sc->jt_rowval, s);
    rc |= sc->d_h_colptr.upload(sc->h_colptr, s); rc |= sc->d_h_rowval.upload(sc->h_rowval, s);
    rc |= sc->jac_coo.alloc(nnzj); rc |= sc->hess_coo.alloc(nnzh);
    rc |= sc->jt_nz.alloc(sc->nnz_jt); rc |= sc->h_nz.alloc(sc->nnz_hess); rc |= sc->aug_nz.alloc(sc->nnz_aug);
    rc |= sc->diag_buffer.alloc(m); rc |= sc->pr_diag.alloc(n + m); rc |= sc->du_diag.alloc(m);

    mnk_sc_extra* sp = new mnk_sc_extra();
    {
        std::vector<int32_t> rp(n + 1, 0), ri(sc->nnz_jt), rperm(sc->nnz_jt);
        for (int32_t r : jt.rowval) rp[r + 1]++;
        for (int64_t i = 0; i < n; ++i) rp[i + 1] += rp[i];
        std::vector<int32_t> cur(rp.begin(), rp.end() - 1);
        for (int64_t c = 0; c < m; ++c)
            for (int32_t k = jt.colptr[c]; k < jt.colptr[c + 1]; ++k) {
                const int32_t p = cur[jt.rowval[k]]++;
                ri[p] = (int32_t)c; rperm[p] = k;
            }
        rc |= sp->jtr_ptr.upload(rp, s); rc |= sp->jtr_idx.upload(ri, s); rc |= sp->jtr_perm.upload(rperm, s);
    }
    {
        std::vector<int32_t> cnt(n + 1, 0);
        std::vector<int32_t> hcol = col_index(hh.colptr);
        for (int64_t k = 0; k < sc->nnz_hess; ++k) {
            cnt[hcol[k] + 1]++;
            if (hh.rowval[k] != hcol[k]) cnt[hh.rowval[k] + 1]++;
        }
        for (int64_t i = 0; i < n; ++i) cnt[i + 1] += cnt[i];
        std::vector<int32_t> idx(cnt[n]), perm(cnt[n]), cur(cnt.begin(), cnt.end() - 1);
        for (int64_t k = 0; k < sc->nnz_hess; ++k)
            if (hh.rowval[k] != hcol[k]) { const int32_t p = cur[hh.rowval[k]]++; idx[p] = hcol[k]; perm[p] = (int32_t)k; }
        for (int64_t k = 0; k < sc->nnz_hess; ++k) { const int32_t p = cur[hcol[k]]++; idx[p] = hh.rowval[k]; perm[p] = (int32_t)k; }
        rc |= sp->hs_ptr.upload(cnt, s); rc |= sp->hs_idx.upload(idx, s); rc |= sp->hs_perm.upload(perm, s);
    }
    if (rc) { delete sp; delete sc; return -2; }
    MNK_HIP(hipMemsetAsync(sc->jt_nz.p, 0, sc->jt_nz.n * sizeof(double), s));
    MNK_HIP(hipMemsetAsync(sc->h_nz.p, 0, sc->h_nz.n * sizeof(double), s));
    MNK_HIP(hipMemsetAsync(sc->aug_nz.p, 0, sc->aug_nz.n * sizeof(double), s));
    sc->extra = sp;
    mnk_ctx_child_added(ctx);
    *out = sc;
    return 0;
}

int mnk_sc_destroy(mnk_sc* sc) {
    if (!sc) return 0;
    if (sc->ctx) {
        (void)hipSetDevice(sc->ctx->device);
        (void)mnk::stream_wait(sc->ctx->stream);
    }
    delete extra_of(sc);
    sc->extra = nullptr;
    mnk_ctx* ctx = sc->ctx;
    delete sc;
    mnk_ctx_child_gone(ctx);
    return 0;
}

int mnk_sc_sizes(mnk_sc* sc, int64_t* nnz_jt, int64_t* nnz_hess, int64_t* nnz_aug, int64_t* len_jptr) {
    MNK_REQUIRE(sc, "mnk_sc_sizes: NULL argument");
    if (nnz_jt) *nnz_jt = sc->nnz_jt;
    if (nnz_hess) *nnz_hess = sc->nnz_hess;
    if (nnz_aug) *nnz_aug = sc->nnz_aug;
    if (len_jptr) *len_jptr = sc->len_jptr;
    return 0;
}

int mnk_sc_debug_tile_env(mnk_sc* sc, int64_t order, int32_t* out, int cap) {
    if (sc == nullptr || order <= 0 || order > sc->n || cap < 0) return -1;
    const int n = (int)((order + 127) / 128);
    if (out != nullptr)
        for (int I = 0; I < std::min(n, cap); ++I) out[I] = sc->tile_env[I];
    return n;
}

int mnk_sc_get_structure(mnk_sc* sc, int which, int32_t* colptr, int32_t* rowval) {
    MNK_REQUIRE(sc && colptr && rowval, "mnk_sc_get_structure: NULL argument");
    const std::vector<int32_t>*cp, *rv;
    if (which == MNK_SC_JT) { cp = &sc->jt_colptr; rv = &sc->jt_rowval; }
    else if (which == MNK_SC_HESS) { cp = &sc->h_colptr; rv = &sc->h_rowval; }
    else if (which == MNK_SC_AUG) { cp = &sc->aug_colptr; rv = &sc->aug_rowval; }
    else { set_error("mnk_sc_get_structure: bad selector %d", which); return -1; }
    std::copy(cp->begin(), cp->end(), colptr);
    std::copy(rv->begin(), rv->end(), rowval);
    return 0;
}

int mnk_sc_get_map(mnk_sc* sc, int which, int64_t* map) {
    MNK_REQUIRE(sc && map, "mnk_sc_get_map: NULL argument");
    const std::vector<int64_t>* mp = which == MNK_SC_JT ? &sc->jt_map : which == MNK_SC_HESS ? &sc->h_map : nullptr;
    MNK_REQUIRE(mp != nullptr, "mnk_sc_get_map: bad selector");
    std::copy(mp->begin(), mp->end(), map);
    return 0;
}

int mnk_sc_get_ptrs(mnk_sc* sc, int32_t* d_dst, int32_t* d_src, int32_t* h_dst, int32_t* h_src, int32_t* j_dst,
                    int32_t* j_c, int32_t* j_k, int32_t* j_l) {
    MNK_REQUIRE(sc, "mnk_sc_get_ptrs: NULL argument");
    auto cp = [](const std::vector<int32_t>& v, int32_t* o) { if (o) std::copy(v.begin(), v.end(), o); };
    cp(sc->d_dst, d_dst); cp(sc->d_src, d_src); cp(sc->hp_dst, h_dst); cp(sc->hp_src, h_src);
    cp(sc->j_dst, j_dst); cp(sc->j_c, j_c); cp(sc->j_k, j_k); cp(sc->j_l, j_l);
    return 0;
}

static int stage_in(mnk_ctx* ctx, double* dev, const double* src, int64_t n, int loc, const double** use) {
    if (loc == MNK_DEVICE) { *use = src; return 0; }
    if (n > 0) {
        MNK_HIP(mnk::h2d_copy(dev, src, n * sizeof(double), ctx->stream));
    }
    *use = dev;
    return 0;
}

int mnk_sc_compress_jacobian(mnk_sc* sc, const double* jac_coo, int loc) {
    MNK_REQUIRE(sc && sc->ctx && (jac_coo || sc->nnzj == 0), "mnk_sc_compress_jacobian: NULL argument or host-only handle");
    MNK_HIP(hipSetDevice(sc->ctx->device));
    const double* src;
    int rc = stage_in(sc->ctx, sc->jac_coo.p, jac_coo, sc->nnzj, loc, &src);
    if (rc) return rc;
    if (sc->nnz_jt > 0)
        hipLaunchKernelGGL(segsum_kernel, dim3((unsigned)((sc->nnz_jt + 255) / 256)), dim3(256), 0, sc->ctx->stream,
                           sc->jt_nz.p, src, sc->jt_seg_ptr.p, sc->jt_seg_src.p, sc->nnz_jt);
    MNK_HIP(hipGetLastError());
    return 0;
}

int mnk_sc_compress_hessian(mnk_sc* sc, const double* hess_coo, int loc) {
    MNK_REQUIRE(sc && sc->ctx && (hess_coo || sc->nnzh == 0), "mnk_sc_compress_hessian: NULL argument or host-only handle");
    MNK_HIP(hipSetDevice(sc->ctx->device));
    const double* src;
    int rc = stage_in(sc->ctx, sc->hess_coo.p, hess_coo, sc->nnzh, loc, &src);
    if (rc) return rc;
    if (sc->nnz_hess > 0)
        hipLaunchKernelGGL(segsum_kernel, dim3((unsigned)((sc->nnz_hess + 255) / 256)), dim3(256), 0, sc->ctx->stream,
                           sc->h_nz.p, src, sc->h_seg_ptr.p, sc->h_seg_src.p, sc->nnz_hess);
    MNK_HIP(hipGetLastError());
    return 0;
}

int mnk_sc_build(mnk_sc* sc, const double* pr_diag, const double* du_diag, int loc) {
    MNK_REQUIRE(sc && sc->ctx, "mnk_sc_build: NULL argument or host-only handle");
    MNK_HIP(hipSetDevice(sc->ctx->device));
    hipStream_t s = sc->ctx->stream;
    if (pr_diag == nullptr && du_diag == nullptr) {
        MNK_REQUIRE(extra_of(sc)->st.have_diag, "mnk_sc_build: no diagonals given and mnk_sc_set_aug_diagonal was not called");
        pr_diag = sc->pr_diag.p;
        du_diag = sc->du_diag.p;
        loc = MNK_DEVICE;
    }
    MNK_REQUIRE(pr_diag && (du_diag || sc->m == 0), "mnk_sc_build: NULL argument");
    const double *pr, *du;
    int rc = stage_in(sc->ctx, sc->pr_diag.p, pr_diag, sc->n + sc->m, loc, &pr);
    rc |= stage_in(sc->ctx, sc->du_diag.p, du_diag, sc->m, loc, &du);
    if (rc) return rc;
    const bool keep = loc == MNK_DEVICE && pr != sc->pr_diag.p;
// ... 166 lines not shown
```

Baseline: 107.7 it/s.

## Skip leading zero k-steps per 64-row half-tile envelope in DAG GEMM updates

Adds a finer half-tile (64-row) skyline envelope next to the existing 128-row tile envelope. In the DAG update kernel, each wave computes a shared start step and its own first nonzero k-step from the envelopes of its row and column halves. Loads and the gate start later, and MFMA work is skipped for k-slices that are structurally zero for that wave's quadrant. This cuts wasted MFMA and memory traffic in the banded/envelope region of the LDL factorization, at the cost of extra per-task scalar logic and a per-iteration branch in the GEMM mainloop.

```diff
diff --git a/include/madnlp_hip.h b/include/madnlp_hip.h
--- a/include/madnlp_hip.h
+++ b/include/madnlp_hip.h
@@ -302,6 +302,9 @@
 
 int mnk_sc_debug_tile_env(mnk_sc* sc, int64_t order, int32_t* out, int cap);
 int mnk_debug_tile_env_csc(int64_t n, const int32_t* colptr, const int32_t* rowval, int index_base, int32_t* out, int cap);
+int mnk_sc_debug_tile_envh(mnk_sc* sc, int64_t order, int32_t* out, int cap);
+int mnk_debug_tile_envh_csc(int64_t n, const int32_t* colptr, const int32_t* rowval, int index_base, int32_t* out, int cap);
+int mnk_debug_envh_ksteps(int ntile, int chunk, int band_tiles, int js2, int taper0, const int* env, const int* envh, int64_t* count);
 
 int mnk_debug_update(mnk_ctx* ctx, int variant, int64_t M, int64_t K, const double* A, int64_t lda,
                      double* C, double* C2, int64_t ldc, int reps, double* ms);
diff --git a/madnlp.jl_amd/_lib.py b/madnlp.jl_amd/_lib.py
--- a/madnlp.jl_amd/_lib.py
+++ b/madnlp.jl_amd/_lib.py
@@ -236,6 +236,9 @@
     "mnk_debug_dag_deal": (C.c_int, [C.c_int] * 10 + [_vp, _vp, C.c_int, _vp, _vp]),
     "mnk_sc_debug_tile_env": (C.c_int, [_vp, C.c_int64, _vp, C.c_int]),
     "mnk_debug_tile_env_csc": (C.c_int, [C.c_int64, _vp, _vp, C.c_int, _vp, C.c_int]),
+    "mnk_sc_debug_tile_envh": (C.c_int, [_vp, C.c_int64, _vp, C.c_int]),
+    "mnk_debug_tile_envh_csc": (C.c_int, [C.c_int64, _vp, _vp, C.c_int, _vp, C.c_int]),
+    "mnk_debug_envh_ksteps": (C.c_int, [C.c_int] * 5 + [_vp, _vp, _vp]),
     "mnk_factorize_batch_begin": (C.c_int, []),
     "mnk_factorize_batch_end": (C.c_int, []),
     "mnk_solve_batch_begin": (C.c_int, []),
diff --git a/madnlp.jl_amd/csrc/common.h b/madnlp.jl_amd/csrc/common.h
--- a/madnlp.jl_amd/csrc/common.h
+++ b/madnlp.jl_amd/csrc/common.h
@@ -221,5 +221,6 @@
 constexpr int DAG_QHEAD_WORDS = (DAG_NQ + 1) * DAG_QHEAD_STRIDE;
 void dag_deal_tasks(const std::vector<int>& tasks, const std::vector<int>& ready, int t0, int t1, int nq, int gang, std::vector<int>& order,
                     std::vector<int>& off);
-
-}
+void dag_envh_count(const std::vector<int>& tasks, const int* env, const int* envh, int nenv, int64_t* count);
+
+}
diff --git a/madnlp.jl_amd/csrc/dag.hip b/madnlp.jl_amd/csrc/dag.hip
--- a/madnlp.jl_amd/csrc/dag.hip
+++ b/madnlp.jl_amd/csrc/dag.hip
@@ -26,6 +26,7 @@
     int64_t N;
     const int* env;
     const int* envgate;
+    const int* envh;
 };
 
 typedef const DagInst __attribute__((address_space(4))) * DagInstP;
@@ -471,6 +472,7 @@
     int64_t N;
     const int* env;
     const int* envgate;
+    const int* envh;
     const int* qoff;
     int* qheads;
     int nq;
@@ -514,6 +516,7 @@
     __shared__ unsigned long long s_stat[4];
     if (threadIdx.x < 4) s_stat[threadIdx.x] = 0;
     const int* __restrict__ env = a.env != nullptr && __builtin_amdgcn_readfirstlane(*a.envgate) == 0 ? a.env : nullptr;
+    const int* __restrict__ envh = env != nullptr ? a.envh : nullptr;
     __syncthreads();
     for (;;) {
         int tid = threadIdx.x;
@@ -553,6 +556,15 @@
             eI = __builtin_amdgcn_readfirstlane(env[I]);
             k0 = min(kend, max(kbeg, max(eI, __builtin_amdgcn_readfirstlane(env[J]))));
         }
+        int kf = 0, ks = 0;
+        if (envh != nullptr && (!(flags & DAG_FINAL) || (flags & DAG_BANDACC))) {
+            const int w = __builtin_amdgcn_readfirstlane(tid >> 6);
+            const int hI0 = __builtin_amdgcn_readfirstlane(envh[2 * I]), hI1 = __builtin_amdgcn_readfirstlane(envh[2 * I + 1]);
+            const int hJ0 = __builtin_amdgcn_readfirstlane(envh[2 * J]), hJ1 = __builtin_amdgcn_readfirstlane(envh[2 * J + 1]);
+            ks = min(max(8 * max(min(hI0, hI1), min(hJ0, hJ1)) - 16 * k0, 0), 16 * (kend - k0));
+            kf = (I == J && w == 2) ? INT_MAX : 8 * max((w & 1) ? hI1 : hI0, (w >> 1) ? hJ1 : hJ0) - 16 * k0 - ks;
+        }
+        const int nk = 16 * (kend - k0) - ks;
         int limit = 0;
         auto gate_at = [&](int kc) -> int {
             const unsigned long long w0 = tr ? wall_clock64() : 0;
@@ -562,13 +574,13 @@
         };
         auto gate = [&](int kt) -> bool {
             if (kt < limit) return true;
-            const int r = gate_at(k0 + (kt >> 4));
+            const int r = gate_at(k0 + ((kt + ks) >> 4));
             if (r < 0) return false;
-            limit = (__builtin_amdgcn_readfirstlane(r) - k0) * 16;
+            limit = (__builtin_amdgcn_readfirstlane(r) - k0) * 16 - ks;
             return true;
         };
-        const double* Ak = a.F + (a.fake_share > 0 ? (int64_t)128 * (kend + I % a.fake_share) : row0) + (int64_t)128 * k0 * a.ld;
-        const double* Bk = (LDL ? a.V : a.F) + (a.fake_share > 0 ? (int64_t)128 * (kend + J % a.fake_share) : col0) + (int64_t)128 * k0 * a.ld;
+        const double* Ak = a.F + (a.fake_share > 0 ? (int64_t)128 * (kend + I % a.fake_share) : row0) + (int64_t)(128 * k0 + 8 * ks) * a.ld;
+        const double* Bk = (LDL ? a.V : a.F) + (a.fake_share > 0 ? (int64_t)128 * (kend + J % a.fake_share) : col0) + (int64_t)(128 * k0 + 8 * ks) * a.ld;
         auto wait_chunk_order = [&]() -> bool {
             if (flags & DAG_FIRST) return true;
             const int* word = a.tprog + (int64_t)I * a.ntile + J;
@@ -614,10 +626,10 @@
 #pragma unroll
                 for (int j = 0; j < 4; ++j) acc[i][j] = v4f64{0.0, 0.0, 0.0, 0.0};
             if (flags & DAG_FINAL) __builtin_amdgcn_s_setprio(3);
-            if (!gemm_nt_mainloop<2, 2, 4, 0, 8>(acc, Ak, a.ld, Bk, a.ld, (kend - k0) * 16, smem_raw, tid, gate)) return;
+            if (!gemm_nt_mainloop<2, 2, 4, 0, 8>(acc, Ak, a.ld, Bk, a.ld, nk, smem_raw, tid, gate, kf)) return;
             if (tr) tr[1] = wall_clock64();
             if (!wait_chunk_order()) return;
-            if (kend > k0)
+            if (kend > k0 && kf < nk)
                 gemm_nt_epilogue<2, 2, 4, 2, false, true>(acc, row0, col0, (int64_t)1 << 40, (int64_t)1 << 40, a.F, a.ld, nullptr, nullptr, 0, tid);
             if (tr) tr[3] = wall_clock64();
         } else {
@@ -629,7 +641,7 @@
             __builtin_amdgcn_s_setprio(3);
             if (!wait_chunk_order()) return;
             gemm_nt_load_neg_lower<2, 2, 4>(acc, row0, col0, a.F, a.ld, tid);
-            if (!gemm_nt_mainloop<2, 2, 4, 0, 8>(acc, Ak, a.ld, Bk, a.ld, (kend - k0) * 16, smem_raw, tid, gate)) return;
+            if (!gemm_nt_mainloop<2, 2, 4, 0, 8>(acc, Ak, a.ld, Bk, a.ld, nk, smem_raw, tid, gate, kf)) return;
             if (tr) tr[1] = wall_clock64();
             gemm_nt_store_neg_lower<2, 2, 4>(acc, row0, col0, a.F, a.ld, tid);
             if (tr) tr[3] = wall_clock64();
@@ -787,6 +799,24 @@
     }
 }
 
+void dag_envh_count(const std::vector<int>& tasks, const int* env, const int* envh, int nenv, int64_t* count) {
+    count[0] = count[1] = 0;
+    for (size_t t = 0; t + 3 < tasks.size(); t += 4) {
+        const int flags = tasks[t] & 255, I = tasks[t + 1] & 0xffff, J = tasks[t + 2] & 0xfff, kb = tasks[t + 3] & 0xffff, ke = tasks[t + 3] >> 16;
+        if (flags & DAG_FILL) continue;
+        const bool in = env != nullptr && I < nenv && J < nenv;
+        const int k0 = in ? std::min(ke, std::max(kb, std::max(env[I], env[J]))) : kb;
+        if (in && (flags & DAG_FINAL) && !(flags & DAG_BANDACC) && J < env[I]) continue;
+        count[0] += 8 * (int64_t)(ke - k0);
+        if (!in || envh == nullptr || ((flags & DAG_FINAL) && !(flags & DAG_BANDACC))) continue;
+        for (int r = 0; r < 2; ++r)
+            for (int c = 0; c < 2; ++c) {
+                const int h0 = (I == J && r == 0 && c == 1) ? 2 * ke : std::max(envh[2 * I + r], envh[2 * J + c]);
+                count[1] += std::min(2 * ke, std::max(2 * k0, h0)) - 2 * k0;
+            }
+    }
+}
+
 template <bool LDL>
 static int launch_bulk_t(hipStream_t s, const DagArgs& a, int nwg) {
     const size_t smem = TILE3_LDS_BYTES;
@@ -826,7 +856,7 @@
     static const int fake = getenv("MNK_DAG_FAKE_SHARE") ? atoi(getenv("MNK_DAG_FAKE_SHARE")) : 0;
     if (insts == nullptr) {
         DagArgs1 a{one.F, one.ld, one.V, one.dinv, one.dblk, one.inv16, reinterpret_cast<const int4*>(tasks), ntasks, one.front, one.af,
-                   one.tprog, ntile, qctr, one.info, spin_limit, trace, wgstat, one.vmax, fake, one.zfill, one.N, one.env, one.envgate,
+                   one.tprog, ntile, qctr, one.info, spin_limit, trace, wgstat, one.vmax, fake, one.zfill, one.N, one.env, one.envgate, one.envh,
                    qoff, qheads, nq};
         return ldl ? launch_bulk1_t<true>(s, a, nwg) : launch_bulk1_t<false>(s, a, nwg);
     }
@@ -888,7 +918,7 @@
     const bool env = ls->envelope && ls->env_dev != nullptr && ls->env_word.p != nullptr;
     return mnk::DagInst{ls->fact.p, ls->ld, ls->algo == MNK_LDL ? ls->vfull.p : nullptr, ls->dinv.p, ls->dblk.p, ls->inv16.p,
                         front, af, tprog, ls->info_dev.p, mnk_ls_growth_word(ls), zfill, ls->N, env ? ls->env_dev : nullptr,
-                        env ? ls->env_word.p + 1 : nullptr};
+                        env ? ls->env_word.p + 1 : nullptr, env && ls->envelope_half ? ls->envh_dev : nullptr};
 }
 
 int mnk_ls_dag_prepare(mnk_ls* ls) {
@@ -975,6 +1005,7 @@
     const mnk::DagInst inst = dag_instance(ls);
     ls->dag_filled = inst.zfill != nullptr;
     ls->env_used = inst.env != nullptr;
+    ls->envh_used = inst.envh != nullptr;
     hipLaunchKernelGGL(mnk::dag_reset_kernel, dim3((unsigned)std::min<size_t>((nflags + 1023) / 1024, 64)), dim3(256), 0, s,
                        ls->dag_flags.p, (int64_t)nflags, ls->info_dev.p, inst, (mnk::DagInst*)nullptr, (const mnk::SmallSysRec*)nullptr,
                        ls->env_word.p, ls->dag_qheads.p, ls->dag_qheads.p ? 2 * mnk::DAG_QHEAD_WORDS : 0);
@@ -1126,6 +1157,7 @@
             hin.push_back(dag_instance(ls));
             ls->dag_filled = hin.back().zfill != nullptr;
             ls->env_used = hin.back().env != nullptr;
+            ls->envh_used = false;
             hipLaunchKernelGGL(mnk::dag_reset_kernel, dim3((unsigned)std::min<size_t>((nflags + 1023) / 1024, 64)), dim3(256), 0, h,
                                ls->dag_flags.p, (int64_t)nflags, ls->info_dev.p, hin.back(), insts_dev + (hin.size() - 1),
                                (const mnk::SmallSysRec*)nullptr, ls->env_word.p);
@@ -1259,7 +1291,9 @@
                 ls->dag_filled = hin.back().zfill != nullptr;
                 hin.back().env = nullptr;
                 hin.back().envgate = nullptr;
+                hin.back().envh = nullptr;
                 ls->env_used = false;
+                ls->envh_used = false;
                 fronts.push_back(hin.back().front);
                 afs.push_back(hin.back().af);
                 st_inst[i] = hin.back();
@@ -1456,3 +1490,11 @@
         for (int i = 0; i < std::min(n, cap) * 4; ++i) tasks_out[i] = h[i];
     return n;
 }
+
+extern "C" int mnk_debug_envh_ksteps(int ntile, int chunk, int band_tiles, int js2, int taper0, const int* env, const int* envh, int64_t* count) {
+    if (ntile <= 0 || chunk <= 0 || band_tiles <= 0 || taper0 <= 0 || count == nullptr) return -1;
+    std::vector<int> h;
+    (void)mnk::dag_build_tasks(ntile, chunk, band_tiles, js2, h, taper0, nullptr);
+    mnk::dag_envh_count(h, env, envh, ntile, count);
+    return (int)(h.size() / 4);
+}
diff --git a/madnlp.jl_amd/csrc/factor.hip b/madnlp.jl_amd/csrc/factor.hip
--- a/madnlp.jl_amd/csrc/factor.hip
+++ b/madnlp.jl_amd/csrc/factor.hip
@@ -1018,6 +1018,7 @@
     }
     ls->algo_now = ls->panel_algo;
     ls->env_used = false;
+    ls->envh_used = false;
     const int64_t min_rows = mnk_batch_active() ? std::min<int64_t>(ls->dag_min_rows, 256) : ls->dag_min_rows;
     if (ls->algo_now == 5 && (ctx->dag_cus < ls->dag_band || !ls->lookahead || Np < min_rows || Np > ls->dag_max_rows)) ls->algo_now = 4;
     if (ls->algo_now == 5 && ctx->sp_dag == nullptr && mnk_ctx_ensure_dag(ctx) != 0) { (void)hipGetLastError(); ls->algo_now = 4; }
diff --git a/madnlp.jl_amd/csrc/gemm_tile.h b/madnlp.jl_amd/csrc/gemm_tile.h
--- a/madnlp.jl_amd/csrc/gemm_tile.h
+++ b/madnlp.jl_amd/csrc/gemm_tile.h
@@ -51,7 +51,7 @@
 template <int WM, int WN, int WT, int DBG, int BKT, class GATE = GemmNoGate>
 __device__ __forceinline__ bool gemm_nt_mainloop(v4f64 (&acc)[WT][WT], const double* __restrict__ Ag, int64_t lda,
                                                  const double* __restrict__ Bg, int64_t ldb, int nk, char* smem_raw,
-                                                 int tid, GATE gate = GATE()) {
+                                                 int tid, GATE gate = GATE(), int kfirst = 0) {
     constexpr int NT = 64 * WM * WN;
     constexpr int WS = 16 * WT;
     constexpr int BM = WS * WM, BN = WS * WN;
@@ -138,19 +138,21 @@
         }
         const double* as = As + cur * BKT * LDA_S + wm * WS + l15;
         const double* bs = Bs + cur * BKT * LDB_S + wn * WS + l15;
-#pragma unroll
-        for (int kk = 0; kk < BKT / 4; ++kk) {
-            double af[WT], bf[WT];
-#pragma unroll
-            for (int i = 0; i < WT; ++i) {
-                af[i] = as[(kk * 4 + l4) * LDA_S + i * 16];
-                bf[i] = bs[(kk * 4 + l4) * LDB_S + i * 16];
-            }
-#pragma unroll
-            for (int ni = 0; ni < WT; ++ni)
-#pragma unroll
-                for (int mi = 0; mi < WT; ++mi)
-                    acc[ni][mi] = __builtin_amdgcn_mfma_f64_16x16x4f64(bf[ni], af[mi], acc[ni][mi], 0, 0, 0);
+        if (kt >= kfirst) {
+#pragma unroll
+            for (int kk = 0; kk < BKT / 4; ++kk) {
+                double af[WT], bf[WT];
+#pragma unroll
+                for (int i = 0; i < WT; ++i) {
+                    af[i] = as[(kk * 4 + l4) * LDA_S + i * 16];
+                    bf[i] = bs[(kk * 4 + l4) * LDB_S + i * 16];
+                }
+#pragma unroll
+                for (int ni = 0; ni < WT; ++ni)
+#pragma unroll
+                    for (int mi = 0; mi < WT; ++mi)
+                        acc[ni][mi] = __builtin_amdgcn_mfma_f64_16x16x4f64(bf[ni], af[mi], acc[ni][mi], 0, 0, 0);
+            }
         }
         if (DMA) {
             asm volatile("s_waitcnt vmcnt(0)" ::: "memory");
diff --git a/madnlp.jl_amd/csrc/ls.h b/madnlp.jl_amd/csrc/ls.h
--- a/madnlp.jl_amd/csrc/ls.h
+++ b/madnlp.jl_amd/csrc/ls.h
@@ -14,6 +14,8 @@
     std::vector<int32_t> jt_colptr, jt_rowval, h_colptr, h_rowval, aug_colptr, aug_rowval;
     std::vector<int32_t> tile_env;
     mnk::DevBuf<int32_t> d_tile_env;
+    std::vector<int32_t> tile_envh;
+    mnk::DevBuf<int32_t> d_tile_envh;
     std::vector<int64_t> jt_map, h_map;
     std::vector<int32_t> d_dst, d_src, hp_dst, hp_src, j_dst, j_c, j_k, j_l;
     mnk::DevBuf<int32_t> jt_seg_ptr, jt_seg_src, h_seg_ptr, h_seg_src;
@@ -40,6 +42,21 @@
         env[I] = f / 128;
     }
     return env;
+}
+
+inline std::vector<int32_t> mnk_tile_envelope_half(int64_t n, const int32_t* row, const int32_t* col, int64_t nnz) {
+    std::vector<int32_t> fnz(n);
+    for (int64_t i = 0; i < n; ++i) fnz[i] = (int32_t)i;
+    for (int64_t k = 0; k < nnz; ++k)
+        if (row[k] >= 0 && row[k] < n && col[k] < fnz[row[k]]) fnz[row[k]] = col[k];
+    const int64_t nhalf = 2 * ((n + 127) / 128);
+    std::vector<int32_t> envh(nhalf);
+    for (int64_t h = 0; h < nhalf; ++h) {
+        int32_t f = (int32_t)(64 * h);
+        for (int64_t i = 64 * h; i < std::min<int64_t>(n, 64 * h + 64); ++i) f = std::min(f, fnz[i]);
+        envh[h] = f / 64;
+    }
+    return envh;
 }
 
 struct mnk_dc {
@@ -124,6 +141,11 @@
     const int32_t* env_dev = nullptr;
     std::vector<int32_t> env_host;
     mnk::DevBuf<int32_t> env_own;
+    int envelope_half = 1;
+    const int32_t* envh_dev = nullptr;
+    std::vector<int32_t> envh_host;
+    mnk::DevBuf<int32_t> envh_own;
+    bool envh_used = false;
     mnk::DevBuf<int> env_word;
     bool env_used = false;
     bool env_armed = false;
diff --git a/madnlp.jl_amd/csrc/ls.hip b/madnlp.jl_amd/csrc/ls.hip
--- a/madnlp.jl_amd/csrc/ls.hip
+++ b/madnlp.jl_amd/csrc/ls.hip
@@ -644,6 +644,7 @@
             return 0;
         }
     if (!strcmp(key, "pivot_tol")) { ls->pivot_tol = value; return 0; }
+    if (!strcmp(key, "envelope_half")) { ls->envelope_half = value != 0.0; return 0; }
     if (!strcmp(key, "envelope")) { ls->envelope = value != 0.0; return 0; }
     if (!strcmp(key, "split_a")) { ls->split_a = (int)value; return 0; }
     if (!strcmp(key, "tail_rows")) { ls->tail_rows = (int64_t)value; return 0; }
@@ -845,8 +846,10 @@
 }
 extern "C" {
 
-static int* set_envelope(mnk_ls* ls, const int32_t* env_dev, const std::vector<int32_t>& env_host) {
+static int* set_envelope(mnk_ls* ls, const int32_t* env_dev, const std::vector<int32_t>& env_host, const int32_t* envh_dev,
+                         const std::vector<int32_t>& envh_host) {
     ls->env_dev = nullptr;
+    ls->envh_dev = nullptr;
     if (!ls->envelope || env_dev == nullptr || ls->algo == MNK_QR || ls->algo == MNK_LU || ls->algo == MNK_EVD) return nullptr;
     if (!ls->env_word.p) {
         if (ls->env_word.alloc(2) || hipMemsetAsync(ls->env_word.p, 0, 2 * sizeof(int), ls->ctx->stream) != hipSuccess) {
@@ -859,6 +862,10 @@
     ls->env_armed = true;
     ls->env_dev = env_dev;
     ls->env_host.assign(env_host.begin(), env_host.begin() + std::min<size_t>(env_host.size(), (size_t)(ls->Np / 128)));
+    if (ls->envelope_half && envh_dev != nullptr && envh_host.size() == 2 * env_host.size()) {
+        ls->envh_dev = envh_dev;
+        ls->envh_host.assign(envh_host.begin(), envh_host.begin() + 2 * ls->env_host.size());
+    }
     return ls->env_word.p;
 }
 
@@ -866,7 +873,7 @@
     int rc = prepare_fill(ls);
     if (rc) return rc;
     const int64_t nnz = sc->nnz_aug;
-    int* nonfinite = set_envelope(ls, sc->d_tile_env.p, sc->tile_env);
+    int* nonfinite = set_envelope(ls, sc->d_tile_env.p, sc->tile_env, sc->d_tile_envh.p, sc->tile_envh);
     hipLaunchKernelGGL(scatter_csc_kernel, dim3((unsigned)((nnz + 255) / 256)), dim3(256), 0, ls->ctx->stream,
                        ls->fact.p, ls->ld, sc->aug_row.p, sc->aug_col.p, sc->aug_nz.p, nnz, amax_word(ls),
                        ls->N < sc->n ? (int32_t)ls->N : INT32_MAX, nonfinite);
@@ -893,6 +900,7 @@
     mnk_ls* c = ls->probe_ls;
     c->pivot_tol = ls->pivot_tol;
     c->envelope = ls->envelope;
+    c->envelope_half = ls->envelope_half;
     if (c->dag_xcd_queues != ls->dag_xcd_queues || c->dag_gang != ls->dag_gang) {
         c->dag_xcd_queues = ls->dag_xcd_queues;
         c->dag_gang = ls->dag_gang;
@@ -1054,14 +1062,16 @@
     rc |= dcol.upload(col, ls->ctx->stream);
     rc |= dnz.upload(nzv, ls->ctx->stream);
     const std::vector<int32_t> env = ls->envelope ? mnk_tile_envelope(N, row.data(), col.data(), nnz) : std::vector<int32_t>();
+    const std::vector<int32_t> envh = ls->envelope && ls->envelope_half ? mnk_tile_envelope_half(N, row.data(), col.data(), nnz) : std::vector<int32_t>();
     if (ls->envelope) rc |= ls->env_own.upload(env, ls->ctx->stream);
+    if (!envh.empty()) rc |= ls->envh_own.upload(envh, ls->ctx->stream);
     if (rc) return -2;
     rc = ensure_wbuf(ls);
     if (rc) return rc;
-    auto transfer = [ls, nnz, &drow, &dcol, &dnz, &env]() -> int {
+    auto transfer = [ls, nnz, &drow, &dcol, &dnz, &env, &envh]() -> int {
         int r = prepare_fill(ls);
         if (r) return r;
-        int* nonfinite = set_envelope(ls, env.empty() ? nullptr : ls->env_own.p, env);
+        int* nonfinite = set_envelope(ls, env.empty() ? nullptr : ls->env_own.p, env, envh.empty() ? nullptr : ls->envh_own.p, envh);
         if (nnz > 0)
             hipLaunchKernelGGL(scatter_csc_kernel, dim3((unsigned)((nnz + 255) / 256)), dim3(256), 0, ls->ctx->stream,
                                ls->fact.p, ls->ld, drow.p, dcol.p, dnz.p, nnz, amax_word(ls), INT32_MAX, nonfinite);
@@ -1091,6 +1101,18 @@
     if (out != nullptr)
         for (int I = 0; I < std::min((int)env.size(), cap); ++I) out[I] = env[I];
     return (int)env.size();
+}
+
+int mnk_debug_tile_envh_csc(int64_t n, const int32_t* colptr, const int32_t* rowval, int index_base, int32_t* out, int cap) {
+    if (n <= 0 || colptr == nullptr || rowval == nullptr || cap < 0) return -1;
+    const int64_t nnz = colptr[n] - index_base;
+    std::vector<int32_t> row(nnz), col(nnz);
+    for (int64_t c = 0; c < n; ++c)
+        for (int64_t k = colptr[c] - index_base; k < colptr[c + 1] - index_base; ++k) { row[k] = rowval[k] - index_base; col[k] = (int32_t)c; }
+    const std::vector<int32_t> envh = mnk_tile_envelope_half(n, row.data(), col.data(), nnz);
+    if (out != nullptr)
+        for (int h = 0; h < std::min((int)envh.size(), cap); ++h) out[h] = envh[h];
+    return (int)envh.size();
 }
 
 int mnk_ls_inertia(mnk_ls* ls, int64_t* num_pos, int64_t* num_zero, int64_t* num_neg) {
@@ -1326,6 +1348,16 @@
             skipped += std::min(ke, std::max(kb, e)) - kb;
         }
         *value = (double)(!strcmp(key, "env_ksteps") ? total : skipped);
+        return 0;
+    }
+    if (!strcmp(key, "envh_ksteps") || !strcmp(key, "envh_ksteps_skipped")) {
+        int gate = 1;
+        if (ls->env_used && ls->env_word.p) MNK_HIP(mnk::d2h_copy(&gate, ls->env_word.p + 1, sizeof(int), ls->ctx->stream));
+        const bool on = ls->env_used && gate == 0;
+        int64_t cnt[2] = {0, 0};
+        mnk::dag_envh_count(ls->dag_host_tasks, on ? ls->env_host.data() : nullptr, on && ls->envh_used ? ls->envh_host.data() : nullptr,
+                            (int)ls->env_host.size(), cnt);
+        *value = (double)(!strcmp(key, "envh_ksteps") ? cnt[0] : cnt[1]);
         return 0;
     }
     set_error("mnk_ls_get_stat: unknown key '%s'", key);
diff --git a/madnlp.jl_amd/csrc/sparse_kkt.hip b/madnlp.jl_amd/csrc/sparse_kkt.hip
--- a/madnlp.jl_amd/csrc/sparse_kkt.hip
+++ b/madnlp.jl_amd/csrc/sparse_kkt.hip
@@ -242,6 +242,7 @@
     sc->nnz_aug = slot + 1;
     sc->len_jptr = L;
     sc->tile_env = mnk_tile_envelope(n, a_row.data(), a_col.data(), sc->nnz_aug);
+    sc->tile_envh = mnk_tile_envelope_half(n, a_row.data(), a_col.data(), sc->nnz_aug);
 
     if (!ctx) { *out = sc; return 0; }
     hipStream_t s = ctx->stream;
@@ -257,6 +258,7 @@
     rc |= sc->aug_jk.upload(a_jk, s); rc |= sc->aug_jl.upload(a_jl, s);
     rc |= sc->aug_row.upload(a_row, s); rc |= sc->aug_col.upload(a_col, s);
     rc |= sc->d_tile_env.upload(sc->tile_env, s);
+    rc |= sc->d_tile_envh.upload(sc->tile_envh, s);
     rc |= sc->d_jt_colptr.upload(sc->jt_colptr, s); rc |= sc->d_jt_rowval.upload(sc->jt_rowval, s);
     rc |= sc->d_h_colptr.upload(sc->h_colptr, s); rc |= sc->d_h_rowval.upload(sc->h_rowval, s);
     rc |= sc->jac_coo.alloc(nnzj); rc |= sc->hess_coo.alloc(nnzh);
@@ -328,6 +330,14 @@
     const int n = (int)((order + 127) / 128);
     if (out != nullptr)
         for (int I = 0; I < std::min(n, cap); ++I) out[I] = sc->tile_env[I];
+    return n;
+}
+
+int mnk_sc_debug_tile_envh(mnk_sc* sc, int64_t order, int32_t* out, int cap) {
+    if (sc == nullptr || order <= 0 || order > sc->n || cap < 0) return -1;
+    const int n = 2 * (int)((order + 127) / 128);
+    if (out != nullptr)
+        for (int h = 0; h < std::min(n, cap); ++h) out[h] = sc->tile_envh[h];
     return n;
 }
 
```

Result: faster. 108.8 it/s (median of 6 runs) (+1.0%).
